# omerkurt-okt/buck-gnn

Hardware: AMD Instinct MI355X
Metric: graphs/sec (fwd+bwd) 6-layer SAGE h=512, ~5k-node meshes, batch 16, 1/2/4/8 GPU (higher is better)
Workload: dtype f32

## Files before the change

### buck-gnn_amd/bgnn/_lib.py

```python
from __future__ import annotations

import ctypes
import os
import threading

_HERE = os.path.dirname(os.path.abspath(__file__))
LIB_PATH = os.environ.get("BGNN_LIBRARY") or os.path.join(_HERE, "_lib", "libbgnn.so")
ABI_VERSION = 17

_lock = threading.Lock()
_lib = None

c_p = ctypes.c_void_p
c_i32 = ctypes.c_int32
c_i64 = ctypes.c_int64
c_f32 = ctypes.c_float
c_u64 = ctypes.c_uint64
c_sz = ctypes.c_size_t


class CsrStruct(ctypes.Structure):

    _fields_ = [
        ("rowptr", c_p),
        ("col", c_p),
        ("heavy_row", c_p),
        ("heavy_chunk0", c_p),
        ("chunk_heavy", c_p),
        ("n_rows", c_i64),
        ("nnz", c_i64),
        ("n_heavy", c_i32),
        ("n_chunks", c_i32),
        ("chunk", c_i32),
        ("ranges_all", c_i32),
        ("gsrc", c_p),
        ("gmask", c_p),
        ("gcnt", c_p),
        ("grow", c_p),
        ("n_groups", c_i64),
        ("group_rows", c_i32),
        ("_pad2", c_i32),
        ("ranges", c_p),
    ]


SIGNATURES = {
    "bgnn_abi_version": (c_i32, []),
    "bgnn_last_error_string": (ctypes.c_char_p, []),
    "bgnn_store_gather_graph": (c_i32, [c_p, c_i32, c_i64, c_i64, c_i64, c_i64, c_p, c_i64, c_p, c_p, c_p, c_p,
                                        c_p, c_p, c_p, c_p, c_p, c_p, c_p, c_p, c_p]),
    "bgnn_store_gather_rows": (c_i32, [c_p, c_i32, c_i32, c_i64, c_p, c_i64, c_p, c_p]),
    "bgnn_get_tuning": (c_i32, [c_i32]),
    "bgnn_heavy_timing": (c_i32, [c_i32]),
    "bgnn_gemm_w_tile": (c_i32, [c_i64, c_i64, c_i64]),
    "bgnn_gemm_wsplit_bytes": (c_sz, [c_i64, c_i64]),
    "bgnn_gemm_wsplit": (c_i32, [c_p, c_i32, c_i64, c_i64, c_i64, c_i64, c_p, c_i64, c_p, c_i64, c_i32, c_p]),
    "bgnn_gemm_f32_w": (c_i32, [c_i64, c_i64, c_i64, c_p, c_i64, c_p, c_i32, c_p, c_i64, c_p, c_i32, c_p, c_p, c_p,
                                c_p, c_i64, c_f32, c_u64, c_p]),
    "bgnn_heavy_timing_read": (c_i32, [c_i32, c_p, c_p]),
    "bgnn_set_tuning": (c_i32, [c_i32, c_i32]),
    "bgnn_graph_build_ws_bytes": (c_sz, [c_i64, c_i64]),
    "bgnn_graph_build": (c_i32, [c_p, c_i64, c_i64, c_p, c_p, c_p, c_p, c_p, c_p, c_sz, c_p, c_p]),
    "bgnn_index_csr_build": (c_i32, [c_p, c_i64, c_i64, c_p, c_p, c_p, c_sz, c_p, c_p]),
    "bgnn_heavy_plan_ws_bytes": (c_sz, [c_i64]),
    "bgnn_heavy_plan": (c_i32, [c_p, c_i64, c_i64, c_i32, c_p, c_p, c_p, c_p, c_p, c_sz, c_p]),
    "bgnn_spmm_fwd": (c_i32, [ctypes.POINTER(CsrStruct), c_p, c_i64, c_i32, c_i32, c_p, c_i64, c_p, c_p, c_p]),
    "bgnn_spmm_bwd": (c_i32, [ctypes.POINTER(CsrStruct), c_p, c_p, c_p, c_i64, c_i32, c_i32, c_p, c_i64, c_p, c_p,
                              c_i32, c_p]),
    "bgnn_heavy_ranges_bytes": (c_sz, [c_i32]),
    "bgnn_heavy_ranges": (c_i32, [ctypes.POINTER(CsrStruct), c_p, c_p]),
    "bgnn_range_partial_bytes": (c_sz, [c_i64, c_i32]),
    "bgnn_range_sums_finish": (c_i32, [c_p, c_i64, c_i32, ctypes.POINTER(CsrStruct), c_i32, c_p, c_i64, c_p, c_p,
                                       c_p]),
    "bgnn_bn_slots": (c_i32, [c_i64, c_i32]),
    "bgnn_bn_stats": (c_i32, [c_p, c_i64, c_i32, c_p, c_p]),
    "bgnn_bn_apply": (c_i32, [c_p, c_i64, c_i32, c_p, c_p, c_p, c_p]),
    "bgnn_bn_bwd_stats": (c_i32, [c_p, c_p, c_p, c_p, c_i64, c_i32, c_p, c_p]),
    "bgnn_bn_bwd_dx": (c_i32, [c_p, c_p, c_p, c_p, c_p, c_p, c_i64, c_i32, c_p, c_p]),
    "bgnn_spmm_bwd_add": (c_i32, [ctypes.POINTER(CsrStruct), c_p, c_p, c_p, c_i64, c_i32, c_i32, c_p, c_i64, c_p,
                                  c_i64, c_p, c_p, c_p]),
    "bgnn_spmm_bwd_max": (c_i32, [ctypes.POINTER(CsrStruct), c_p, c_p, c_i64, c_p, c_i64, c_i32, c_p, c_p, c_i64, c_p,
                                  c_i64, c_p, c_p, c_p]),
    "bgnn_spmm_max_arg_bytes": (c_sz, [c_i64, c_i32, c_i32]),
    "bgnn_sage_fwd_slots": (c_i32, [ctypes.POINTER(CsrStruct)]),
    "bgnn_group_plan": (c_i32, [c_p, c_p, c_i64, c_i32, c_i32, c_p, c_i64, c_p, c_p, c_p, c_p]),
    "bgnn_store_gather_groups": (c_i32, [c_p, c_i32, c_i32, c_i64, c_i64, c_i64, c_i64] + [c_p] * 14),
    "bgnn_sage_fwd": (c_i32, [ctypes.POINTER(CsrStruct), c_p, c_i64, c_p, c_i64, c_p, c_i32, c_i32, c_p, c_p, c_p,
                              c_p, c_p, c_i64, c_p]),
    "bgnn_bn_finalize": (c_i32, [c_p, c_i32, c_i32, c_i64, c_p, c_p, c_f32, c_f32, c_p, c_p, c_p, c_p, c_p, c_p,
                                 c_p]),
    "bgnn_bn_finalize_shifted": (c_i32, [c_p, c_i32, c_i32, c_i64, c_p, c_p, c_p, c_f32, c_f32, c_p, c_p, c_p, c_p, c_p, c_p,
                                 c_p]),
    "bgnn_bn_eval_coeffs": (c_i32, [c_i32, c_p, c_p, c_f32, c_p, c_p, c_p, c_p, c_p]),
    "bgnn_sage_apply": (c_i32, [c_p, c_p, c_p, c_p, c_i32, c_f32, c_u64, c_i64, c_i32, c_p, c_p, c_p, c_p, c_p]),
    "bgnn_sage_infer_bf16": (c_i32, [ctypes.POINTER(CsrStruct), c_p, c_i64, c_p, c_p, c_p, c_p, c_i64, c_i32, c_i32,
                                     c_p, c_i64, c_i32, c_p, c_p]),
    "bgnn_spmm_fwd_bf16": (c_i32, [ctypes.POINTER(CsrStruct), c_p, c_i64, c_i32, c_i32, c_p, c_i64, c_i32, c_p, c_p]),
    "bgnn_spmm_bwd_bf16": (c_i32, [ctypes.POINTER(CsrStruct), c_p, c_p, c_i64, c_i32, c_i32, c_p, c_i64, c_i32, c_p,
                                   c_p]),
    "bgnn_spmm_max_bf16": (c_i32, [ctypes.POINTER(CsrStruct), c_p, c_i64, c_i32, c_p, c_i64, c_p, c_p, c_p]),
    "bgnn_sage_tail_bf16": (c_i32, [c_p, c_i64, c_p, c_p, c_p, c_p, c_i64, c_i64, c_i32, c_p, c_i64, c_i32, c_p]),
    "bgnn_rows_slots": (c_i32, [c_i64]),
    "bgnn_sage_bwd_stats": (c_i32, [c_p, c_p, c_p, c_p, c_p, c_p, c_p, c_f32, c_u64, c_i64, c_i32, c_p, c_p]),
    "bgnn_reduce_partials": (c_i32, [c_p, c_i32, c_i32, c_p, c_p, c_i32, c_p]),
    "bgnn_linear_bwd_prep_slots": (c_i32, []),
    "bgnn_linear_bwd_prep": (c_i32, [c_p, c_p, c_i64, c_i32, c_p, c_p, c_p, c_p]),
    "bgnn_linear_bwd_prep_bf16": (c_i32, [c_p, c_p, c_i64, c_i32, c_p, c_p, c_p]),
    "bgnn_absmax_items_f32": (c_i32, [c_p, c_i32, c_i64, c_i64, c_i64, c_i64, c_p, c_i64, c_p]),
    "bgnn_add_dropped_bf16": (c_i32, [c_p, c_p, c_i64, c_f32, c_u64, c_p, c_p]),
    "bgnn_gemm_bf16_dropadd": (c_i32, [c_i64, c_i64, c_i64, c_p, c_i64, c_p, c_i64, c_p, c_i64, c_p, c_i64, c_f32,
                                       c_u64, c_p]),
    "bgnn_rel_error_loss": (c_i32, [c_p, c_p, c_i64, c_f32, c_f32, c_f32, c_p, c_p, c_p]),
    "bgnn_small_linear_fwd": (c_i32, [c_p, c_i64, c_i32, c_p, c_p, c_i32, c_i32, c_p, c_p]),
    "bgnn_small_linear_bwd": (c_i32, [c_p, c_p, c_p, c_i64, c_i32, c_p, c_i32, c_p, c_p, c_p, c_p]),
    "bgnn_sage_bwd_rows": (c_i32, [c_p, c_p, c_p, c_p, c_p, c_p, c_p, c_p, c_p, c_p, c_p, c_f32, c_u64, c_i32, c_i64,
                                   c_i32, c_p, c_i64, c_p, c_p, c_p, c_p, c_i32, c_p, c_p, c_p, c_p]),
    "bgnn_l2norm_bwd": (c_i32, [c_p, c_p, c_p, c_i64, c_i32, c_p, c_i64, c_p, c_p, c_p]),
    "bgnn_gemm_bf16": (c_i32, [c_i32, c_i32, c_i64, c_i64, c_i64, c_f32, c_p, c_i64, c_p, c_i64, c_f32, c_p, c_i64,
                               c_p, c_i32, c_i32, c_p, c_sz, c_p]),
    "bgnn_gemm_gather_add_bf16": (c_i32, [c_i64, c_i64, c_i64, c_p, c_i64, c_p, c_i64, c_p, c_i64, c_p, c_i32, c_p,
                                          c_p, c_i64, c_p, c_p, c_i64, c_i32, c_p, c_sz, c_p]),
    "bgnn_gemm_b16_variant": (c_i32, [c_i32]),
    "bgnn_add_dropout_bf16": (c_i32, [c_p, c_p, c_i64, c_f32, c_u64, c_p, c_p]),
    "bgnn_segment_sum_bf16": (c_i32, [c_p, c_p, c_i64, c_p, c_i64, c_i32, c_i32, c_p, c_i64, c_p]),
    "bgnn_segment_bcast_bf16": (c_i32, [c_p, c_p, c_i64, c_p, c_i64, c_i32, c_i32, c_p, c_i64, c_p]),
    "bgnn_gemm_ws_bytes": (c_sz, [c_i64, c_i64, c_i64, c_i32, c_i32]),
    "bgnn_gemm_set_cfg": (c_i32, [c_i32]),
    "bgnn_gemm_f32_planes": (c_i32, [c_i32, c_i32, c_i64, c_i64, c_i64, c_f32, c_p, c_i64, c_i64, c_i64, c_p, c_i64,
                                     c_f32, c_p, c_i64, c_i64, c_i64, c_p, c_i32, c_p, c_sz, c_p]),
    "bgnn_gemm_f32_scaled": (c_i32, [c_i32, c_i32, c_i64, c_i64, c_i64, c_f32, c_p, c_i64, c_i64, c_i64, c_p, c_i64,
                                     c_f32, c_p, c_i64, c_i64, c_i64, c_p, c_i32, c_p, c_p, c_p, c_i32, c_p, c_sz,
                                     c_p]),
    "bgnn_gemm_ws_bytes_ex": (c_sz, [c_i64, c_i64, c_i64, c_i32, c_i32, c_i32]),
    "bgnn_gemm_gather_add": (c_i32, [c_i32, c_i32, c_i64, c_i64, c_i64, c_p, c_i64, c_p, c_i64, c_p, c_i64, c_p, c_i32,
                                     c_p, c_p, c_i64, c_p, c_p, c_i64, c_i32, c_p, c_sz, c_p]),
    "bgnn_absmax_f32": (c_i32, [c_p, c_i64, c_i64, c_i64, c_p, c_i32, c_p]),
    "bgnn_gemm_f32_ex": (c_i32, [c_i32, c_i32, c_i64, c_i64, c_i64, c_f32, c_p, c_i64, c_p, c_i64, c_f32, c_p,
                                 c_i64, c_p, c_i32, c_p, c_sz, c_p]),
    "bgnn_topk_rank": (c_i32, [c_p, c_p, c_p, c_i64, c_p, c_p]),
    "bgnn_topk_select": (c_i32, [c_p, c_p, c_p, c_p, c_i64, c_p, c_p, c_p, c_p]),
    "bgnn_gather_scale": (c_i32, [c_p, c_i64, c_i32, c_p, c_p, c_i64, c_p, c_i64, c_p]),
    "bgnn_gather_scale_bwd": (c_i32, [c_p, c_i64, c_p, c_i64, c_i32, c_p, c_p, c_i64, c_p, c_i64, c_p, c_p]),
    "bgnn_filter_edges_ws_bytes": (c_sz, [c_i64]),
    "bgnn_filter_edges": (c_i32, [c_p, c_i64, c_p, c_i64, c_p, c_p, c_p, c_p, c_sz, c_p]),
    "bgnn_mlp2_supported": (c_i32, [c_i32, c_i32, c_i32]),
    "bgnn_mlp2_fwd": (c_i32, [c_p, c_i64, c_i32, c_i32, c_i32, c_p, c_p, c_p, c_p, c_p, c_p, c_p]),
    "bgnn_mlp2_bwd_ws_bytes": (c_sz, [c_i64]),
    "bgnn_mlp2_bwd": (c_i32, [c_p, c_i64, c_i32, c_i32, c_i32, c_p, c_p, c_p, c_p, c_p, c_p, c_p, c_p, c_p, c_p,
                              c_sz, c_p]),
    "bgnn_gemm_f32_dropadd": (c_i32, [c_i32, c_i32, c_i64, c_i64, c_i64, c_p, c_i64, c_p, c_i64, c_p, c_i64, c_p,
                                      c_p, c_p, c_i64, c_f32, c_u64, c_p, c_sz, c_p]),
    "bgnn_gemm_f32_dropadd_cols": (c_i32, [c_i64, c_i64, c_i64, c_p, c_i64, c_p, c_i64, c_p, c_i64, c_p, c_p, c_p,
                                           c_i64, c_i64, c_f32, c_u64, c_p, c_sz, c_p]),
    "bgnn_add_dropout": (c_i32, [c_p, c_p, c_i64, c_f32, c_u64, c_p, c_p]),
    "bgnn_fold_weights_supported": (c_i32, [c_i64, c_i64]),
    "bgnn_fold_weights_ws_bytes": (c_sz, [c_i64, c_i64]),
    "bgnn_fold_weights_fwd": (c_i32, [c_i64, c_i64, c_p, c_i64, c_p, c_i64, c_p, c_p, c_p, c_i64, c_p, c_p, c_i64,
                                      c_p, c_p]),
    "bgnn_fold_weights_bwd": (c_i32, [c_i64, c_i64, c_p, c_i64, c_p, c_p, c_i64, c_p, c_i64, c_p, c_p, c_p, c_i64,
                                      c_p, c_i64, c_p, c_p, c_sz, c_p]),
    "bgnn_gemm_f32": (c_i32, [c_i32, c_i32, c_i64, c_i64, c_i64, c_f32, c_p, c_i64, c_p, c_i64, c_f32, c_p, c_i64,
                              c_p, c_sz, c_p]),
}


class BgnnError(RuntimeError):
    def __init__(self, fn: str, code: int, msg: str):
        super().__init__(f"{fn} failed with code {code}: {msg}")
        self.code = code


def load():
    global _lib
    if _lib is not None:
        return _lib
    with _lock:
        if _lib is not None:
            return _lib
        if not os.path.exists(LIB_PATH):
            raise ImportError(
                f"bgnn: native library not found at {LIB_PATH}; build it with "
                "`python -c 'import __graft_entry__ as g; g.build()'` or `make -C buck-gnn_amd`")
        lib = ctypes.CDLL(LIB_PATH)
        for name, (res, args) in SIGNATURES.items():
            fn = getattr(lib, name)
            fn.restype = res
            fn.argtypes = args
        v = lib.bgnn_abi_version()
        if v != ABI_VERSION:
            raise ImportError(f"bgnn: ABI version mismatch (library {v}, python {ABI_VERSION})")
        _lib = lib
        return lib


def _checked(lib, name: str, args):
    fn = getattr(lib, name)
    sig = SIGNATURES.get(name)
    if sig is not None and len(args) != len(sig[1]):
        raise TypeError(f"bgnn: {name} takes {len(sig[1])} arguments, {len(args)} given")
    return fn


def call(name: str, *args):
    lib = load()
    rc = _checked(lib, name, args)(*args)
    if rc != 0:
        msg = lib.bgnn_last_error_string().decode(errors="replace")
        raise BgnnError(name, rc, msg)
    return rc


def query(name: str, *args):
    lib = load()
    return _checked(lib, name, args)(*args)
```

### buck-gnn_amd/bgnn/buckgnn.py

```python
from __future__ import annotations

from typing import Optional

import torch
from torch import Tensor, nn

from . import ea as ea_mod
from .ea import GradSlot as EAGradSlot, graphnet_block, skip_dropout
from . import _lib
from . import fused as _fused
from .fused import RangeRows, mlp, mlp_bf16, prepare_weights, sage_layer, small_mlp
from .graph import SegmentIndex, graph_for, _index_cache
from .nn import SAGEConv, SAGPooling, global_mean_pool, scatter_mean
from .ops import segment_reduce

FUSED_ENCODER = True
FOLD_ENCODER = True
FUSED_POOL = True

_SAGE_VARIANTS = {
    "GraphSage_sumAggr": ("sage_blocks_sum", "sum", True),
    "GraphSage_addAggr": ("sage_blocks_add", "add", True),
    "GraphSage_meanAggr": ("sage_blocks_mean", "mean", True),
    "GraphSage_maxAggr": ("sage_blocks_max", "max", True),
# ... 110 lines not shown
            self.batch_norms = nn.ModuleList()
            self.sage_mlps = nn.ModuleList()
            for _ in range(num_layers):
                getattr(self, attr).append(SAGEConv(in_channels=h, out_channels=h, normalize=True, aggr=aggr))
                self.batch_norms.append(nn.BatchNorm1d(h))
                self.sage_mlps.append(nn.Linear(h, h))
        self.batch_norm = nn.BatchNorm1d(h)
        self.relu = nn.ReLU()
        self.dropout = nn.Dropout(p=dropout_rate)
        self.pooling_mpl = MLPPooling(h, h, h)
        if model_name in ("GraphSAGE_SAG", "EAGNN_SAG"):
            n_before = num_layers // 2
            n_after = num_layers - n_before
            sag = model_name == "GraphSAGE_SAG"
            pre, bns = ("sage_layers_", True) if sag else ("gnn_layers_", False)

            def block():
                return SAGEConv(h, h, normalize=True, aggr="add") if sag else GraphNetBlock(h)
            setattr(self, pre + "1", nn.ModuleList([block() for _ in range(n_before)]))
            self.batch_norms_1 = nn.ModuleList([nn.BatchNorm1d(h) for _ in range(n_before)] if bns else [])
            self.pool = SAGPooling(h, ratio=0.5, GNN=SAGEConv, aggr="add")
            setattr(self, pre + "2", nn.ModuleList([block() for _ in range(n_after)]))
            self.batch_norms_2 = nn.ModuleList([nn.BatchNorm1d(h) for _ in range(n_after)] if bns else [])
        self.use_fused = True
        self.ea_bf16 = False
        self.infer_bf16 = False
        self._step = 0

    def get_pooling_layer(self, x: Tensor, edge_index: Tensor, batch: Optional[Tensor]) -> Tensor:
        mode = self.pooling_layer
        if mode == "mean":
            if batch is None:
                return global_mean_pool(x, None)
            return segment_reduce(x, batch_segments(batch), "mean")
        if mode == "hybrid":
            raise AttributeError("'BuckGNN' object has no attribute 'hybrid_pooling'")
        if mode == "mlp":
            return self.pooling_mpl(x, batch)
        if "super" not in mode and mode != "mlp_no_super" and mode != "mean_no_super":
            raise ValueError(f"Unknown pooling layer: {mode}")
        sup = super_node_index(batch, x.size(0), x.device)
        keep = torch.ones(x.size(0), dtype=torch.bool, device=x.device)
        keep[sup] = False
        real = torch.nonzero(keep).flatten()
        if batch is None:
            rb = torch.zeros(real.numel(), dtype=torch.long, device=x.device)
        else:
            rb = batch[real]
        if mode == "mean_no_super":
            return global_mean_pool(x[real], rb)
        if mode == "supernode_only":
            return x[sup]
        if mode == "supernode_with_pooling":
            return torch.cat([global_mean_pool(x[real], rb), x[sup]], 1)
        if mode == "mlp_no_super":
            return self.pooling_mpl(x[real], rb)
        raise ValueError(f"Unknown pooling layer: {mode}")

    def _seed(self) -> int:
        return int(torch.randint(0, 2 ** 62, (1,)).item())

    def _decode(self, h: Tensor) -> Tensor:
        dec = self.decoder
        hooked = bool(dec._forward_pre_hooks or dec._forward_hooks)
        out = small_mlp(dec, h) if (self.use_fused and not hooked) else None
        return dec(h) if out is None else out

    def _fused_ok(self, x: Tensor) -> bool:
        return (self.use_fused and x.is_cuda and x.dtype == torch.float32 and self.hidden_channels % 4 == 0
                and self.hidden_channels <= 512)

    def _sage_fused(self, x: Tensor, aggr: str) -> bool:
        return self._fused_ok(x) and aggr in ("add", "sum", "mean", "max")

    def _infer_bf16_on(self, x: Tensor, aggr: str, bns) -> bool:
        h = self.hidden_channels
        aggrs = ("add", "sum", "mean", "max") if self.infer_bf16 == "all" else ("add", "sum", "mean")
        return bool(self.infer_bf16 and not self.training and not torch.is_grad_enabled()
                    and self._fused_ok(x) and aggr in aggrs and h % 8 == 0 and h <= 512
                    and (bns is None or all(bn.track_running_stats and bn.running_mean is not None
                                            for bn in bns)))

    def _sage_loop_bf16(self, x: Tensor, edge_index: Tensor, convs, bns, aggr: str, pool=None):
        L = len(convs) if convs is not None else self.num_layers
        graph = graph_for(edge_index, x.size(0))
        if aggr == "max":
            x = self._sage_loop_bf16_max(x, graph, convs, bns, L)
            return (x, segment_reduce(x, pool, "mean")) if pool is not None else x
        red = 1 if aggr == "mean" else 0
        for i in range(L):
            conv = convs[i] if convs is not None else self.shared_graphsage_block
            coeffs = _fused.bn_eval_coeffs(bns[i]) if bns is not None else None
            x = _fused.sage_infer_layer(x, _fused.infer_weights(conv), conv.lin_l.bias, coeffs, graph, red,
                                        x_prev=x if 0 < i < L - 1 else None, out_f32=i == L - 1)
        return (x, segment_reduce(x, pool, "mean")) if pool is not None else x

    def _sage_loop_bf16_max(self, x: Tensor, graph, convs, bns, L: int) -> Tensor:
        if L == 0:
            return x
        N, H = x.size(0), self.hidden_channels
        bufs = [torch.empty(N, 2 * H, dtype=torch.bfloat16, device=x.device) for _ in range(min(L, 2))]
        y = torch.empty(N, H, dtype=torch.bfloat16, device=x.device)
        bufs[0][:, H:].copy_(x)
        out = None
        for i in range(L):
            conv = convs[i] if convs is not None else self.shared_graphsage_block
            coeffs = _fused.bn_eval_coeffs(bns[i]) if bns is not None else None
            cur = bufs[i % 2]
            last = i == L - 1
            out = (torch.empty(N, H, dtype=torch.float32, device=x.device) if last
                   else bufs[(i + 1) % 2][:, H:])
            _fused.sage_infer_max_layer(cur, _fused.infer_weights_max(conv), conv.lin_l.bias, coeffs, graph,
                                        cur[:, H:] if 0 < i < L - 1 else None, out, out_f32=last, y=y)
        return out

    def _foldable_encoder(self, x: Tensor) -> bool:
        enc = self.node_encoder
        return (FOLD_ENCODER and FUSED_ENCODER and isinstance(enc, nn.Sequential) and len(enc) >= 2
                and isinstance(enc[-1], nn.Linear) and enc[-1].out_features == self.hidden_channels
                and x.size(0) >= 1024 and self.num_layers >= 1)

    def _sage_loop(self, x: Tensor, edge_index: Tensor, convs, bns, aggr: str, skip_last_excluded: bool,
                   x_amax: Optional[Tensor] = None, x_in: Optional[nn.Linear] = None, pool=None):
        L = len(convs) if convs is not None else self.num_layers
        p = self.dropout.p
        if x_in is None and self._infer_bf16_on(x, aggr, bns):
            return self._sage_loop_bf16(x, edge_index, convs, bns, aggr, pool)
        if self._sage_fused(x, aggr):
            graph = graph_for(edge_index, x.size(0))
            red = {"mean": 1, "max": 2}.get(aggr, 0)
            amax = x_amax
            scratch = torch.zeros(4 * L + 5, dtype=torch.float32, device=x.device)
            bufs, fold_amax = scratch[:4 * L].view(L, 4), scratch[4 * L:]
            layers = [convs[i] if convs is not None else self.shared_graphsage_block for i in range(L)]
            rng_on = _range_rows_on(graph, red, x.size(0), layers[0].lin_l.weight.size(0))
            R = graph.fwd.plan.n_heavy if rng_on else 0
            wprep = prepare_weights([(c.lin_l.weight, c.lin_r.weight) for c in layers], bufs,
                                    [not (i == 0 and x_in is not None) for i in range(L)],
                                    n_rows=x.size(0) + R if red != 2 else 0)
            self._count_bn_batches(bns)
            x_full = None
            for i in range(L):
                conv = layers[i]
                bn = bns[i] if bns is not None else None
                skip = 0 < i < L - 1
                fold = x_in if i == 0 else None
                rng = (RangeRows(x_full=x_full, x_amax=bufs[i - 1, 3:4] if x_full is not None else None,
                                 out=i < L - 1, out_amax=bufs[i, 3:4]) if rng_on else None)
                pl = pool if (i == L - 1 and red != 2) else None
                out = sage_layer(x, conv.lin_l.weight, conv.lin_l.bias, conv.lin_r.weight, bn, graph, red,
                                 skip, p, self.training, self._seed(), x_amax=amax, return_amax=True,
                                 amax_buf=bufs[i], w_in=None if fold is None else fold.weight,
                                 b_in=None if fold is None else fold.bias, wprep=wprep[i], count_batch=False,
                                 fold_amax=fold_amax, rng=rng, pool=pl)
                x, amax = out[0], out[1]
                x_full = rng.holder[0] if (rng is not None and rng.holder) else None
            if pool is not None:
                return x, (out[2] if (red != 2 and L > 0) else segment_reduce(x, pool, "mean"))
            return x
        if x_in is not None:
            x = x_in(x)
        for i in range(L):
            x_prev = x
            conv = convs[i] if convs is not None else self.shared_graphsage_block
            x = conv(x, edge_index)
            if bns is not None:
                x = bns[i](x)
            x = self.relu(x)
            if 0 < i < L - 1:
                x = x + x_prev
            x = self.dropout(x)
        return (x, segment_reduce(x, pool, "mean")) if pool is not None else x

    def _count_bn_batches(self, bns) -> None:
        if bns is None or not self.training:
            return
        ts = [bn.num_batches_tracked for bn in bns if bn.track_running_stats]
        if ts:
            torch._foreach_add_(ts, 1)

    def _sag_sage_loop(self, x: Tensor, edge_index: Tensor, convs, bns, first_skip: bool,
                       x_amax: Optional[Tensor] = None, x_in: Optional[nn.Linear] = None) -> Tensor:
        p = self.dropout.p
        if self._sage_fused(x, "add"):
            graph = graph_for(edge_index, x.size(0))
            bufs = torch.zeros(len(convs), 3, dtype=torch.float32, device=x.device)
            for i, (conv, bn) in enumerate(zip(convs, bns)):
                skip = first_skip or i > 0
                fold = x_in if i == 0 else None
                y, y_amax = sage_layer(x, conv.lin_l.weight, conv.lin_l.bias, conv.lin_r.weight, bn, graph, 0,
                                       False, p, self.training, self._seed(), x_amax=x_amax, return_amax=True,
                                       amax_buf=bufs[i], w_in=None if fold is None else fold.weight,
                                       b_in=None if fold is None else fold.bias)
                x, x_amax = (y + x, None) if skip else (y, y_amax)
            return x
        if x_in is not None:
            x = x_in(x)
        for i, (conv, bn) in enumerate(zip(convs, bns)):
            identity = x
            x = self.dropout(self.relu(bn(conv(x, edge_index))))
            if first_skip or i > 0:
                x = x + identity
        return x

    def _skip_dropout(self, x, e, x_prev, e_prev, skip: bool, fused: bool, e_slot=None):
        if not fused:
            if skip:
                x, e = x + x_prev, e + e_prev
            return self.dropout(x), self.dropout(e)
        p = self.dropout.p
        return (skip_dropout(x, x_prev if skip else None, p, self.training, self._seed()),
                skip_dropout(e, e_prev if skip else None, p, self.training, self._seed(), slot=e_slot))

    def _ea_block(self, blk, x, e, edge_index, fused: bool):
        return graphnet_block(blk, x, e, edge_index, self.ea_bf16) if fused else blk(x, edge_index, e)

    def forward(self, x, edge_index, edge_attr, batch=None, mask=None):
        name = self.model_name
        if "super" in self.pooling_layer:
            is_real_node = x[:, -1] == 0 if x.size(1) > 0 else torch.ones(x.size(0), dtype=torch.bool,
                                                                           device=x.device)
            real_node_batch = batch[is_real_node] if batch is not None else None
        x_amax = None
        x_in = None
        sage = _SAGE_VARIANTS.get(name, (None, "add", None))[1] if name != "GraphSage_addAggr_Shared" else "add"
        infer = ((name in _SAGE_VARIANTS or name == "GraphSage_addAggr_Shared")
                 and self._infer_bf16_on(x, sage, self.batch_norms if name in _SAGE_VARIANTS else None))
        if (name in _SAGE_VARIANTS or name == "GraphSage_addAggr_Shared"
                or (name == "GraphSAGE_SAG" and len(self.sage_layers_1) >= 1)) and not infer \
                and self._sage_fused(x, sage) and sage != "max" and self._foldable_encoder(x):
            x_in = self.node_encoder[-1]
            x, x_amax = mlp(self.node_encoder[:-1], x, return_amax=True)
        elif self._fused_ok(x) and x.size(0) >= 1024 and FUSED_ENCODER:
            x, x_amax = mlp(self.node_encoder, x, return_amax=True)
        else:
            x = self.node_encoder(x)
        ea_fused = name in ("EA_GNN", "EA_GNN_Shared", "EAGNN_SAG") and self._fused_ok(x)
        if ea_fused:
            if self.ea_bf16 and ea_mod.BF16_STORAGE and edge_attr.size(0) >= 1024 and FUSED_ENCODER:
                e = mlp_bf16(self.edge_encoder, edge_attr)
            else:
                e = (mlp(self.edge_encoder, edge_attr) if edge_attr.size(0) >= 1024 and FUSED_ENCODER
                     else self.edge_encoder(edge_attr))
        if name == "EA_GNN_Shared":
            if not ea_fused:
                e = self.edge_encoder(edge_attr)
            for i in range(self.num_layers):
                x_prev, e_prev = x, e
                if ea_fused:
                    x, e = graphnet_block(self.shared_gn_block, x, e, edge_index, self.ea_bf16)
                else:
                    x, e = self.shared_gn_block(x, edge_index, e)
                x, e = self._skip_dropout(x, e, x_prev, e_prev, 0 < i < self.num_layers - 1, ea_fused)
        pool = (batch_segments(batch) if (FUSED_POOL and self.prediction_type == "buckling"
                                          and self.pooling_layer == "mean" and batch is not None
                                          and (name == "GraphSage_addAggr_Shared" or name in _SAGE_VARIANTS)
                                          and self._sage_fused(x, sage) and sage != "max") else None)
        pooled = None
        if name == "GraphSage_addAggr_Shared":
            x = self._sage_loop(x, edge_index, None, None, "add", True, x_amax, x_in, pool=pool)
            if pool is not None:
                x, pooled = x
        elif name == "EA_GNN":
            if not ea_fused:
                e = self.edge_encoder(edge_attr)
            L = len(self.gn_blocks)
            for i, blk in enumerate(self.gn_blocks):
                x_prev, e_prev = x, e
                slot = EAGradSlot() if (ea_fused and self.ea_bf16 and self.training and i < L - 1) else None
                if ea_fused:
                    x, e = graphnet_block(blk, x, e, edge_index, self.ea_bf16, slot=slot, slot_in=0 < i < L - 1)
                else:
                    x, e = blk(x, edge_index, e)
                x, e = self._skip_dropout(x, e, x_prev, e_prev, 0 < i < L - 1, ea_fused, e_slot=slot)
        elif name in _SAGE_VARIANTS:
            attr, aggr, _ = _SAGE_VARIANTS[name]
            x = self._sage_loop(x, edge_index, getattr(self, attr), self.batch_norms, aggr, True, x_amax, x_in,
                                pool=pool)
            if pool is not None:
                x, pooled = x
        elif name in ("GraphSage_addAggr_woBatchNorm", "GraphSage_MLP"):
            getattr(self, "sage_blocks_add")
        elif name == "GraphSage_sumAggr_woBatchNorm":
            getattr(self, "sage_blocks_sum")
        elif name == "GraphSAGE_SAG":
            x = self._sag_sage_loop(x, edge_index, self.sage_layers_1, self.batch_norms_1, False, x_amax, x_in)
            x, edge_index, edge_attr, batch, _perm, _score = self.pool(x, edge_index, edge_attr, batch)
            x = self._sag_sage_loop(x, edge_index, self.sage_layers_2, self.batch_norms_2, True)
        elif name == "EAGNN_SAG":
            if not ea_fused:
                e = self.edge_encoder(edge_attr)
            for i, blk in enumerate(self.gnn_layers_1):
                x_prev, e_prev = x, e
                x, e = self._ea_block(blk, x, e, edge_index, ea_fused)
                x, e = self.dropout(x), self.dropout(e)
                if i > 0:
                    x, e = x + x_prev, e + e_prev
            x, edge_index, e, batch, _perm, _score = self.pool(x, edge_index, e, batch)
            for blk in self.gnn_layers_2:
                x_prev, e_prev = x, e
                x, e = self._ea_block(blk, x, e, edge_index, ea_fused)
                x, e = self.dropout(x), self.dropout(e)
                x, e = x + x_prev, e + e_prev

        if self.prediction_type == "buckling":
            if pooled is None:
                pooled = self.get_pooling_layer(x, edge_index, batch)
# ... 7 lines not shown
```

### buck-gnn_amd/bgnn/fused.py

```python
from __future__ import annotations

import torch

from . import _lib
from .graph import Graph, _stream, require_cuda

GEMM_BACKEND = "hip"

PLANE_TILE = 128
Z_PLANES = False
DZ_PLANES = False
DGRAD_WT = True
FOLD_WEIGHTS_TORCH = False
FOLD_NATIVE = True
DGRAD_DROPADD = True

BF16_PREP = True
ABSMAX_ITEMS = True
PERSISTENT_WPACK = True
MAX_MERGED = True
WSPLIT = True

TIMERS = None
TIMER_EVENT = None
# ... 332 lines not shown
        ws_bytes = _lib.query("bgnn_mlp2_bwd_ws_bytes", N)
        ws = torch.empty(max(ws_bytes, 1), dtype=torch.uint8, device=x.device)
        _lib.call("bgnn_mlp2_bwd", x.data_ptr(), N, F, D1, D2, W1.data_ptr(), b1.data_ptr(), W2.data_ptr(),
                  h.data_ptr(), dh.data_ptr(), dW1.data_ptr(), db1.data_ptr(), dW2.data_ptr(), db2.data_ptr(),
                  ws.data_ptr(), ws_bytes, _stream())
        return None, dW1, db1, dW2, db2


class SmallMLPFn(torch.autograd.Function):

    @staticmethod
    def forward(ctx, x, relus, *params):
        x = x.contiguous()
        B = x.size(0)
        s = _stream()
        acts = [x]
        for i, relu in enumerate(relus):
            W, b = params[2 * i], params[2 * i + 1]
            N, K = W.shape
            y = torch.empty(B, N, dtype=torch.float32, device=x.device)
            _lib.call("bgnn_small_linear_fwd", acts[-1].data_ptr(), B, K, W.data_ptr(), _ptr(b), N, int(relu),
                      y.data_ptr(), s)
            acts.append(y)
        ctx.relus = relus
        ctx.has_bias = [params[2 * i + 1] is not None for i in range(len(relus))]
        ctx.save_for_backward(*acts, *[params[2 * i] for i in range(len(relus))])
        return acts[-1]

    @staticmethod
    def backward(ctx, g):
        L = len(ctx.relus)
        saved = ctx.saved_tensors
        acts, Ws = saved[:L + 1], saved[L + 1:]
        s = _stream()
        g = g.contiguous()
        B = g.size(0)
        grads = [None] * (2 * L)
        gx = None
        for i in reversed(range(L)):
            W = Ws[i]
            N, K = W.shape
            dW = torch.empty_like(W)
            db = torch.empty(N, dtype=torch.float32, device=W.device) if ctx.has_bias[i] else None
            need_dx = i > 0 or ctx.needs_input_grad[0]
            dx = torch.empty(B, K, dtype=torch.float32, device=W.device) if need_dx else None
            _lib.call("bgnn_small_linear_bwd", g.data_ptr(), acts[i + 1].data_ptr() if ctx.relus[i] else None,
                      acts[i].data_ptr(), B, K, W.data_ptr(), N, _ptr(dx), dW.data_ptr(), _ptr(db), s)
            grads[2 * i], grads[2 * i + 1] = dW, db
            g = dx
            gx = dx
        return (gx, None, *grads)


SMALL_MLP = True
SMALL_MLP_MAX_ROWS = 256


def small_mlp(seq: torch.nn.Sequential, x: torch.Tensor):
    if not (SMALL_MLP and x.is_cuda and x.dtype == torch.float32 and x.dim() == 2
            and 0 < x.size(0) <= SMALL_MLP_MAX_ROWS):
        return None
    mods = list(seq)
    relus, params = [], []
    i = 0
    while i < len(mods):
        m = mods[i]
        if not (isinstance(m, torch.nn.Linear) and m.weight.dtype == torch.float32 and m.in_features % 4 == 0
                and m.weight.is_contiguous()):
            return None
        relu = i + 1 < len(mods) and isinstance(mods[i + 1], torch.nn.ReLU)
        relus.append(relu)
        params += [m.weight, m.bias]
        i += 2 if relu else 1
    return SmallMLPFn.apply(x, tuple(relus), *params)


def _mlp2_prefix(mods, x: torch.Tensor) -> bool:
    if not FUSED_MLP2 or len(mods) < 4 or x.requires_grad or x.dtype != torch.float32 or x.dim() != 2:
        return False
    l1, r1, l2, r2 = mods[:4]
    if not (isinstance(l1, torch.nn.Linear) and isinstance(l2, torch.nn.Linear) and isinstance(r1, torch.nn.ReLU)
            and isinstance(r2, torch.nn.ReLU) and l1.bias is not None and l2.bias is not None):
        return False
    if l2.in_features != l1.out_features or x.size(1) != l1.in_features:
        return False
    return bool(_lib.query("bgnn_mlp2_supported", l1.in_features, l1.out_features, l2.out_features))


def _require_f32(x: torch.Tensor, what: str) -> None:
    if x.dtype != torch.float32:
        raise TypeError(f"{what}: the fused path takes float32 activations (got {x.dtype}); bf16 features run on "
                        "the per-module path (bgnn.nn.SAGEConv)")


def mlp(seq: torch.nn.Sequential, x: torch.Tensor, return_amax: bool = False, bf16: bool = False):
    _require_f32(x, "mlp")
    mods = list(seq)
    i = 0
    amax = None
    if not bf16 and _mlp2_prefix(mods, x):
        x, amax = _Mlp2Fn.apply(x.contiguous(), mods[0].weight, mods[0].bias, mods[2].weight, mods[2].bias)
        if len(mods) == 4:
            return (x, amax) if return_amax else x
        mods = mods[4:]
    n_lin = sum(isinstance(m, torch.nn.Linear) for m in mods)
    bufs = torch.zeros(n_lin, 2, dtype=torch.float32, device=x.device)
    k = 0
    while i < len(mods):
        m = mods[i]
        if isinstance(m, torch.nn.Linear):
            fuse = i + 1 < len(mods) and isinstance(mods[i + 1], torch.nn.ReLU)
            x, amax = linear(x, m.weight, m.bias, fuse, x_amax=amax, return_amax=True, bf16=bf16, amax_buf=bufs[k])
            k += 1
            i += 2 if fuse else 1
        else:
            x = m(x)
            amax = None
            i += 1
    return (x, amax) if return_amax else x


def _ptr(t):
    return None if t is None else t.data_ptr()


class RangeRows:
    __slots__ = ("x_full", "x_amax", "out", "out_amax", "bwd", "holder")

    def __init__(self, x_full=None, x_amax=None, out=False, out_amax=None, bwd=True):
        self.x_full, self.x_amax, self.out, self.out_amax, self.bwd = x_full, x_amax, out, out_amax, bwd
        self.holder = []


RANGE_ROWS = True


class LayerConfig:
    __slots__ = ("reduce", "bn", "training", "momentum", "eps", "skip", "p", "seed", "famax", "rng")

    def __init__(self, reduce: int, bn: bool, training: bool, momentum: float, eps: float, skip: bool,
                 p: float, seed: int):
        self.reduce = reduce
        self.bn = bn
        self.training = training
        self.momentum = momentum
        self.eps = eps
        self.skip = skip
        self.p = p if training else 0.0
        self.seed = seed
        self.famax = None
        self.rng = None


def _glue_fwd(o, bn_part, slots, x_prev, gamma, beta, running_mean, running_var, cfg: LayerConfig, next_amax,
              graph: Graph = None):
    N, H = o.shape
    dev = o.device
    s = _stream()
    scale = shift = mean = invstd = None
    if cfg.bn:
        scale = torch.empty(H, dtype=torch.float32, device=dev)
        shift = torch.empty(H, dtype=torch.float32, device=dev)
        mean = torch.empty(H, dtype=torch.float32, device=dev)
        invstd = torch.empty(H, dtype=torch.float32, device=dev)
        if cfg.training:
            _lib.call("bgnn_bn_finalize", bn_part.data_ptr(), slots, H, N, _ptr(gamma), _ptr(beta), cfg.eps,
                      cfg.momentum, _ptr(running_mean), _ptr(running_var), mean.data_ptr(), invstd.data_ptr(),
                      scale.data_ptr(), shift.data_ptr(), s)
        else:
            _lib.call("bgnn_bn_eval_coeffs", H, _ptr(gamma), _ptr(beta), cfg.eps, running_mean.data_ptr(),
                      running_var.data_ptr(), scale.data_ptr(), shift.data_ptr(), s)
            mean.copy_(running_mean)
            invstd.copy_(torch.rsqrt(running_var + cfg.eps))
    rng = cfg.rng
    if rng is not None and rng.out:
        R = graph.fwd.plan.n_heavy
        full = torch.empty(N + R, H, dtype=torch.float32, device=dev)
        x_next = full[:N]
        rp = torch.empty(_lib.query("bgnn_range_partial_bytes", N, H) // 4, dtype=torch.float32, device=dev)
        _lib.call("bgnn_sage_apply", o.data_ptr(), _ptr(scale), _ptr(shift), x_prev.data_ptr(), int(cfg.skip),
                  float(cfg.p), cfg.seed, N, H, x_next.data_ptr(), next_amax.data_ptr(), graph.fwd.ranges.data_ptr(),
                  rp.data_ptr(), s)
        _lib.call("bgnn_range_sums_finish", rp.data_ptr(), N, H, graph.fwd.ref(), 0, full[N:].data_ptr(), H,
                  next_amax.data_ptr(), rng.out_amax.data_ptr(), s)
        rng.holder.append(full)
        return x_next, (scale, shift, mean, invstd)
    x_next = torch.empty(N, H, dtype=torch.float32, device=dev)
    _lib.call("bgnn_sage_apply", o.data_ptr(), _ptr(scale), _ptr(shift), x_prev.data_ptr(), int(cfg.skip),
              float(cfg.p), cfg.seed, N, H, x_next.data_ptr(), next_amax.data_ptr(), None, None, s)
    return x_next, (scale, shift, mean, invstd)


def _glue_bwd_stats(g, o, scale, shift, mean, invstd, cfg: LayerConfig, g_rows=None):
    if not cfg.bn:
        return None, None, None, None
    N, H = o.shape
    dev = o.device
    s = _stream()
    rs = _lib.query("bgnn_rows_slots", N)
    part2 = torch.empty(rs, 2, H, dtype=torch.float32, device=dev)
    _lib.call("bgnn_sage_bwd_stats", g.data_ptr(), _ptr(g_rows), o.data_ptr(), scale.data_ptr(), shift.data_ptr(),
              mean.data_ptr(), invstd.data_ptr(), float(cfg.p), cfg.seed, N, H, part2.data_ptr(), s)
    sums = torch.empty(2, H, dtype=torch.float32, device=dev)
    _lib.call("bgnn_reduce_partials", part2.data_ptr(), rs, H, sums[0].data_ptr(), sums[1].data_ptr(), 0, s)
    dbeta, dgamma = sums[0], sums[1]
    if cfg.training:
        return dgamma, dbeta, sums[0], sums[1]
    z = torch.zeros(H, dtype=torch.float32, device=dev)
    return dgamma, dbeta, z, z


def _fold_native_ok(famax, wcat, w_in, b_in) -> bool:
    return bool(FOLD_NATIVE and GEMM_BACKEND == "hip" and famax is not None and famax.is_contiguous()
                and famax.numel() >= 5 and wcat.stride(1) == 1 and w_in.stride(1) == 1 and b_in.is_contiguous()
                and _lib.query("bgnn_fold_weights_supported", wcat.size(1), w_in.size(1)))


class SageLayerFn(torch.autograd.Function):

    @staticmethod
    def forward(ctx, x_prev, x_amax, w_l, b_l, w_r, gamma, beta, running_mean, running_var, graph: Graph,
                cfg: LayerConfig, amax=None, w_in=None, b_in=None, wprep=None, pool=None):
        dev = x_prev.device
        x_prev = x_prev.contiguous()
        H = w_l.size(0)
        N = x_prev.size(0)
        if isinstance(wprep, WPrep):
            wcat, wcat_t_pre, img_f, img_d = wprep.wcat, wprep.wcat_t, wprep, wprep
        elif wprep is not None:
            (wcat, wcat_t_pre), img_f, img_d = wprep, None, None
        else:
            wcat, wcat_t_pre, img_f, img_d = torch.cat([w_l, w_r], 0).contiguous(), None, None, None
        img_f = img_f if (img_f is not None and img_f.img_f is not None) else None
        img_d = img_d if (img_d is not None and img_d.img_d is not None) else None
        if amax is None:
            amax = torch.zeros(3, dtype=torch.float32, device=dev)
        w_amax, next_amax, dz_amax = amax[0:1], amax[1:2], amax[2:3]
        folded = w_in is not None
        if folded:
            if cfg.skip:
                raise ValueError("sage_layer: a folded input transform needs a layer without skip")
            wf_t = None
            fold_native = not FOLD_WEIGHTS_TORCH and _fold_native_ok(cfg.famax, wcat, w_in, b_in)
            if FOLD_WEIGHTS_TORCH:
                wf = torch.mm(wcat, w_in)
                bf = torch.mv(wcat, b_in)
            elif fold_native:
                K_in = w_in.size(1)
                wf = torch.empty(2 * H, K_in, dtype=torch.float32, device=dev)
                bf = torch.empty(2 * H, dtype=torch.float32, device=dev)
                wf_t = torch.empty(K_in, 2 * H, dtype=torch.float32, device=dev) if DGRAD_WT else None
                _lib.call("bgnn_fold_weights_fwd", H, K_in, wcat.data_ptr(), wcat.stride(0), w_in.data_ptr(),
                          w_in.stride(0), b_in.data_ptr(), cfg.famax.data_ptr(), wf.data_ptr(), K_in, bf.data_ptr(),
                          _ptr(wf_t), 2 * H, w_amax.data_ptr(), _stream())
            else:
                fs = cfg.famax
                fa = (fs[0:1], fs[1:2], fs[2:3]) if fs is not None else (None, None, None)
                if fs is not None:
                    absmax(wcat, fa[0], accumulate=True)
                    absmax(w_in, fa[1], accumulate=True)
                    absmax(b_in.view(1, -1), fa[2], accumulate=True)
                wf = gemm(wcat, w_in.contiguous(), trans_a=False, trans_b=False, a_amax=fa[0], b_amax=fa[1])
                bf = gemm(wcat, b_in.contiguous().view(H, 1), trans_a=False, trans_b=False, a_amax=fa[0],
                          b_amax=fa[2]).view(-1)
            if not fold_native:
                absmax(wf, w_amax, accumulate=True)
            wmat = wf
        else:
            if wprep is None:
                absmax(wcat, w_amax, accumulate=True)
            wmat, bf = wcat, None
        if x_amax is None:
            x_amax = absmax(x_prev)
        planes = Z_PLANES and H % PLANE_TILE == 0 and not folded
        rng = cfg.rng
        x_full = rng.x_full if (rng is not None and rng.x_full is not None and not folded and not planes) else None
        if x_full is not None and x_full.data_ptr() != x_prev.data_ptr():
            raise RuntimeError("sage_layer: RangeRows.x_full must start at x_prev")
        xa, a_amax_g = (x_full, rng.x_amax) if x_full is not None else (x_prev, x_amax)
        M = xa.size(0)
        with _timed("gemm_fwd_fold" if folded else "gemm_fwd"):
            if planes:
                z = torch.empty(2, N, H, dtype=torch.float32, device=dev)
                gemm(x_prev, wmat, trans_a=False, trans_b=True, out=Planes(z), a_amax=x_amax, b_amax=w_amax)
                zl, zr, ldz = z[0], z[1], H
            elif (img_f is not None and not folded
                  and _lib.query("bgnn_gemm_w_tile", M, 2 * H, H) == img_f.bn_f):
                z = torch.empty(M, 2 * H, dtype=torch.float32, device=dev)
                _lib.call("bgnn_gemm_f32_w", M, 2 * H, H, xa.data_ptr(), xa.stride(0), img_f.img_f.data_ptr(),
                          img_f.bn_f, z.data_ptr(), 2 * H, None, 0, a_amax_g.data_ptr(), w_amax.data_ptr(), None, None,
                          0, 0.0, 0, _stream())
                zl, zr, ldz = z, z[:, H:], 2 * H
            else:
                z = gemm(xa, wmat, trans_a=False, trans_b=True, bias=bf, a_amax=a_amax_g, b_amax=w_amax)
                zl, zr, ldz = z, z[:, H:], 2 * H
        hagg = z[N:] if x_full is not None else None
        o = torch.empty(N, H, dtype=torch.float32, device=dev)
        nrm = torch.empty(N, dtype=torch.float32, device=dev)
        slots = _lib.query("bgnn_sage_fwd_slots", graph.fwd.ref())
        bn_part = torch.empty(slots, 2, H, dtype=torch.float32, device=dev)
        part = (torch.empty(graph.fwd.plan.n_chunks * H, dtype=torch.float32, device=dev)
                if graph.fwd.plan.n_chunks else None)
        s = _stream()
        with _timed("sage_fwd"):
            _lib.call("bgnn_sage_fwd", graph.fwd.ref(), zl.data_ptr(), ldz, zr.data_ptr(), ldz, b_l.data_ptr(), H,
                      cfg.reduce, o.data_ptr(), nrm.data_ptr(), bn_part.data_ptr(), _ptr(part), _ptr(hagg),
                      2 * H if hagg is not None else 0, s)
        del z, zl, zr, hagg
        x_next, (scale, shift, mean, invstd) = _glue_fwd(o, bn_part, slots, x_prev, gamma, beta, running_mean,
                                                         running_var, cfg, next_amax, graph)
        ctx.graph = graph
        ctx.cfg = cfg
        ctx.folded = folded
        ctx.wcat_t = wcat_t_pre
        ctx.img_d = img_d if not folded else None
        ctx.set_materialize_grads(False)
        ctx.fold = (w_in, b_in, wf, wf_t) if folded else None
        ctx.save_for_backward(x_prev, o, nrm, wcat, gamma if gamma is not None else torch.empty(0, device=dev),
                              scale if scale is not None else torch.empty(0, device=dev),
                              shift if shift is not None else torch.empty(0, device=dev),
                              mean if mean is not None else torch.empty(0, device=dev),
                              invstd if invstd is not None else torch.empty(0, device=dev),
                              x_amax, w_amax, dz_amax)
        ctx.mark_non_differentiable(next_amax)
        ctx.pool = pool
        if pool is not None:
            from .ops import spmm_fwd
            pooled, _ = spmm_fwd(pool.fwd, x_next, 1, pool.num_rows)
            return x_next, next_amax, pooled
        return x_next, next_amax

    @staticmethod
    def backward(ctx, g, _g_amax, g_pool=None):
        cfg: LayerConfig = ctx.cfg
        g_rows = None
        if g_pool is not None:
            seg = ctx.pool
            gp = g_pool.contiguous() / seg.fwd.degree().clamp_min(1).to(g_pool.dtype).unsqueeze(1)
            if g is None and not cfg.skip:
                g, g_rows = gp, seg.index
            else:
                gb = gp.index_select(0, seg.index)
                g = gb if g is None else g + gb
        if g is None:
            return (None,) * 16
        x_prev, o, nrm, wcat, gamma, scale, shift, mean, invstd, x_amax, w_amax, dz_amax = ctx.saved_tensors
        graph: Graph = ctx.graph
        g = g.contiguous()
        N, H = o.shape
        planes = DZ_PLANES and H % PLANE_TILE == 0
        dev = o.device
        s = _stream()
        bn = cfg.bn
        dgamma, dbeta, sum_g2, sum_g2xhat = _glue_bwd_stats(g, o, scale, shift, mean, invstd, cfg, g_rows)
        if planes:
            dzt = torch.empty(2, N, H, dtype=torch.float32, device=dev)
            dz, dzl, dh, lddz = Planes(dzt), dzt[0], dzt[1], H
        else:
            dz = torch.empty(N, 2 * H, dtype=torch.float32, device=dev)
            dzl, dh, lddz = dz, dz[:, H:], 2 * H
        dropadd = (cfg.skip and DGRAD_DROPADD and GEMM_BACKEND == "hip" and DGRAD_WT and not planes
                   and H % 4 == 0 and _lib.query("bgnn_get_tuning", 5) == 2)
        gskip = torch.empty(N, H, dtype=torch.float32, device=dev) if (cfg.skip and not dropadd) else None
        rs = _lib.query("bgnn_rows_slots", N)
        part_db = torch.empty(rs, 2, H, dtype=torch.float32, device=dev)
        bw = graph.bwd
        rb = (cfg.rng is not None and cfg.rng.bwd and not planes and bw.ranges is not None)
        rp = (torch.empty(_lib.query("bgnn_range_partial_bytes", N, H) // 4, dtype=torch.float32, device=dev)
              if rb else None)
        _lib.call("bgnn_sage_bwd_rows", g.data_ptr(), _ptr(g_rows), o.data_ptr(), nrm.data_ptr(),
                  _ptr(scale) if bn else None, _ptr(shift) if bn else None,
                  _ptr(gamma) if (bn and gamma.numel()) else None,
                  _ptr(mean) if bn else None, _ptr(invstd) if bn else None, _ptr(sum_g2), _ptr(sum_g2xhat),
                  float(cfg.p), cfg.seed, int(cfg.skip and not dropadd), N, H, dh.data_ptr(), lddz, _ptr(gskip),
                  part_db.data_ptr(), dz_amax.data_ptr(), graph.fwd.rowptr.data_ptr() if ctx.folded else None,
                  (2 if cfg.reduce == 1 else 1) if ctx.folded else 0, _ptr(bw.ranges) if rb else None,
                  graph.fwd.rowptr.data_ptr() if (rb and cfg.reduce == 1) else None, _ptr(rp), s)
        if rb:
            _lib.call("bgnn_range_sums_finish", rp.data_ptr(), N, H, bw.ref(), 1, dzl.data_ptr(), lddz, None,
                      dz_amax.data_ptr(), s)
        db2 = torch.empty(2 if ctx.folded else 1, H, dtype=torch.float32, device=dev)
        _lib.call("bgnn_reduce_partials", part_db.data_ptr(), rs, H, db2[-1].data_ptr(),
                  db2[0].data_ptr() if ctx.folded else None, 0, s)
        db, db_zl = db2[-1], (db2[0] if ctx.folded else None)
        part = torch.empty(bw.plan.n_chunks * H, dtype=torch.float32, device=dev) if bw.plan.n_chunks else None
        with _timed("spmm_bwd"):
            _lib.call("bgnn_spmm_bwd", bw.ref(), graph.perm_t.data_ptr(), graph.fwd.rowptr.data_ptr(),
                      dh.data_ptr(), lddz, H, cfg.reduce, dzl.data_ptr(), lddz, _ptr(part),
                      dz_amax.data_ptr(), int(rb), s)
        has_affine = bn and gamma.numel() > 0
        if ctx.folded:
            w_in, b_in, wf, wf_t = ctx.fold
            wf_t = (wf_t if wf_t is not None else wf.t().contiguous()) if DGRAD_WT else wf
            with _timed("gemm_dgrad_fold"):
                dx = gemm(dz, wf_t, trans_a=False, trans_b=DGRAD_WT, a_amax=dz_amax, b_amax=w_amax)
            fs = cfg.famax
            fa = (fs[0:1], fs[1:2], fs[2:3], fs[3:4], fs[4:5]) if fs is not None else (None,) * 5
            with _timed("gemm_wgrad_fold"):
                dwf = gemm(dz, x_prev, trans_a=True, trans_b=False, a_amax=dz_amax, b_amax=x_amax,
                           c_amax=fa[3])
            dbf = db2.view(-1)
            fold_native = not FOLD_WEIGHTS_TORCH and _fold_native_ok(fs, wcat, w_in, b_in) and dwf.stride(1) == 1
            if fs is not None and not fold_native:
                absmax(db2, fa[4], accumulate=True)
            if fold_native:
                K_in = w_in.size(1)
                dw = torch.empty(2 * H, H, dtype=torch.float32, device=dev)
                dw_in = torch.empty(H, K_in, dtype=torch.float32, device=dev)
                db_in = torch.empty(H, dtype=torch.float32, device=dev)
                ws_bytes = _lib.query("bgnn_fold_weights_ws_bytes", H, K_in)
                ws = torch.empty(ws_bytes, dtype=torch.uint8, device=dev) if ws_bytes else None
                _lib.call("bgnn_fold_weights_bwd", H, K_in, dwf.data_ptr(), dwf.stride(0), dbf.data_ptr(),
                          wcat.data_ptr(), wcat.stride(0), w_in.data_ptr(), w_in.stride(0), b_in.data_ptr(),
                          fs.data_ptr(), dw.data_ptr(), H, dw_in.data_ptr(), K_in, db_in.data_ptr(), _ptr(ws),
                          ws_bytes, s)
            elif FOLD_WEIGHTS_TORCH:
                dw = torch.addmm(torch.outer(dbf, b_in), dwf, w_in.t())
                dw_in = torch.mm(wcat.t(), dwf)
                db_in = torch.mv(wcat.t(), dbf)
            else:
                dw = gemm(dwf, w_in.contiguous(), trans_a=False, trans_b=True, a_amax=fa[3],
                          b_amax=fa[1])
                dw.add_(torch.outer(dbf, b_in))
                dw_in = gemm(wcat, dwf, trans_a=True, trans_b=False, a_amax=fa[0], b_amax=fa[3])
                db_in = gemm(wcat, dbf.view(-1, 1), trans_a=True, trans_b=False, a_amax=fa[0],
                             b_amax=fa[4]).view(-1)
            return (dx, None, dw[:H], db, dw[H:], dgamma if has_affine else None, dbeta if has_affine else None,
                    None, None, None, None, None, dw_in, db_in, None, None)
        wcat_t = (ctx.wcat_t if ctx.wcat_t is not None else wcat.t().contiguous()) if DGRAD_WT else wcat
        img_d = ctx.img_d if (not planes and DGRAD_WT) else None
        if (img_d is not None and (dropadd or gskip is None)
                and _lib.query("bgnn_gemm_w_tile", N, H, 2 * H) == img_d.bn_d):
            dx = torch.empty(N, H, dtype=torch.float32, device=dev)
            with _timed("gemm_dgrad"):
                _lib.call("bgnn_gemm_f32_w", N, H, 2 * H, dz.data_ptr(), lddz, img_d.img_d.data_ptr(), img_d.bn_d,
                          dx.data_ptr(), H, None, 0, dz_amax.data_ptr(), w_amax.data_ptr(), None,
                          g.data_ptr() if dropadd else None, H, float(cfg.p) if dropadd else 0.0,
                          cfg.seed if dropadd else 0, s)
        elif dropadd:
            dx = torch.empty(N, H, dtype=torch.float32, device=dev)
            M_, K_ = N, 2 * H
            ws_bytes = _lib.query("bgnn_gemm_ws_bytes_ex", M_, H, K_, 0, 1, 0)
            ws = torch.empty(ws_bytes, dtype=torch.uint8, device=dev) if ws_bytes else None
            with _timed("gemm_dgrad"):
                _lib.call("bgnn_gemm_f32_dropadd", 0, 1, M_, H, K_, dz.data_ptr(), lddz, wcat_t.data_ptr(),
                          wcat_t.stride(0), dx.data_ptr(), H, dz_amax.data_ptr(), w_amax.data_ptr(), g.data_ptr(),
                          H, float(cfg.p), cfg.seed, _ptr(ws), ws_bytes, s)
        elif gskip is not None:
            with _timed("gemm_dgrad"):
                dx = gemm(dz, wcat_t, trans_a=False, trans_b=DGRAD_WT, out=gskip, beta=1.0, a_amax=dz_amax,
                          b_amax=w_amax)
        else:
            with _timed("gemm_dgrad"):
                dx = gemm(dz, wcat_t, trans_a=False, trans_b=DGRAD_WT, a_amax=dz_amax, b_amax=w_amax)
        with _timed("gemm_wgrad"):
            dw = gemm(dz, x_prev, trans_a=True, trans_b=False, a_amax=dz_amax, b_amax=x_amax)
        dw_l, dw_r = dw[:H], dw[H:]
        return (dx, None, dw_l, db, dw_r, dgamma if has_affine else None, dbeta if has_affine else None,
                None, None, None, None, None, None, None, None, None)


def _max_transform(x, w_l, w_r, graph: Graph, x_amax, w_amax, name: str):
    from .ops import spmm_fwd
    N, C = x.shape
    with _timed("agg_max"):
        agg, arg = spmm_fwd(graph.fwd, x, 2, N, want_arg=True)
    wk = torch.cat([w_l, w_r], 1)
    in_place = C % 32 == 0 and (x.data_ptr() - agg.data_ptr()) % 16 == 0
    a = Pair(agg, x) if in_place else torch.cat([agg, x], 1)
    with _timed(name):
        y = gemm(a, wk, trans_a=False, trans_b=True, a_amax=x_amax, b_amax=w_amax)
    return y, agg, arg


def _max_rows_fwd(y, b_l, H: int):
    from .graph import empty_csr
    N = y.size(0)
    dev = y.device
    csr = empty_csr(N, dev)
    bias = b_l if b_l is not None else torch.zeros(H, dtype=torch.float32, device=dev)
    o = torch.empty(N, H, dtype=torch.float32, device=dev)
    nrm = torch.empty(N, dtype=torch.float32, device=dev)
    slots = _lib.query("bgnn_sage_fwd_slots", csr.ref())
    bn_part = torch.empty(slots, 2, H, dtype=torch.float32, device=dev)
    _lib.call("bgnn_sage_fwd", csr.ref(), y.data_ptr(), y.stride(0), y.data_ptr(), y.stride(0), bias.data_ptr(), H,
              0, o.data_ptr(), nrm.data_ptr(), bn_part.data_ptr(), None, None, 0, _stream())
    return o, nrm, bn_part, slots


def _max_backward(dh, dz_amax, wcat_t, x, agg, arg, graph: Graph, x_amax, w_amax, addend_beta_src,
                  need_dx: bool, p: float = 0.0, seed: int = 0):
    N, H = dh.shape
    C = x.size(1)
    dev = dh.device
    dx = None
    hip16 = GEMM_BACKEND == "hip" and _lib.query("bgnn_get_tuning", 5) == 2
    if need_dx and MAX_MERGED and hip16 and C % 256 == 0:
        wkt = torch.cat([wcat_t[:, :H], wcat_t[:, H:]], 0)
        with _timed("gemm_dgrad"):
            dt = torch.empty(N, 2 * C, dtype=torch.float32, device=dev)
            if addend_beta_src is not None:
                ws_bytes = _lib.query("bgnn_gemm_ws_bytes_ex", N, 2 * C, H, 0, 1, 0)
                ws = torch.empty(ws_bytes, dtype=torch.uint8, device=dev) if ws_bytes else None
                _lib.call("bgnn_gemm_f32_dropadd_cols", N, 2 * C, H, dh.data_ptr(), dh.stride(0), wkt.data_ptr(), H,
                          dt.data_ptr(), 2 * C, dz_amax.data_ptr(), w_amax.data_ptr(), addend_beta_src.data_ptr(),
                          addend_beta_src.stride(0), C, float(p), seed, _ptr(ws), ws_bytes, _stream())
            else:
                gemm(dh, wkt, trans_a=False, trans_b=True, out=dt, a_amax=dz_amax, b_amax=w_amax)
        dagg, t = dt[:, :C], dt[:, C:]
        dx = torch.empty(N, C, dtype=torch.float32, device=dev)
        bw = graph.bwd
        part = torch.empty(bw.plan.n_chunks * C, dtype=torch.float32, device=dev) if bw.plan.n_chunks else None
        with _timed("spmm_bwd"):
            _lib.call("bgnn_spmm_bwd_max", bw.ref(), graph.perm_t.data_ptr(), graph.fwd.rowptr.data_ptr(), N,
                      dagg.data_ptr(), 2 * C, C, arg.data_ptr(), t.data_ptr(), 2 * C,
                      dx.data_ptr(), dx.stride(0), _ptr(part), None, _stream())
        del dt, dagg, t
    elif need_dx:
        wl_t, wr_t = wcat_t[:, :H], wcat_t[:, H:]
        with _timed("gemm_dgrad"):
            dagg = gemm(dh, wl_t, trans_a=False, trans_b=True, a_amax=dz_amax, b_amax=w_amax)
            if addend_beta_src is not None and hip16:
                t = torch.empty(N, wcat_t.size(0), dtype=torch.float32, device=dev)
                ws_bytes = _lib.query("bgnn_gemm_ws_bytes_ex", N, t.size(1), H, 0, 1, 0)
                ws = torch.empty(ws_bytes, dtype=torch.uint8, device=dev) if ws_bytes else None
                _lib.call("bgnn_gemm_f32_dropadd", 0, 1, N, t.size(1), H, dh.data_ptr(), dh.stride(0),
                          wr_t.data_ptr(), wr_t.stride(0), t.data_ptr(), t.stride(0), dz_amax.data_ptr(),
                          w_amax.data_ptr(), addend_beta_src.data_ptr(), addend_beta_src.stride(0), float(p), seed,
                          _ptr(ws), ws_bytes, _stream())
            else:
                t = gemm(dh, wr_t, trans_a=False, trans_b=True, a_amax=dz_amax, b_amax=w_amax)
                if addend_beta_src is not None:
                    t.add_(_dropped(addend_beta_src, p, seed))
        dx = torch.empty(N, x.size(1), dtype=torch.float32, device=dev)
        bw = graph.bwd
        part = torch.empty(bw.plan.n_chunks * x.size(1), dtype=torch.float32, device=dev) if bw.plan.n_chunks else None
        with _timed("spmm_bwd"):
            _lib.call("bgnn_spmm_bwd_max", bw.ref(), graph.perm_t.data_ptr(), graph.fwd.rowptr.data_ptr(), N,
                      dagg.data_ptr(), dagg.stride(0), x.size(1), arg.data_ptr(), t.data_ptr(), t.stride(0),
                      dx.data_ptr(), dx.stride(0), _ptr(part), None, _stream())
    with _timed("gemm_wgrad"):
        if (MAX_MERGED and GEMM_BACKEND == "hip" and C % 256 == 0 and agg.shape == x.shape
                and agg.stride() == x.stride() and (x.data_ptr() - agg.data_ptr()) % 16 == 0):
            dwt = gemm(Pair(agg, x), dh, trans_a=True, trans_b=False, a_amax=x_amax, b_amax=dz_amax)
            dw_l, dw_r = dwt[:C].t(), dwt[C:].t()
        else:
            dw_l = gemm(dh, agg, trans_a=True, trans_b=False, a_amax=dz_amax, b_amax=x_amax)
            dw_r = gemm(dh, x, trans_a=True, trans_b=False, a_amax=dz_amax, b_amax=x_amax)
    return dx, dw_l, dw_r


def _dropped(g, p: float, seed: int):
    out = torch.empty_like(g)
    _lib.call("bgnn_add_dropout", g.data_ptr(), None, g.numel(), float(p), seed, out.data_ptr(), _stream())
    return out


class SageMaxLayerFn(torch.autograd.Function):

    @staticmethod
    def forward(ctx, x_prev, x_amax, w_l, b_l, w_r, gamma, beta, running_mean, running_var, graph: Graph,
                cfg: LayerConfig, amax=None, wprep=None):
        dev = x_prev.device
        x_prev = x_prev.contiguous()
        H = w_l.size(0)
        if amax is None:
            amax = torch.zeros(3, dtype=torch.float32, device=dev)
        w_amax, next_amax, dz_amax = amax[0:1], amax[1:2], amax[2:3]
        if wprep is not None:
            w0, w1 = (wprep.wcat, wprep.wcat_t) if isinstance(wprep, WPrep) else wprep
            wcat_t = w1 if w1 is not None else w0.t().contiguous()
        else:
            wcat_t = torch.cat([w_l, w_r], 0).t().contiguous()
            absmax(wcat_t, w_amax, accumulate=True)
        if x_amax is None:
            x_amax = absmax(x_prev)
        y, agg, arg = _max_transform(x_prev, w_l, w_r, graph, x_amax, w_amax, "gemm_fwd_max")
        with _timed("sage_fwd"):
            o, nrm, bn_part, slots = _max_rows_fwd(y, b_l, H)
        del y
        x_next, (scale, shift, mean, invstd) = _glue_fwd(o, bn_part, slots, x_prev, gamma, beta, running_mean,
                                                         running_var, cfg, next_amax)
        ctx.graph = graph
        ctx.cfg = cfg
        ctx.set_materialize_grads(False)
        e = torch.empty(0, device=dev)
        ctx.save_for_backward(x_prev, agg, arg, o, nrm, wcat_t, gamma if gamma is not None else e,
                              scale if scale is not None else e, shift if shift is not None else e,
                              mean if mean is not None else e, invstd if invstd is not None else e,
                              x_amax, w_amax, dz_amax)
        ctx.mark_non_differentiable(next_amax)
        return x_next, next_amax

    @staticmethod
    def backward(ctx, g, _g_amax):
        if g is None:
            return (None,) * 13
        (x_prev, agg, arg, o, nrm, wcat_t, gamma, scale, shift, mean, invstd, x_amax, w_amax,
         dz_amax) = ctx.saved_tensors
        cfg: LayerConfig = ctx.cfg
        g = g.contiguous()
        N, H = o.shape
        dev = o.device
        s = _stream()
        bn = cfg.bn
        dgamma, dbeta, sum_g2, sum_g2xhat = _glue_bwd_stats(g, o, scale, shift, mean, invstd, cfg)
        dh = torch.empty(N, H, dtype=torch.float32, device=dev)
        rs = _lib.query("bgnn_rows_slots", N)
        part_db = torch.empty(rs, 2, H, dtype=torch.float32, device=dev)
        _lib.call("bgnn_sage_bwd_rows", g.data_ptr(), None, o.data_ptr(), nrm.data_ptr(),
                  _ptr(scale) if bn else None, _ptr(shift) if bn else None,
                  _ptr(gamma) if (bn and gamma.numel()) else None,
                  _ptr(mean) if bn else None, _ptr(invstd) if bn else None, _ptr(sum_g2), _ptr(sum_g2xhat),
                  float(cfg.p), cfg.seed, 0, N, H, dh.data_ptr(), H, None, part_db.data_ptr(), dz_amax.data_ptr(),
                  None, 0, None, None, None, s)
        db = torch.empty(H, dtype=torch.float32, device=dev)
        _lib.call("bgnn_reduce_partials", part_db.data_ptr(), rs, H, db.data_ptr(), None, 0, s)
        dx, dw_l, dw_r = _max_backward(dh, dz_amax, wcat_t, x_prev, agg, arg, ctx.graph, x_amax, w_amax,
                                       g if cfg.skip else None, ctx.needs_input_grad[0], cfg.p, cfg.seed)
        has_affine = bn and gamma.numel() > 0
        return (dx, None, dw_l, db, dw_r, dgamma if has_affine else None, dbeta if has_affine else None,
                None, None, None, None, None, None)


def _weight_pack(pairs, L: int, H: int):
    dev = pairs[0][0].device
    W = torch.empty(L, 2 * H, H, dtype=torch.float32, device=dev)
    Wt = torch.empty(L, H, 2 * H, dtype=torch.float32, device=dev) if DGRAD_WT else None
    torch._foreach_copy_([W[i, k * H:(k + 1) * H] for i in range(L) for k in (0, 1)], [t for pr in pairs for t in pr])
    if Wt is not None:
        Wt.copy_(W.transpose(1, 2))
    return W, Wt


class WPrep:
    __slots__ = ("wcat", "wcat_t", "img_f", "bn_f", "img_d", "bn_d")

    def __init__(self, wcat, wcat_t, img_f=None, bn_f=0, img_d=None, bn_d=0):
        self.wcat, self.wcat_t = wcat, wcat_t
        self.img_f, self.bn_f, self.img_d, self.bn_d = img_f, bn_f, img_d, bn_d


def _wsplit_run(W, i, j, amax_bufs, M):
    _, N, K = W.shape
    bn = _lib.query("bgnn_gemm_w_tile", M, N, K)
    if bn == 0:
        return None, 0
    nb = _lib.query("bgnn_gemm_wsplit_bytes", N, K)
    img = torch.empty(j - i, nb, dtype=torch.uint8, device=W.device)
    _lib.call("bgnn_gemm_wsplit", W[i].data_ptr(), j - i, W.stride(0), N, K, W.stride(1), amax_bufs[i].data_ptr(),
              amax_bufs.stride(0), img.data_ptr(), nb, bn, _stream())
    return img, bn


def prepare_weights(pairs, amax_bufs: torch.Tensor, fill_amax, n_rows: int = 0):
    L = len(pairs)
    H = pairs[0][0].size(0)
    with torch.no_grad():
        if PERSISTENT_WPACK and all(a.dtype == torch.float32 and b.dtype == torch.float32 and a.is_contiguous()
                                    and b.is_contiguous() and a.shape == (H, H) and b.shape == (H, H)
                                    for a, b in pairs):
            W, Wt = _weight_pack(pairs, L, H)
        else:
            W = torch.cat([t for pr in pairs for t in pr], 0).view(L, 2 * H, H)
            Wt = W.transpose(1, 2).contiguous() if DGRAD_WT else None
        i = 0
        while i < L:
            if not fill_amax[i]:
                i += 1
                continue
            j = i
            while j < L and fill_amax[j]:
                j += 1
            if ABSMAX_ITEMS and amax_bufs.is_contiguous() and H % 4 == 0:
                _lib.call("bgnn_absmax_items_f32", W[i].data_ptr(), j - i, 2 * H * H, 2 * H, H, H,
                          amax_bufs[i].data_ptr(), amax_bufs.stride(0), _stream())
            else:
                for k in range(i, j):
                    absmax(W[k], amax_bufs[k, 0:1], accumulate=True)
            i = j
        out = [WPrep(W[i], Wt[i] if Wt is not None else None) for i in range(L)]
        if (WSPLIT and n_rows > 0 and GEMM_BACKEND == "hip" and Wt is not None and not Z_PLANES and not DZ_PLANES
                and amax_bufs.is_contiguous() and _lib.query("bgnn_get_tuning", 5) == 2):
            i = 0
            while i < L:
                if not fill_amax[i]:
                    i += 1
                    continue
                j = i
                while j < L and fill_amax[j]:
                    j += 1
                img_f, bn_f = _wsplit_run(W, i, j, amax_bufs, n_rows)
                img_d, bn_d = _wsplit_run(Wt, i, j, amax_bufs, n_rows)
                for k in range(i, j):
                    o = out[k]
                    if img_f is not None:
                        o.img_f, o.bn_f = img_f[k - i], bn_f
                    if img_d is not None:
                        o.img_d, o.bn_d = img_d[k - i], bn_d
                i = j
    return out


def sage_layer(x_prev: torch.Tensor, w_l: torch.Tensor, b_l: torch.Tensor, w_r: torch.Tensor,
               bn_module, graph: Graph, reduce: int, skip: bool, p: float, training: bool,
               seed: int, x_amax: torch.Tensor = None, return_amax: bool = False, amax_buf=None,
               w_in: torch.Tensor = None, b_in: torch.Tensor = None, wprep=None, count_batch: bool = True,
               fold_amax: torch.Tensor = None, rng: RangeRows = None, pool=None):
    require_cuda(x_prev, w_l, b_l, w_r, what="sage_layer")
    _require_f32(x_prev, "sage_layer")
    H = w_l.size(0)
    if w_in is None and x_prev.size(1) != H:
        raise ValueError(f"sage_layer: x has {x_prev.size(1)} features, the layer {H}")
    if H % 4 or H > 512:
        raise ValueError(f"sage_layer: fused path needs H % 4 == 0 and H <= 512 (got {H})")
    if reduce not in (0, 1, 2):
        raise ValueError("sage_layer: reduce must be 0 (sum), 1 (mean) or 2 (max)")
    if reduce == 2 and w_in is not None:
        raise ValueError("sage_layer: max aggregation needs its input rows (no folded input transform)")
    if reduce == 2 and pool is not None:
        raise ValueError("sage_layer: the fused mean pool is for sum / mean layers")
    if bn_module is not None:
        use_batch_stats = training or not bn_module.track_running_stats
        momentum = bn_module.momentum
        if training and bn_module.track_running_stats:
            if count_batch:
                bn_module.num_batches_tracked.add_(1)
            if momentum is None:
                momentum = 1.0 / float(bn_module.num_batches_tracked.item())
        cfg = LayerConfig(reduce, True, use_batch_stats, float(momentum or 0.0) if bn_module.track_running_stats
                          else 0.0, float(bn_module.eps), skip, p, seed)
        cfg.p = p if training else 0.0
        cfg.famax = fold_amax if w_in is not None else None
        cfg.rng = rng if reduce != 2 else None
        if reduce == 2:
            out = SageMaxLayerFn.apply(x_prev, x_amax, w_l, b_l, w_r, bn_module.weight, bn_module.bias,
                                       bn_module.running_mean, bn_module.running_var, graph, cfg, amax_buf, wprep)
        else:
            out = SageLayerFn.apply(x_prev, x_amax, w_l, b_l, w_r, bn_module.weight, bn_module.bias,
                                    bn_module.running_mean, bn_module.running_var, graph, cfg, amax_buf, w_in, b_in,
                                    wprep, pool)
    else:
        cfg = LayerConfig(reduce, False, training, 0.0, 0.0, skip, p, seed)
        cfg.famax = fold_amax if w_in is not None else None
        cfg.rng = rng if reduce != 2 else None
        if reduce == 2:
            out = SageMaxLayerFn.apply(x_prev, x_amax, w_l, b_l, w_r, None, None, None, None, graph, cfg, amax_buf,
                                       wprep)
        else:
            out = SageLayerFn.apply(x_prev, x_amax, w_l, b_l, w_r, None, None, None, None, graph, cfg, amax_buf,
                                    w_in, b_in, wprep, pool)
    if pool is not None:
        return out if return_amax else (out[0], out[2])
    return out if return_amax else out[0]


class SageConvFn(torch.autograd.Function):

    @staticmethod
    def forward(ctx, x, w_l, b_l, w_r, graph: Graph, reduce: int):
        dev = x.device
        x = x.contiguous()
        N = x.size(0)
        H = w_l.size(0)
        wcat = torch.cat([w_l, w_r], 0).contiguous()
        amax = torch.zeros(2, dtype=torch.float32, device=dev)
        w_amax, x_amax = amax[0:1], amax[1:2]
        absmax(wcat, w_amax, accumulate=True)
        absmax(x, x_amax, accumulate=True)
        ctx.graph = graph
        ctx.reduce = reduce
        ctx.has_bias = b_l is not None
        if reduce == 2:
            y, agg, arg = _max_transform(x, w_l, w_r, graph, x_amax, w_amax, "conv_gemm_fwd")
            with _timed("conv_sage_fwd"):
                o, nrm, _, _ = _max_rows_fwd(y, b_l, H)
            ctx.save_for_backward(x, o, nrm, wcat, x_amax, w_amax, agg, arg)
            return o
        with _timed("conv_gemm_fwd"):
            z = gemm(x, wcat, trans_a=False, trans_b=True, a_amax=x_amax, b_amax=w_amax)
        bias = b_l if b_l is not None else torch.zeros(H, dtype=torch.float32, device=dev)
        o = torch.empty(N, H, dtype=torch.float32, device=dev)
        nrm = torch.empty(N, dtype=torch.float32, device=dev)
        slots = _lib.query("bgnn_sage_fwd_slots", graph.fwd.ref())
        bn_part = torch.empty(slots, 2, H, dtype=torch.float32, device=dev)
        part = (torch.empty(graph.fwd.plan.n_chunks * H, dtype=torch.float32, device=dev)
                if graph.fwd.plan.n_chunks else None)
        with _timed("conv_sage_fwd"):
            _lib.call("bgnn_sage_fwd", graph.fwd.ref(), z.data_ptr(), 2 * H, z[:, H:].data_ptr(), 2 * H,
                      bias.data_ptr(), H, reduce, o.data_ptr(), nrm.data_ptr(), bn_part.data_ptr(), _ptr(part),
                      None, 0, _stream())
        ctx.save_for_backward(x, o, nrm, wcat, x_amax, w_amax)
        return o

    @staticmethod
    def backward(ctx, g):
        x, o, nrm, wcat, x_amax, w_amax = ctx.saved_tensors[:6]
        graph: Graph = ctx.graph
        g = g.contiguous()
        N, H = o.shape
        dev = o.device
        s = _stream()
        mx = ctx.reduce == 2
        dz = torch.empty(N, H if mx else 2 * H, dtype=torch.float32, device=dev)
        dh = dz if mx else dz[:, H:]
        rs = _lib.query("bgnn_rows_slots", N)
        part_db = torch.empty(rs, 2, H, dtype=torch.float32, device=dev)
        dz_amax = torch.zeros(1, dtype=torch.float32, device=dev)
        _lib.call("bgnn_l2norm_bwd", g.data_ptr(), o.data_ptr(), nrm.data_ptr(), N, H, dh.data_ptr(), dh.stride(0),
                  part_db.data_ptr(), dz_amax.data_ptr(), s)
        db = None
        if ctx.has_bias and ctx.needs_input_grad[2]:
            db = torch.empty(H, dtype=torch.float32, device=dev)
            _lib.call("bgnn_reduce_partials", part_db.data_ptr(), rs, H, db.data_ptr(), None, 0, s)
        if mx:
            agg, arg = ctx.saved_tensors[6:]
            dx, dw_l, dw_r = _max_backward(dh, dz_amax, wcat.t().contiguous(), x, agg, arg, graph, x_amax, w_amax,
                                           None, ctx.needs_input_grad[0])
            return dx, dw_l, db, dw_r, None, None
        bw = graph.bwd
        part = torch.empty(bw.plan.n_chunks * H, dtype=torch.float32, device=dev) if bw.plan.n_chunks else None
        with _timed("conv_spmm_bwd"):
            _lib.call("bgnn_spmm_bwd", bw.ref(), graph.perm_t.data_ptr(), graph.fwd.rowptr.data_ptr(),
                      dh.data_ptr(), 2 * H, H, ctx.reduce, dz.data_ptr(), 2 * H, _ptr(part),
                      dz_amax.data_ptr(), 0, s)
        dx = None
        if ctx.needs_input_grad[0]:
            with _timed("conv_gemm_dgrad"):
                dx = gemm(dz, wcat.t().contiguous(), trans_a=False, trans_b=True, a_amax=dz_amax, b_amax=w_amax)
        dw = None
        if ctx.needs_input_grad[1] or ctx.needs_input_grad[3]:
            with _timed("conv_gemm_wgrad"):
                dw = gemm(dz, x, trans_a=True, trans_b=False, a_amax=dz_amax, b_amax=x_amax)
        return (dx, None if dw is None else dw[:H], db, None if dw is None else dw[H:], None, None)


def sage_conv(x: torch.Tensor, w_l: torch.Tensor, b_l, w_r: torch.Tensor, graph: Graph, reduce: int):
    require_cuda(x, w_l, w_r, what="sage_conv")
    _require_f32(x, "sage_conv")
    return SageConvFn.apply(x, w_l, b_l, w_r, graph, reduce)



def infer_weights(conv) -> torch.Tensor:
    w_l, w_r = conv.lin_l.weight, conv.lin_r.weight
    key = (w_l._version, w_r._version, w_l.data_ptr(), w_r.data_ptr(), str(w_l.device))
    hit = getattr(conv, "_bgnn_infer_wcat", None)
    if hit is not None and hit[0] == key:
        return hit[1]
    with torch.no_grad():
        wcat = torch.cat([w_l.detach(), w_r.detach()], 0).to(torch.bfloat16).contiguous()
    conv._bgnn_infer_wcat = (key, wcat)
    return wcat


def bn_eval_coeffs(bn):
    H = bn.num_features
    dev = bn.running_mean.device
    scale = torch.empty(H, dtype=torch.float32, device=dev)
    shift = torch.empty(H, dtype=torch.float32, device=dev)
    _lib.call("bgnn_bn_eval_coeffs", H, _ptr(bn.weight), _ptr(bn.bias), float(bn.eps), bn.running_mean.data_ptr(),
              bn.running_var.data_ptr(), scale.data_ptr(), shift.data_ptr(), _stream())
    return scale, shift


@torch.no_grad()
def sage_infer_layer(x: torch.Tensor, w_cat: torch.Tensor, bias, bn_coeffs, graph: Graph, reduce: int,
                     x_prev=None, out_f32: bool = False) -> torch.Tensor:
    require_cuda(x, w_cat, bias, x_prev, what="sage_infer_layer")
    N, H = x.size(0), w_cat.size(1)
    if w_cat.dtype != torch.bfloat16 or w_cat.size(0) != 2 * H or x.size(1) != H:
        raise ValueError("sage_infer_layer: w_cat must be bfloat16 [2H, H] and x [N, H]")
    if H % 8 or H > 512:
        raise ValueError(f"sage_infer_layer: needs H % 8 == 0 and H <= 512 (got {H})")
    if reduce not in (0, 1):
        raise ValueError("sage_infer_layer: reduce must be 0 (sum) or 1 (mean)")
    dev = x.device
    xb = x if x.dtype == torch.bfloat16 else x.to(torch.bfloat16)
    if xb.stride(1) != 1 or xb.stride(0) % 8:
        xb = xb.contiguous()
    with _timed("infer_gemm"):
        z = gemm_bf16(xb, w_cat, trans_a=False, trans_b=True, out_bf16=True)
    xp = None
    if x_prev is not None:
        xp = x_prev if x_prev.dtype == torch.bfloat16 else x_prev.to(torch.bfloat16)
        if xp.stride(1) != 1 or xp.stride(0) % 8:
            xp = xp.contiguous()
    scale, shift = bn_coeffs if bn_coeffs is not None else (None, None)
    out = torch.empty(N, H, dtype=torch.float32 if out_f32 else torch.bfloat16, device=dev)
    n_chunks = graph.fwd.plan.n_chunks
    part = torch.empty(n_chunks * H, dtype=torch.float32, device=dev) if n_chunks else None
    with _timed("sage_infer"):
        _lib.call("bgnn_sage_infer_bf16", graph.fwd.ref(), z.data_ptr(), z.stride(0), _ptr(bias), _ptr(scale),
                  _ptr(shift), _ptr(xp), xp.stride(0) if xp is not None else 0, H, reduce, out.data_ptr(),
                  out.stride(0), int(out_f32), _ptr(part), _stream())
    return out



def infer_weights_max(conv) -> torch.Tensor:
    w_l, w_r = conv.lin_l.weight, conv.lin_r.weight
    key = (w_l._version, w_r._version, w_l.data_ptr(), w_r.data_ptr(), str(w_l.device))
    hit = getattr(conv, "_bgnn_infer_wcat_max", None)
    if hit is not None and hit[0] == key:
# ... 38 lines not shown
```

### buck-gnn_amd/csrc/common.h

```cpp
#pragma once

#include <hip/hip_runtime.h>
#include <stdint.h>
#include <stdio.h>
#include <stdarg.h>
#include <string.h>

#include "../../include/bgnn.h"

namespace bgnn {

constexpr int kWave = 64;
constexpr int kNumXcd = 8;

void set_error(const char* fmt, ...);
int fail(int code, const char* fmt, ...);

#define BGNN_HIP(expr)                                                              \
    do {                                                                            \
        hipError_t _e = (expr);                                                     \
        if (_e != hipSuccess)                                                       \
            return ::bgnn::fail((int)_e, "%s failed: %s (%s:%d)", #expr,            \
                                hipGetErrorString(_e), __FILE__, __LINE__);         \
    } while (0)

#define BGNN_CHECK_LAUNCH() BGNN_HIP(hipGetLastError())

#define BGNN_REQUIRE(cond, ...)                                                     \
    do {                                                                            \
        if (!(cond)) return ::bgnn::fail(BGNN_E_ARG, __VA_ARGS__);                  \
    } while (0)

static inline hipStream_t as_stream(void* s) { return reinterpret_cast<hipStream_t>(s); }
static inline bool aligned16(const void* p) { return ((uintptr_t)p & 15) == 0; }

static inline size_t align_up(size_t x, size_t a) { return (x + a - 1) / a * a; }

__device__ __forceinline__ int xcd_remap(int b, int nblk) {
    const int q = nblk / kNumXcd, r = nblk % kNumXcd;
    const int x = b % kNumXcd, i = b / kNumXcd;
    return (x < r ? x * (q + 1) : r * (q + 1) + (x - r) * q) + i;
}

__device__ __forceinline__ int xcd_remap_rev(int b, int nblk) {
    const int q = nblk / kNumXcd, r = nblk % kNumXcd;
    const int x = b % kNumXcd, i = b / kNumXcd;
    const int len = x < r ? q + 1 : q;
    return (x < r ? x * (q + 1) : r * (q + 1) + (x - r) * q) + len - 1 - i;
}

__device__ __forceinline__ float group_sum(float v, int width) {
    for (int m = width >> 1; m > 0; m >>= 1) v += __shfl_xor(v, m, kWave);
    return v;
}

__device__ __forceinline__ uint64_t mix64(uint64_t z) {
    z += 0x9E3779B97F4A7C15ull;
    z = (z ^ (z >> 30)) * 0xBF58476D1CE4E5B9ull;
    z = (z ^ (z >> 27)) * 0x94D049BB133111EBull;
    return z ^ (z >> 31);
}

__device__ __forceinline__ uint32_t keep_bits4(uint64_t seed, uint64_t g, uint32_t thr) {
    const uint64_t h = mix64(seed ^ (g * 0xD1B54A32D192ED03ull));
    uint32_t m = 0;
#pragma unroll
    for (int k = 0; k < 4; ++k) m |= (((uint32_t)(h >> (16 * k)) & 0xFFFFu) >= thr ? 1u : 0u) << k;
    return m;
}

static inline uint32_t dropout_threshold(float p) {
    if (!(p > 0.f)) return 0u;
    double t = (double)p * 65536.0 + 0.5;
    if (t > 65536.0) t = 65536.0;
    return (uint32_t)t;
}

void set_gemm_mode(int mode);
int gemm_mode();
void set_rows_nt(int on);
int rows_nt();
void set_rows_rev(int on);
int rows_rev();

__device__ __forceinline__ void store4(float* p, float a, float b, float c, float d, bool nt) {
    typedef float f32x4_t __attribute__((ext_vector_type(4)));
    const f32x4_t t = {a, b, c, d};
    if (nt) __builtin_nontemporal_store(t, reinterpret_cast<f32x4_t*>(p));
    else *reinterpret_cast<f32x4_t*>(p) = t;
}

}
```

### buck-gnn_amd/csrc/sage.hip

```cpp
#include "common.h"
#include "ranges.h"

namespace bgnn {

constexpr int kGroups = 16;

__global__ __launch_bounds__(256) void k_slots_stage1(float* __restrict__ part, int n_slots, int W, int per) {
    const int c = blockIdx.x * 256 + threadIdx.x;
    const int g = blockIdx.y;
    if (c >= W) return;
    const int s0 = g * per, s1 = min(n_slots, s0 + per);
    if (s0 >= s1) return;
    float acc[8] = {0, 0, 0, 0, 0, 0, 0, 0};
    int s = s0;
    for (; s + 8 <= s1; s += 8) {
#pragma unroll
        for (int u = 0; u < 8; ++u) acc[u] += part[(int64_t)(s + u) * W + c];
    }
    for (; s < s1; ++s) acc[0] += part[(int64_t)s * W + c];
    part[(int64_t)s0 * W + c] = ((acc[0] + acc[1]) + (acc[2] + acc[3])) + ((acc[4] + acc[5]) + (acc[6] + acc[7]));
}

inline int slots_stage1(float* part, int n_slots, int H, hipStream_t s) {
    if (n_slots <= kGroups) return 1;
    const int per = (n_slots + kGroups - 1) / kGroups;
    hipLaunchKernelGGL(k_slots_stage1, dim3((2 * H + 255) / 256, kGroups), dim3(256), 0, s, part, n_slots, 2 * H,
                       per);
    return per;
}

__global__ __launch_bounds__(256) void k_reduce_partials(const float* __restrict__ part, int n_slots, int stride,
                                                         int H, float* __restrict__ out0, float* __restrict__ out1,
                                                         int accumulate) {
    __shared__ double red[4][2][64];
    const int cl = threadIdx.x & 63, ph = threadIdx.x >> 6;
    const int c = blockIdx.x * 64 + cl;
    double s0 = 0.0, s1 = 0.0;
    if (c < H)
        for (int sl = ph * stride; sl < n_slots; sl += 4 * stride) {
            s0 += (double)part[(int64_t)sl * 2 * H + c];
            s1 += (double)part[(int64_t)sl * 2 * H + H + c];
        }
    red[ph][0][cl] = s0;
    red[ph][1][cl] = s1;
    __syncthreads();
    if (ph == 0 && c < H) {
        s0 = (red[0][0][cl] + red[1][0][cl]) + (red[2][0][cl] + red[3][0][cl]);
        s1 = (red[0][1][cl] + red[1][1][cl]) + (red[2][1][cl] + red[3][1][cl]);
        if (out0) out0[c] = accumulate ? out0[c] + (float)s0 : (float)s0;
        if (out1) out1[c] = accumulate ? out1[c] + (float)s1 : (float)s1;
    }
}

__global__ __launch_bounds__(256) void k_bn_finalize(const float* __restrict__ part, int n_slots, int stride, int H,
                                                     int64_t count, const float* __restrict__ gamma,
                                                     const float* __restrict__ beta, float eps, float momentum,
                                                     float* __restrict__ rmean, float* __restrict__ rvar,
                                                     float* __restrict__ mean, float* __restrict__ invstd,
                                                     float* __restrict__ scale, float* __restrict__ shift) {
    __shared__ double red[4][2][64];
    const int cl = threadIdx.x & 63, ph = threadIdx.x >> 6;
    const int c = blockIdx.x * 64 + cl;
    double s0 = 0.0, s1 = 0.0;
    if (c < H)
        for (int sl = ph * stride; sl < n_slots; sl += 4 * stride) {
            s0 += (double)part[(int64_t)sl * 2 * H + c];
            s1 += (double)part[(int64_t)sl * 2 * H + H + c];
        }
    red[ph][0][cl] = s0;
    red[ph][1][cl] = s1;
    __syncthreads();
    if (ph == 0 && c < H) {
        s0 = (red[0][0][cl] + red[1][0][cl]) + (red[2][0][cl] + red[3][0][cl]);
        s1 = (red[0][1][cl] + red[1][1][cl]) + (red[2][1][cl] + red[3][1][cl]);
        const double n = (double)count;
        const double mu = s0 / n;
        double var = s1 / n - mu * mu;
        if (var < 0.0) var = 0.0;
        const double is = 1.0 / sqrt(var + (double)eps);
        const float g = gamma ? gamma[c] : 1.f;
        const float b = beta ? beta[c] : 0.f;
        mean[c] = (float)mu;
        invstd[c] = (float)is;
        scale[c] = (float)((double)g * is);
        shift[c] = (float)((double)b - mu * (double)g * is);
        if (rmean && rvar && momentum > 0.f) {
            const double unb = count > 1 ? var * n / (n - 1.0) : var;
            rmean[c] = (float)((1.0 - momentum) * (double)rmean[c] + momentum * mu);
            rvar[c] = (float)((1.0 - momentum) * (double)rvar[c] + momentum * unb);
        }
    }
}

template <int MODE>
__global__ __launch_bounds__(256) void k_reduce_slots(const float* __restrict__ part, int n_slots, int H,
                                                      float* __restrict__ out0, float* __restrict__ out1,
                                                      int accumulate, int64_t count, const float* __restrict__ gamma,
                                                      const float* __restrict__ beta, float eps, float momentum,
                                                      float* __restrict__ rmean, float* __restrict__ rvar,
                                                      float* __restrict__ mean, float* __restrict__ invstd,
                                                      float* __restrict__ scale, float* __restrict__ shift,
                                                      const float* __restrict__ kshift) {
    constexpr int CPB = 8, NPH = 256 / CPB;
    __shared__ double red[2][NPH][CPB];
    const int cl = threadIdx.x % CPB, ph = threadIdx.x / CPB;
    const int c = blockIdx.x * CPB + cl;
    const int64_t W = 2 * (int64_t)H;
    double s0 = 0.0, s1 = 0.0;
    if (c < H) {
        int sl = ph;
        for (; sl + 7 * NPH < n_slots; sl += 8 * NPH) {
            float a[8], b[8];
#pragma unroll
            for (int u = 0; u < 8; ++u) {
                a[u] = part[(int64_t)(sl + u * NPH) * W + c];
                b[u] = part[(int64_t)(sl + u * NPH) * W + H + c];
            }
#pragma unroll
            for (int u = 0; u < 8; ++u) {
                s0 += (double)a[u];
                s1 += (double)b[u];
            }
        }
        for (; sl < n_slots; sl += NPH) {
            s0 += (double)part[(int64_t)sl * W + c];
            s1 += (double)part[(int64_t)sl * W + H + c];
        }
    }
    red[0][ph][cl] = s0;
    red[1][ph][cl] = s1;
    __syncthreads();
    for (int o = NPH / 2; o > 0; o >>= 1) {
        if (ph < o) {
            red[0][ph][cl] += red[0][ph + o][cl];
            red[1][ph][cl] += red[1][ph + o][cl];
        }
        __syncthreads();
    }
    if (ph != 0 || c >= H) return;
    s0 = red[0][0][cl];
    s1 = red[1][0][cl];
    if constexpr (MODE == 0) {
        if (out0) out0[c] = accumulate ? out0[c] + (float)s0 : (float)s0;
        if (out1) out1[c] = accumulate ? out1[c] + (float)s1 : (float)s1;
    } else {
        const double n = (double)count;
        const double mu0 = s0 / n;
        double var = s1 / n - mu0 * mu0;
        if (var < 0.0) var = 0.0;
        const double mu = kshift ? (double)kshift[c] + mu0 : mu0;
        const double is = 1.0 / sqrt(var + (double)eps);
        const float g = gamma ? gamma[c] : 1.f;
        const float b = beta ? beta[c] : 0.f;
        mean[c] = (float)mu;
        invstd[c] = (float)is;
        scale[c] = (float)((double)g * is);
        shift[c] = (float)((double)b - mu * (double)g * is);
        if (rmean && rvar && momentum > 0.f) {
            const double unb = count > 1 ? var * n / (n - 1.0) : var;
            rmean[c] = (float)((1.0 - momentum) * (double)rmean[c] + momentum * mu);
            rvar[c] = (float)((1.0 - momentum) * (double)rvar[c] + momentum * unb);
        }
    }
}

static int g_one_pass_reduce = 1;

__global__ void k_bn_eval(int H, const float* __restrict__ gamma, const float* __restrict__ beta, float eps,
                          const float* __restrict__ rmean, const float* __restrict__ rvar,
                          float* __restrict__ scale, float* __restrict__ shift) {
    const int c = blockIdx.x * blockDim.x + threadIdx.x;
    if (c >= H) return;
    const double is = 1.0 / sqrt((double)rvar[c] + (double)eps);
    const double g = gamma ? gamma[c] : 1.0;
    const double b = beta ? beta[c] : 0.0;
    scale[c] = (float)(g * is);
    shift[c] = (float)(b - (double)rmean[c] * g * is);
}

__device__ __forceinline__ void block_amax(uint32_t* amax, uint32_t m) {
    for (int o = 32; o > 0; o >>= 1) m = max(m, (uint32_t)__shfl_xor((int)m, o, kWave));
    __shared__ uint32_t red[4];
    if ((threadIdx.x & 63) == 0) red[threadIdx.x >> 6] = m;
    __syncthreads();
    if (threadIdx.x == 0) {
        m = max(max(red[0], red[1]), max(red[2], red[3]));
        if (m) atomicMax(amax, m);
    }
}

__global__ __launch_bounds__(256) void k_sage_apply(const float4* __restrict__ o, const float* __restrict__ scale,
                                                    const float* __restrict__ shift,
                                                    const float4* __restrict__ xprev, int skip, uint32_t thr,
                                                    float inv_keep, uint64_t seed, int64_t n4, int H4,
                                                    float4* __restrict__ xn, uint32_t* __restrict__ amax, int nt,
                                                    int rev) {
    uint32_t m = 0;
    int64_t lo = 0, hi = n4, i0 = (int64_t)blockIdx.x * blockDim.x + threadIdx.x, st = (int64_t)gridDim.x * blockDim.x;
    if (rev) {
        const int64_t nr = n4 / H4, x = blockIdx.x & 7;
        lo = (nr * x / 8) * H4;
        hi = (nr * (x + 1) / 8) * H4;
        i0 = (int64_t)(blockIdx.x >> 3) * blockDim.x + threadIdx.x;
        st = (int64_t)(gridDim.x >> 3) * blockDim.x;
    }
    for (int64_t q = i0; q < hi - lo; q += st) {
        const int64_t i = rev ? hi - 1 - q : q;
        const int c = (int)(i % H4) * 4;
        float4 v = o[i];
        float y[4] = {v.x, v.y, v.z, v.w};
        if (scale) {
            const float4 sc = *reinterpret_cast<const float4*>(scale + c);
            const float4 sh = *reinterpret_cast<const float4*>(shift + c);
            y[0] = y[0] * sc.x + sh.x; y[1] = y[1] * sc.y + sh.y;
            y[2] = y[2] * sc.z + sh.z; y[3] = y[3] * sc.w + sh.w;
        }
#pragma unroll
        for (int k = 0; k < 4; ++k) y[k] = fmaxf(y[k], 0.f);
        if (skip) {
            const float4 p = xprev[i];
            y[0] += p.x; y[1] += p.y; y[2] += p.z; y[3] += p.w;
        }
        if (thr) {
            const uint32_t keep = keep_bits4(seed, (uint64_t)i, thr);
#pragma unroll
            for (int k = 0; k < 4; ++k) y[k] = ((keep >> k) & 1u) ? y[k] * inv_keep : 0.f;
        }
        store4(reinterpret_cast<float*>(xn + i), y[0], y[1], y[2], y[3], nt);
#pragma unroll
        for (int k = 0; k < 4; ++k) m = max(m, __float_as_uint(y[k]) & 0x7fffffffu);
    }
    if (amax) block_amax(amax, m);
}

template <int NV>
__global__ __launch_bounds__(256) void k_sage_apply_rows(const float* __restrict__ o, const float* __restrict__ scale,
                                                         const float* __restrict__ shift,
                                                         const float* __restrict__ xprev, int skip, uint32_t thr,
                                                         float inv_keep, uint64_t seed, int64_t n_rows, int H,
                                                         int64_t rpb, float* __restrict__ xn,
                                                         uint32_t* __restrict__ amax, int nt,
                                                         const int32_t* __restrict__ ranges,
                                                         float* __restrict__ rpart) {
    const int lane = threadIdx.x & 63;
    const int wave = __builtin_amdgcn_readfirstlane(threadIdx.x >> 6);
    const int lb = xcd_remap_rev(blockIdx.x, gridDim.x);
    const int64_t r0 = (int64_t)lb * rpb;
    const int64_t r1 = min(n_rows, r0 + rpb);
    const int H4 = H / 4;
    BlockRanges br;
    br.load(ranges, r0, r1);
    __shared__ float4 racc[4][kRangeSlots][128];
    int c4[NV];
    bool cok[NV];
    float4 sc[NV], sh[NV];
#pragma unroll
    for (int v = 0; v < NV; ++v) {
        c4[v] = lane + 64 * v;
        cok[v] = c4[v] < H4;
        const int c = cok[v] ? 4 * c4[v] : 0;
        sc[v] = scale ? *reinterpret_cast<const float4*>(scale + c) : make_float4(1.f, 1.f, 1.f, 1.f);
        sh[v] = shift ? *reinterpret_cast<const float4*>(shift + c) : make_float4(0.f, 0.f, 0.f, 0.f);
#pragma unroll
        for (int q = 0; q < kRangeSlots; ++q)
            if (cok[v]) racc[wave][q][c4[v]] = make_float4(0.f, 0.f, 0.f, 0.f);
    }
    uint32_t m = 0;
    auto row = [&](int64_t r) {
        const int sl = br.slot(r);
#pragma unroll
        for (int v = 0; v < NV; ++v) {
            if (!cok[v]) continue;
            const int64_t i = r * H4 + c4[v];
            const float4 ov = reinterpret_cast<const float4*>(o)[i];
            float y[4] = {ov.x, ov.y, ov.z, ov.w};
            if (scale) {
                y[0] = y[0] * sc[v].x + sh[v].x; y[1] = y[1] * sc[v].y + sh[v].y;
                y[2] = y[2] * sc[v].z + sh[v].z; y[3] = y[3] * sc[v].w + sh[v].w;
            }
#pragma unroll
            for (int k = 0; k < 4; ++k) y[k] = fmaxf(y[k], 0.f);
            if (skip) {
                const float4 p = reinterpret_cast<const float4*>(xprev)[i];
                y[0] += p.x; y[1] += p.y; y[2] += p.z; y[3] += p.w;
            }
            if (thr) {
                const uint32_t keep = keep_bits4(seed, (uint64_t)i, thr);
#pragma unroll
                for (int k = 0; k < 4; ++k) y[k] = ((keep >> k) & 1u) ? y[k] * inv_keep : 0.f;
            }
            store4(xn + 4 * i, y[0], y[1], y[2], y[3], nt);
#pragma unroll
            for (int k = 0; k < 4; ++k) m = max(m, __float_as_uint(y[k]) & 0x7fffffffu);
            if (sl >= 0) {
                float4 t = racc[wave][sl][c4[v]];
                t.x += y[0]; t.y += y[1]; t.z += y[2]; t.w += y[3];
                racc[wave][sl][c4[v]] = t;
            }
        }
    };
    int64_t r = r1 - 1 - wave;
    for (; r - 4 >= r0; r -= 8) {
        row(r);
        row(r - 4);
    }
    if (r >= r0) row(r);
    if (amax) block_amax(amax, m);
    __syncthreads();
    float4* dst = reinterpret_cast<float4*>(rpart + (int64_t)lb * kRangeSlots * H);
    for (int c = threadIdx.x; c < kRangeSlots * H4; c += 256) {
        const int q = c / H4, cc = c % H4;
        const float4 a0 = racc[0][q][cc], a1 = racc[1][q][cc], a2 = racc[2][q][cc], a3 = racc[3][q][cc];
        dst[c] = make_float4((a0.x + a1.x) + (a2.x + a3.x), (a0.y + a1.y) + (a2.y + a3.y),
                             (a0.z + a1.z) + (a2.z + a3.z), (a0.w + a1.w) + (a2.w + a3.w));
    }
}

__global__ __launch_bounds__(256) void k_sage_bwd_stats(const float* __restrict__ g,
                                                        const int64_t* __restrict__ g_rows,
                                                        const float* __restrict__ o,
                                                        const float* __restrict__ scale,
                                                        const float* __restrict__ shift,
                                                        const float* __restrict__ mean,
                                                        const float* __restrict__ invstd, uint32_t thr,
                                                        float inv_keep, uint64_t seed, int64_t n_rows, int H,
                                                        int64_t rows_per_block, float* __restrict__ part) {
    __shared__ __attribute__((aligned(16))) float red[2][2][512];
    const int H4 = H / 4;
    const int rpi = 256 / H4;
    const int t = threadIdx.x;
    const int c4 = t % H4, ph = t / H4;
    const int lb = xcd_remap(blockIdx.x, gridDim.x);
    const int64_t r0 = (int64_t)lb * rows_per_block;
    const int64_t r1 = min(n_rows, r0 + rows_per_block);
    float s0[4] = {0, 0, 0, 0}, s1[4] = {0, 0, 0, 0};
    const int c = c4 * 4;
    if (ph < rpi) {
        const float4 sc = *reinterpret_cast<const float4*>(scale + c);
        const float4 sh = *reinterpret_cast<const float4*>(shift + c);
        const float4 mu = *reinterpret_cast<const float4*>(mean + c);
        const float4 is = *reinterpret_cast<const float4*>(invstd + c);
        const float scv[4] = {sc.x, sc.y, sc.z, sc.w}, shv[4] = {sh.x, sh.y, sh.z, sh.w};
        const float muv[4] = {mu.x, mu.y, mu.z, mu.w}, isv[4] = {is.x, is.y, is.z, is.w};
        for (int64_t r = r0 + ph; r < r1; r += rpi) {
            const int64_t i4 = r * H4 + c4;
            const float4 gv = reinterpret_cast<const float4*>(g)[(g_rows ? g_rows[r] : r) * H4 + c4];
            const float4 ov = reinterpret_cast<const float4*>(o)[i4];
            float gg[4] = {gv.x, gv.y, gv.z, gv.w}, oo[4] = {ov.x, ov.y, ov.z, ov.w};
            uint32_t m = 0xF;
            if (thr) m = keep_bits4(seed, (uint64_t)i4, thr);
#pragma unroll
            for (int k = 0; k < 4; ++k) {
                float g1 = ((m >> k) & 1u) ? gg[k] * (thr ? inv_keep : 1.f) : 0.f;
                const float yp = oo[k] * scv[k] + shv[k];
                const float g2 = yp > 0.f ? g1 : 0.f;
                const float xh = (oo[k] - muv[k]) * isv[k];
                s0[k] += g2;
                s1[k] += g2 * xh;
            }
        }
    }
    __shared__ __attribute__((aligned(16))) float red_all[256][8];
#pragma unroll
    for (int k = 0; k < 4; ++k) { red_all[t][k] = s0[k]; red_all[t][4 + k] = s1[k]; }
    __syncthreads();
    (void)red;
    if (t < H4) {
        float a0[4] = {0, 0, 0, 0}, a1[4] = {0, 0, 0, 0};
        for (int q = 0; q < rpi; ++q)
#pragma unroll
            for (int k = 0; k < 4; ++k) {
                a0[k] += red_all[q * H4 + t][k];
                a1[k] += red_all[q * H4 + t][4 + k];
            }
        float* dst = part + (int64_t)lb * 2 * H;
        *reinterpret_cast<float4*>(dst + c) = make_float4(a0[0], a0[1], a0[2], a0[3]);
        *reinterpret_cast<float4*>(dst + H + c) = make_float4(a1[0], a1[1], a1[2], a1[3]);
    }
}

template <int NV, bool RELU = true, bool RANGES = false>
__global__ __launch_bounds__(256) __attribute__((amdgpu_waves_per_eu(4))) void k_sage_bwd_rows(
    const float* __restrict__ g, const int64_t* __restrict__ g_rows, const float* __restrict__ o,
    const float* __restrict__ nrm, const float* __restrict__ scale, const float* __restrict__ shift, const float* __restrict__ gamma,
    const float* __restrict__ mean, const float* __restrict__ invstd, const float* __restrict__ sum_g2,
    const float* __restrict__ sum_g2xhat, uint32_t thr, float inv_keep, uint64_t seed, int skip,
    int64_t n_rows, int H, int64_t rows_per_block, float* __restrict__ dh, int64_t lddh,
    float* __restrict__ gskip, float* __restrict__ part, uint32_t* __restrict__ amax, int nt,
    const int32_t* __restrict__ w_rowptr, int w_mode, int rev, const int32_t* __restrict__ ranges,
    const int32_t* __restrict__ rw_rowptr, float* __restrict__ rpart) {
    const int lane = threadIdx.x & 63;
    uint32_t tmax = 0;
    const int wave = __builtin_amdgcn_readfirstlane(threadIdx.x >> 6);
    const int lb = xcd_remap(blockIdx.x, gridDim.x);
    const int64_t r0 = (int64_t)lb * rows_per_block;
    const int64_t r1 = min(n_rows, r0 + rows_per_block);
    const int H4 = H / 4;
    const bool bn = (mean != nullptr);
    const float invn = 1.f / (float)(n_rows > 0 ? n_rows : 1);
    int cpos[NV];
    bool cok[NV];
#pragma unroll
    for (int v = 0; v < NV; ++v) {
        cpos[v] = (lane + 64 * v) * 4;
        cok[v] = cpos[v] < H;
    }
    __shared__ __attribute__((aligned(16))) float cst[7][512];
    for (int c = threadIdx.x; c < H; c += 256) {
        cst[0][c] = scale ? scale[c] : 1.f;
        cst[1][c] = shift ? shift[c] : 0.f;
        if (bn) {
            const float gi = (gamma ? gamma[c] : 1.f) * invstd[c];
            cst[2][c] = gi;
            cst[3][c] = gi * sum_g2[c] * invn;
            cst[4][c] = gi * sum_g2xhat[c] * invn;
            cst[5][c] = mean[c];
            cst[6][c] = invstd[c];
        } else {
            cst[2][c] = 1.f; cst[3][c] = 0.f; cst[4][c] = 0.f; cst[5][c] = 0.f; cst[6][c] = 0.f;
        }
    }
    __syncthreads();
    float db[NV][4], dw[NV][4];
#pragma unroll
    for (int v = 0; v < NV; ++v)
#pragma unroll
        for (int k = 0; k < 4; ++k) db[v][k] = dw[v][k] = 0.f;
    __shared__ __attribute__((aligned(16))) float red[4][RANGES ? kRangeSlots : 2][512];
    BlockRanges br;
    if constexpr (RANGES) {
        br.load(ranges, r0, r1);
#pragma unroll
        for (int q = 0; q < kRangeSlots; ++q)
#pragma unroll
            for (int v = 0; v < NV; ++v)
                if (cok[v]) *reinterpret_cast<float4*>(&red[wave][q][cpos[v]]) = make_float4(0.f, 0.f, 0.f, 0.f);
    }

    float4 gn[NV], on[NV];
    auto fetch = [&](int64_t rr) {
        const int64_t gr = g_rows ? g_rows[rr] : rr;
#pragma unroll
        for (int v = 0; v < NV; ++v) {
            const int64_t i4 = rr * H4 + (cok[v] ? (cpos[v] >> 2) : 0);
            gn[v] = reinterpret_cast<const float4*>(g)[gr * H4 + (cok[v] ? (cpos[v] >> 2) : 0)];
            on[v] = reinterpret_cast<const float4*>(o)[i4];
        }
    };
    const int64_t nr = r1 - r0 - wave;
    const int64_t cnt = nr > 0 ? (nr + 3) / 4 : 0;
    const int64_t rfirst = rev ? r1 - 1 - wave : r0 + wave;
    const int64_t rstep = rev ? -4 : 4;
    if (cnt > 0) fetch(rfirst);
    for (int64_t j = 0; j < cnt; ++j) {
        const int64_t r = rfirst + j * rstep;
        float ov[NV][4], dov[NV][4], g1v[NV][4];
        float4 gc[NV], oc[NV];
#pragma unroll
        for (int v = 0; v < NV; ++v) { gc[v] = gn[v]; oc[v] = on[v]; }
        if (j + 1 < cnt) fetch(r + rstep);
        float dot = 0.f;
#pragma unroll
        for (int v = 0; v < NV; ++v) {
            if (!cok[v]) {
#pragma unroll
                for (int k = 0; k < 4; ++k) ov[v][k] = dov[v][k] = g1v[v][k] = 0.f;
                continue;
            }
// ... 220 lines not shown
    for (int k = 0; k < 8; ++k) red[t][k] = acc[k];
    __syncthreads();
    if (t < C8) {
        float s8[8];
#pragma unroll
        for (int k = 0; k < 8; ++k) s8[k] = red[t][k];
        for (int q = 1; q < rpi; ++q)
#pragma unroll
            for (int k = 0; k < 8; ++k) s8[k] += red[t + q * C8][k];
        float4* dst = reinterpret_cast<float4*>(part + (int64_t)blockIdx.x * 2 * (8 * C8)) + 2 * t;
        dst[0] = make_float4(s8[0], s8[1], s8[2], s8[3]);
        dst[1] = make_float4(s8[4], s8[5], s8[6], s8[7]);
    }
}

extern "C" int bgnn_linear_bwd_prep_bf16(const void* g, const void* y, int64_t N, int32_t C, void* g_out,
                                         float* partial, void* stream) {
    BGNN_REQUIRE(g && partial && N >= 0, "linear_bwd_prep_bf16: null pointer or negative size");
    BGNN_REQUIRE(y == nullptr || g_out != nullptr, "linear_bwd_prep_bf16: a ReLU mask needs g_out");
    BGNN_REQUIRE(C >= 8 && C <= 2048 && C % 8 == 0 && (256 % (C / 8)) == 0,
                 "linear_bwd_prep_bf16: C = %d must be 8 * a power of two <= 2048", C);
    BGNN_REQUIRE((((uintptr_t)g | (uintptr_t)(g_out ? g_out : g) | (uintptr_t)partial | (uintptr_t)(y ? y : g)) & 15) == 0,
                 "linear_bwd_prep_bf16: pointers must be 16-B aligned");
    hipStream_t s = as_stream(stream);
    hipLaunchKernelGGL(k_linear_bwd_prep_bf16, dim3(kPrepBlocks), dim3(256), 0, s, reinterpret_cast<const uint4*>(g),
                       reinterpret_cast<const uint4*>(y), N, C / 8, reinterpret_cast<uint4*>(g_out), partial);
    BGNN_CHECK_LAUNCH();
    return BGNN_OK;
}

extern "C" int32_t bgnn_linear_bwd_prep_slots(void) { return kPrepBlocks; }

extern "C" int bgnn_linear_bwd_prep(const float* g, const float* y, int64_t N, int32_t C, float* g_out,
                                    float* partial, float* amax, void* stream) {
    BGNN_REQUIRE(g && partial && amax && N >= 0, "linear_bwd_prep: null pointer or negative size");
    BGNN_REQUIRE(y == nullptr || g_out != nullptr, "linear_bwd_prep: a ReLU mask needs g_out");
    BGNN_REQUIRE(C >= 4 && C <= 1024 && C % 4 == 0 && (256 % (C / 4)) == 0,
                 "linear_bwd_prep: C = %d must be 4 * a power of two <= 1024", C);
    BGNN_REQUIRE((((uintptr_t)g | (uintptr_t)(g_out ? g_out : g) | (uintptr_t)partial | (uintptr_t)(y ? y : g)) & 15) == 0,
                 "linear_bwd_prep: pointers must be 16-B aligned");
    hipStream_t s = as_stream(stream);
    hipLaunchKernelGGL(k_linear_bwd_prep, dim3(kPrepBlocks), dim3(256), 0, s, reinterpret_cast<const float4*>(g),
                       reinterpret_cast<const float4*>(y), N, C / 4, reinterpret_cast<float4*>(g_out), partial,
                       reinterpret_cast<uint32_t*>(amax));
    BGNN_CHECK_LAUNCH();
    return BGNN_OK;
}

extern "C" int bgnn_reduce_partials(const float* partial, int32_t n_slots, int32_t H, float* out0, float* out1,
                                    int32_t accumulate, void* stream) {
    BGNN_REQUIRE(partial && H > 0 && n_slots >= 0, "reduce_partials: bad args");
    hipStream_t s = as_stream(stream);
    if (g_one_pass_reduce) {
        hipLaunchKernelGGL(k_reduce_slots<0>, dim3((H + 7) / 8), dim3(256), 0, s, partial, n_slots, H, out0, out1,
                           accumulate, (int64_t)0, nullptr, nullptr, 0.f, 0.f, nullptr, nullptr, nullptr, nullptr,
                           nullptr, nullptr, nullptr);
        BGNN_CHECK_LAUNCH();
        return BGNN_OK;
    }
    const int stride = slots_stage1(const_cast<float*>(partial), n_slots, H, s);
    BGNN_CHECK_LAUNCH();
    hipLaunchKernelGGL(k_reduce_partials, dim3((H + 63) / 64), dim3(256), 0, s, partial, n_slots, stride, H, out0,
                       out1, accumulate);
    BGNN_CHECK_LAUNCH();
    return BGNN_OK;
}

extern "C" int bgnn_bn_finalize(const float* bn_partial, int32_t n_slots, int32_t H, int64_t count,
                                const float* gamma, const float* beta, float eps, float momentum,
                                float* running_mean, float* running_var, float* mean, float* invstd, float* scale,
                                float* shift, void* stream) {
    BGNN_REQUIRE(bn_partial && H > 0 && count > 0 && mean && invstd && scale && shift, "bn_finalize: bad args");
    hipStream_t s = as_stream(stream);
    if (g_one_pass_reduce) {
        hipLaunchKernelGGL(k_reduce_slots<1>, dim3((H + 7) / 8), dim3(256), 0, s, bn_partial, n_slots, H, nullptr,
                           nullptr, 0, count, gamma, beta, eps, momentum, running_mean, running_var, mean, invstd,
                           scale, shift, nullptr);
        BGNN_CHECK_LAUNCH();
        return BGNN_OK;
    }
    const int stride = slots_stage1(const_cast<float*>(bn_partial), n_slots, H, s);
    BGNN_CHECK_LAUNCH();
    hipLaunchKernelGGL(k_bn_finalize, dim3((H + 63) / 64), dim3(256), 0, s, bn_partial, n_slots, stride, H, count,
                       gamma, beta, eps, momentum, running_mean, running_var, mean, invstd, scale, shift);
    BGNN_CHECK_LAUNCH();
    return BGNN_OK;
}

extern "C" int bgnn_bn_finalize_shifted(const float* bn_partial, int32_t n_slots, int32_t H, int64_t count,
                                        const float* kshift, const float* gamma, const float* beta, float eps,
                                        float momentum, float* running_mean, float* running_var, float* mean,
                                        float* invstd, float* scale, float* shift, void* stream) {
    BGNN_REQUIRE(bn_partial && kshift && H > 0 && count > 0 && mean && invstd && scale && shift,
                 "bn_finalize_shifted: bad args");
    hipLaunchKernelGGL(k_reduce_slots<1>, dim3((H + 7) / 8), dim3(256), 0, as_stream(stream), bn_partial, n_slots, H,
                       nullptr, nullptr, 0, count, gamma, beta, eps, momentum, running_mean, running_var, mean, invstd,
                       scale, shift, kshift);
    BGNN_CHECK_LAUNCH();
    return BGNN_OK;
}

extern "C" int bgnn_bn_eval_coeffs(int32_t H, const float* gamma, const float* beta, float eps,
                                   const float* running_mean, const float* running_var, float* scale, float* shift,
                                   void* stream) {
    BGNN_REQUIRE(H > 0 && running_mean && running_var && scale && shift, "bn_eval_coeffs: bad args");
    hipStream_t s = as_stream(stream);
    hipLaunchKernelGGL(k_bn_eval, dim3((H + 255) / 256), dim3(256), 0, s, H, gamma, beta, eps, running_mean,
                       running_var, scale, shift);
    BGNN_CHECK_LAUNCH();
    return BGNN_OK;
}

extern "C" int bgnn_sage_apply(const float* o, const float* scale, const float* shift, const float* x_prev,
                               int32_t skip, float p, uint64_t seed, int64_t n_rows, int32_t H, float* x_next,
                               float* amax, const int32_t* ranges, float* range_partial, void* stream) {
    BGNN_REQUIRE(H > 0 && H % 4 == 0, "sage_apply: H must be a multiple of 4");
    BGNN_REQUIRE(n_rows >= 0, "sage_apply: negative n_rows");
    BGNN_REQUIRE(n_rows == 0 || (o && x_next), "sage_apply: null o / x_next");
    BGNN_REQUIRE(p >= 0.f && p < 1.f, "sage_apply: dropout p must be in [0, 1)");
    BGNN_REQUIRE((scale == nullptr) == (shift == nullptr), "sage_apply: scale/shift must both be set or NULL");
    BGNN_REQUIRE(!skip || x_prev, "sage_apply: skip requires x_prev");
    BGNN_REQUIRE(al16(o) && al16(x_next) && (!x_prev || al16(x_prev)) && (!scale || (al16(scale) && al16(shift))),
                 "sage_apply: pointers must be 16-byte aligned");
    BGNN_REQUIRE(!ranges || (range_partial && ((uintptr_t)range_partial & 15) == 0 && H <= 512),
                 "sage_apply: ranges need a 16-B aligned range_partial and H <= 512");
    if (n_rows == 0) return BGNN_OK;
    hipStream_t s = as_stream(stream);
    if (ranges) {
        const uint32_t thr = dropout_threshold(p);
        const float inv_keep = thr ? 1.f / (1.f - p) : 1.f;
        int64_t rpb = 0;
        const int64_t blocks = rows_slots_of(n_rows, &rpb);
        if (H > 256)
            hipLaunchKernelGGL(k_sage_apply_rows<2>, dim3((unsigned)blocks), dim3(256), 0, s, o, scale, shift, x_prev,
                               skip, thr, inv_keep, seed, n_rows, H, rpb, x_next, reinterpret_cast<uint32_t*>(amax),
                               rows_nt(), ranges, range_partial);
        else
            hipLaunchKernelGGL(k_sage_apply_rows<1>, dim3((unsigned)blocks), dim3(256), 0, s, o, scale, shift, x_prev,
                               skip, thr, inv_keep, seed, n_rows, H, rpb, x_next, reinterpret_cast<uint32_t*>(amax),
                               rows_nt(), ranges, range_partial);
        BGNN_CHECK_LAUNCH();
        return BGNN_OK;
    }
    const int64_t n4 = n_rows * (H / 4);
    int64_t blocks = (n4 + 255) / 256;
    if (blocks > 4096) blocks = 4096;
    const int rev = (rows_rev() & 2) ? 1 : 0;
    if (rev) blocks = (blocks + 7) / 8 * 8;
    const uint32_t thr = dropout_threshold(p);
    const float inv_keep = thr ? 1.f / (1.f - p) : 1.f;
    hipLaunchKernelGGL(k_sage_apply, dim3((unsigned)blocks), dim3(256), 0, s, (const float4*)o, scale, shift,
                       (const float4*)x_prev, skip, thr, inv_keep, seed, n4, H / 4, (float4*)x_next,
                       reinterpret_cast<uint32_t*>(amax), rows_nt(), rev);
    BGNN_CHECK_LAUNCH();
    return BGNN_OK;
}

extern "C" int32_t bgnn_rows_slots(int64_t n_rows) {
    int64_t rpb = 0;
    return (int32_t)rows_grid(n_rows, 4, &rpb);
}

extern "C" int bgnn_sage_bwd_stats(const float* g, const int64_t* g_rows, const float* o, const float* scale,
                                   const float* shift,
                                   const float* mean, const float* invstd, float p, uint64_t seed, int64_t n_rows,
                                   int32_t H, float* partial2, void* stream) {
    BGNN_REQUIRE(H > 0 && H % 4 == 0 && H <= 1024, "sage_bwd_stats: H=%d unsupported", H);
    BGNN_REQUIRE(n_rows >= 0, "sage_bwd_stats: negative n_rows");
    BGNN_REQUIRE(g && o && scale && shift && mean && invstd && partial2, "sage_bwd_stats: null pointer");
    BGNN_REQUIRE(al16(g) && al16(o) && al16(scale) && al16(shift) && al16(mean) && al16(invstd) && al16(partial2),
                 "sage_bwd_stats: pointers must be 16-byte aligned");
    hipStream_t s = as_stream(stream);
    int64_t rpb = 0;
    const int64_t blocks = rows_grid(n_rows, 4, &rpb);
    const uint32_t thr = dropout_threshold(p);
    const float inv_keep = thr ? 1.f / (1.f - p) : 1.f;
    hipLaunchKernelGGL(k_sage_bwd_stats, dim3((unsigned)blocks), dim3(256), 0, s, g, g_rows, o, scale, shift, mean, invstd,
                       thr, inv_keep, seed, n_rows, H, rpb, partial2);
    BGNN_CHECK_LAUNCH();
    return BGNN_OK;
}

extern "C" int bgnn_sage_bwd_rows(const float* g, const int64_t* g_rows, const float* o, const float* nrm,
                                  const float* scale,
                                  const float* shift, const float* gamma, const float* mean, const float* invstd,
                                  const float* sum_g2, const float* sum_g2xhat, float p, uint64_t seed,
                                  int32_t skip, int64_t n_rows, int32_t H, float* dh, int64_t lddh, float* gskip,
                                  float* partial_db, float* amax, const int32_t* w_rowptr, int32_t w_mode,
                                  const int32_t* ranges, const int32_t* range_w_rowptr, float* range_partial,
                                  void* stream) {
    BGNN_REQUIRE(H > 0 && H % 4 == 0 && H <= 512, "sage_bwd_rows: H=%d unsupported", H);
    BGNN_REQUIRE(n_rows >= 0, "sage_bwd_rows: negative n_rows");
    BGNN_REQUIRE(g && o && nrm && dh && partial_db, "sage_bwd_rows: null pointer");
    BGNN_REQUIRE(w_mode >= 0 && w_mode <= 2 && (w_mode == 0 || w_rowptr), "sage_bwd_rows: bad row weights");
    BGNN_REQUIRE(lddh >= H && lddh % 4 == 0, "sage_bwd_rows: bad lddh");
    BGNN_REQUIRE(!skip || gskip, "sage_bwd_rows: skip requires gskip");
    BGNN_REQUIRE(!mean || (invstd && sum_g2 && sum_g2xhat), "sage_bwd_rows: BN stats incomplete");
    BGNN_REQUIRE(al16(g) && al16(o) && al16(dh) && (!gskip || al16(gskip)) && al16(partial_db),
                 "sage_bwd_rows: pointers must be 16-byte aligned");
    BGNN_REQUIRE(!ranges || (range_partial && al16(range_partial)), "sage_bwd_rows: ranges need range_partial");
    hipStream_t s = as_stream(stream);
    int64_t rpb = 0;
    const int64_t blocks = rows_grid(n_rows, 4, &rpb);
    const uint32_t thr = dropout_threshold(p);
    const float inv_keep = thr ? 1.f / (1.f - p) : 1.f;
#define BGNN_ROWS(NV, R)                                                                                              \
    hipLaunchKernelGGL((k_sage_bwd_rows<NV, true, R>), dim3((unsigned)blocks), dim3(256), 0, s, g, g_rows, o, nrm,   \
                       scale,                                                                                       \
                       shift, gamma, mean, invstd, sum_g2, sum_g2xhat, thr, inv_keep, seed, skip, n_rows, H, rpb,    \
                       dh, lddh, gskip, partial_db, reinterpret_cast<uint32_t*>(amax), rows_nt(), w_rowptr, w_mode,  \
                       rows_rev() & 1, ranges, range_w_rowptr, range_partial)
    if (ranges) {
        if (H > 256) BGNN_ROWS(2, true);
        else BGNN_ROWS(1, true);
    } else {
        if (H > 256) BGNN_ROWS(2, false);
        else BGNN_ROWS(1, false);
    }
#undef BGNN_ROWS
    BGNN_CHECK_LAUNCH();
    return BGNN_OK;
}

extern "C" int bgnn_l2norm_bwd(const float* g, const float* o, const float* nrm, int64_t n_rows, int32_t H,
                               float* dh, int64_t lddh, float* partial_db, float* amax, void* stream) {
    BGNN_REQUIRE(H > 0 && H % 4 == 0 && H <= 512, "l2norm_bwd: H=%d unsupported", H);
    BGNN_REQUIRE(n_rows >= 0, "l2norm_bwd: negative n_rows");
    BGNN_REQUIRE(g && o && nrm && dh && partial_db && amax, "l2norm_bwd: null pointer");
    BGNN_REQUIRE(lddh >= H && lddh % 4 == 0, "l2norm_bwd: bad lddh");
    BGNN_REQUIRE(al16(g) && al16(o) && al16(dh) && al16(partial_db), "l2norm_bwd: pointers must be 16-byte aligned");
    hipStream_t s = as_stream(stream);
    int64_t rpb = 0;
    const int64_t blocks = rows_grid(n_rows, 4, &rpb);
    if (H > 256)
        hipLaunchKernelGGL((k_sage_bwd_rows<2, false>), dim3((unsigned)blocks), dim3(256), 0, s, g, nullptr, o, nrm, nullptr,
                           nullptr, nullptr, nullptr, nullptr, nullptr, nullptr, 0u, 1.f, (uint64_t)0, 0, n_rows, H,
                           rpb, dh, lddh, nullptr, partial_db, reinterpret_cast<uint32_t*>(amax), rows_nt(), nullptr,
                           0, rows_rev() & 1, nullptr, nullptr, nullptr);
    else
        hipLaunchKernelGGL((k_sage_bwd_rows<1, false>), dim3((unsigned)blocks), dim3(256), 0, s, g, nullptr, o, nrm, nullptr,
                           nullptr, nullptr, nullptr, nullptr, nullptr, nullptr, 0u, 1.f, (uint64_t)0, 0, n_rows, H,
                           rpb, dh, lddh, nullptr, partial_db, reinterpret_cast<uint32_t*>(amax), rows_nt(), nullptr,
                           0, rows_rev() & 1, nullptr, nullptr, nullptr);
    BGNN_CHECK_LAUNCH();
    return BGNN_OK;
}
```

### buck-gnn_amd/csrc/spmm.hip

```cpp
#include <vector>

#include "common.h"
#include "gemm_common.h"
#include "seg_common.h"

namespace bgnn {

enum : int { OP_SUM = 0, OP_MEAN = 1, OP_MAX = 2, OP_MEANT = 3, OP_MAXT = 4 };
enum : int { EPI_PLAIN = 0, EPI_SAGE = 1 };

struct SegArgs {
    const int32_t* rowptr;
    const int32_t* col;
    const int32_t* heavy_row;
    const int32_t* heavy_chunk0;
    const int32_t* chunk_heavy;
    int64_t n_rows;
    int32_t n_heavy, n_chunks, chunk;
    int32_t H;
    int64_t rows_per_block;
    const float* x;     int64_t ldx;
    float* out;         int64_t ldo;
    uint8_t* arg8;
    int32_t* heavy_of;
// ... 908 lines not shown
static bool g_heavy_on = false;
static int g_heavy_dir = 0;

inline HeavyEv* heavy_ev_next(int fwd) {
    if (!g_heavy_on) return nullptr;
    if (g_heavy_used == g_heavy_ev.size()) {
        HeavyEv e{};
        if (hipEventCreateWithFlags(&e.a, hipEventDisableSystemFence) != hipSuccess ||
            hipEventCreateWithFlags(&e.b, hipEventDisableSystemFence) != hipSuccess)
            return nullptr;
        g_heavy_ev.push_back(e);
    }
    HeavyEv* e = &g_heavy_ev[g_heavy_used++];
    e->fwd = fwd;
    return e;
}

inline bool use_group(const SegArgs& A, int op, int vec, int lpr) {
    return g_seg_kernel == 0 && A.gcnt != nullptr && vec == 4 && lpr == 64 && A.chunk <= 64 &&
           (op == OP_SUM || op == OP_MEAN || op == OP_MEANT);
}

inline int64_t light_blocks_sage(const SegArgs& A) {
    return use_group(A, OP_SUM, 4, 64) ? group_grid(A.n_groups) : sweep_grid(A.n_rows);
}

template <int VEC, int NV, int LPR, int OP, int EPI>
int launch_all(SegArgs A, int ctiles, int max_blocks, hipStream_t s, int64_t* blocks_out) {
    int64_t rpb = 0;
    const bool group = use_group(A, OP, VEC, LPR) && ctiles == 1;
    const bool sweep = (VEC == 4 && LPR == 64 && g_seg_kernel != 1 && A.chunk <= 64);
    int64_t blocks;
    if (group) {
        blocks = group_grid(A.n_groups);
    } else if (sweep || EPI == EPI_SAGE) {
        blocks = sweep_grid(A.n_rows);
        rpb = (A.n_rows + blocks - 1) / blocks;
    } else {
        blocks = light_grid(A.n_rows, kWave / LPR, max_blocks, &rpb);
    }
    A.rows_per_block = rpb;
    A.nt = g_seg_nt;
    A.rev = (rows_rev() >> (EPI == EPI_SAGE ? 2 : 3)) & 1;
    if (blocks_out) *blocks_out = blocks;
    A.light_slots = (int32_t)blocks;
    if (A.n_rows > 0) {
        if constexpr (VEC == 4 && LPR == 64 && (OP == OP_SUM || OP == OP_MEAN || OP == OP_MEANT)) {
            if (group) {
                const dim3 gr((unsigned)blocks);
                if (A.group_rows == 8)
                    hipLaunchKernelGGL((k_seg_group<NV, OP, EPI, 8, 4>), gr, dim3(256), 0, s, A);
                else
                    hipLaunchKernelGGL((k_seg_group<NV, OP, EPI, 4, 8>), gr, dim3(256), 0, s, A);
                BGNN_CHECK_LAUNCH();
            }
        }
        if (group) {
        } else if constexpr (VEC == 4 && LPR == 64) {
            if (sweep) {
                const int u = g_seg_u ? g_seg_u : 12;
                if (u == 8)
                    hipLaunchKernelGGL((k_seg_sweep<NV, OP, EPI, 8>), dim3((unsigned)blocks, ctiles), dim3(256), 0,
                                       s, A);
                else if (u == 16)
                    hipLaunchKernelGGL((k_seg_sweep<NV, OP, EPI, 16>), dim3((unsigned)blocks, ctiles), dim3(256), 0,
                                       s, A);
                else
                    hipLaunchKernelGGL((k_seg_sweep<NV, OP, EPI, 12>), dim3((unsigned)blocks, ctiles), dim3(256), 0,
                                       s, A);
            } else {
                hipLaunchKernelGGL((k_seg_light<VEC, NV, LPR, OP, EPI>), dim3((unsigned)blocks, ctiles), dim3(256),
                                   0, s, A);
            }
        } else {
            hipLaunchKernelGGL((k_seg_light<VEC, NV, LPR, OP, EPI>), dim3((unsigned)blocks, ctiles), dim3(256), 0,
                               s, A);
        }
        BGNN_CHECK_LAUNCH();
    }
    if (A.n_chunks > 0) {
        HeavyEv* ev = heavy_ev_next(g_heavy_dir == 0);
        if (ev) (void)hipEventRecord(ev->a, s);
        const bool all_range = A.ranges_all && A.hfirst && (A.hagg || A.hdone);
        constexpr int COP = (OP == OP_MAX) ? OP_MAX : (OP == OP_MAXT ? OP_MAXT : (OP == OP_MEANT ? OP_MEANT : OP_SUM));
        if (!all_range) {
            hipLaunchKernelGGL((k_seg_chunk<VEC, NV, LPR, COP>), dim3((A.n_chunks + 3) / 4, ctiles), dim3(256), 0, s,
                               A);
            BGNN_CHECK_LAUNCH();
        }
        constexpr int MOP = (OP == OP_MAX) ? OP_MAX : (OP == OP_MEAN ? OP_MEAN : OP_SUM);
        if (!(all_range && A.hdone)) {
            hipLaunchKernelGGL((k_seg_combine<VEC, NV, LPR, MOP, EPI>), dim3(A.n_heavy, ctiles),
                               dim3(MOP == OP_MAX ? 256 : 64 * kCombineWaves), 0, s, A);
            BGNN_CHECK_LAUNCH();
        }
        if (ev) (void)hipEventRecord(ev->b, s);
    }
    return BGNN_OK;
}

template <int OP>
int dispatch_plain(SegArgs A, const Geometry& g, hipStream_t s) {
#define BGNN_PLAIN(V, N, L)                                                              \
    if (g.vec == V && g.nv == N && g.lpr == L)                                           \
        return launch_all<V, N, L, OP, EPI_PLAIN>(A, g.ctiles, 2048, s, nullptr);
    BGNN_PLAIN(4, 2, 64)
    BGNN_PLAIN(4, 1, 64)
    BGNN_PLAIN(4, 1, 32)
    BGNN_PLAIN(4, 1, 16)
    BGNN_PLAIN(1, 1, 64)
    BGNN_PLAIN(1, 1, 32)
    BGNN_PLAIN(1, 1, 16)
#undef BGNN_PLAIN
    return fail(BGNN_E_UNSUPPORTED, "spmm: no kernel for vec=%d nv=%d lpr=%d", g.vec, g.nv, g.lpr);
}


inline SegArgs args_from_csr(const bgnn_csr_t* c) {
    SegArgs A{};
    A.rowptr = c->rowptr;
    A.col = c->col;
    A.heavy_row = c->heavy_row;
    A.heavy_chunk0 = c->heavy_chunk0;
    A.chunk_heavy = c->chunk_heavy;
    A.n_rows = c->n_rows;
    A.n_heavy = c->n_heavy;
    A.n_chunks = c->n_chunks;
    A.chunk = c->chunk > 0 ? c->chunk : 0x7fffffff;
    if (c->gsrc && c->gmask && c->gcnt && (c->group_rows == 4 || c->group_rows == 8)) {
        A.gsrc = c->gsrc;
        A.gmask = c->gmask;
        A.gcnt = c->gcnt;
        A.group_rows = c->group_rows;
        A.grow = c->grow;
        A.n_groups = c->grow ? c->n_groups : (c->n_rows + c->group_rows - 1) / c->group_rows;
    }
    if (c->ranges && c->n_heavy > 0) {
        A.hfirst = c->ranges + 2 + 3 * c->n_heavy;
        A.ranges_all = c->ranges_all;
    }
    return A;
}

inline int check_plain(const char* name, const char* xn, const char* on, const bgnn_csr_t* c, const void* x,
                       const void* out) {
    BGNN_REQUIRE(c->n_rows >= 0, "%s: negative n_rows", name);
    BGNN_REQUIRE(c->n_rows == 0 || (x && out), "%s: null %s / %s", name, xn, on);
    BGNN_REQUIRE(c->nnz <= 0 || c->col, "%s: null col", name);
    BGNN_REQUIRE(c->n_chunks <= 0 || (c->heavy_row && c->heavy_chunk0 && c->chunk_heavy),
                 "%s: heavy rows need the CSR's chunk plan", name);
    return BGNN_OK;
}

extern int g_x6_bdma;
extern int g_h3p_nsb;
#ifdef BGNN_H3P_ABLATION
extern int g_h3p_abl;
#endif

}

using namespace bgnn;

extern "C" int bgnn_spmm_fwd(const bgnn_csr_t* csr, const float* x, int64_t ldx, int32_t H, int32_t reduce,
                             float* out, int64_t ldo, void* arg, float* partial, void* stream) {
    BGNN_REQUIRE(csr && csr->rowptr, "spmm_fwd: null csr");
    BGNN_REQUIRE(H > 0 && ldx >= H && ldo >= H, "spmm_fwd: bad H/ld");
    BGNN_REQUIRE(reduce >= 0 && reduce <= 2, "spmm_fwd: bad reduce %d", reduce);
    BGNN_REQUIRE(csr->n_chunks == 0 || partial, "spmm_fwd: partial scratch required for heavy rows");
    if (const int rc = check_plain("spmm_fwd", "x", "out", csr, x, out)) return rc;
    SegArgs A = args_from_csr(csr);
    g_heavy_dir = 0;
    A.H = H;
    A.x = x; A.ldx = ldx;
    A.out = out; A.ldo = ldo;
    if (arg) {
        BGNN_REQUIRE(csr->chunk > 0 && csr->chunk < 255,
                     "spmm_fwd(max, arg): the CSR's chunk must be in [1, 254] for the compact argmax (got %d)",
                     csr->chunk);
        const MaxArgLayout L = max_arg_layout(csr->n_rows, H);
        A.arg8 = static_cast<uint8_t*>(arg);
        A.heavy_of = reinterpret_cast<int32_t*>(static_cast<char*>(arg) + L.heavy_of);
        A.arg_h = reinterpret_cast<int32_t*>(static_cast<char*>(arg) + L.arg_h);
    }
    if (csr->n_rows == 0) return BGNN_OK;
    A.partial = partial;
    A.partial_arg = partial ? reinterpret_cast<int32_t*>(partial + (int64_t)csr->n_chunks * H) : nullptr;
    const bool al = aligned16(x) && aligned16(out) && ldx % 4 == 0 && ldo % 4 == 0 &&
                    (!partial || aligned16(partial)) && (!arg || aligned16(arg));
    const Geometry g = pick_geometry(H, al);
    hipStream_t s = as_stream(stream);
    switch (reduce) {
        case BGNN_REDUCE_SUM: return dispatch_plain<OP_SUM>(A, g, s);
        case BGNN_REDUCE_MEAN: return dispatch_plain<OP_MEAN>(A, g, s);
        default: return dispatch_plain<OP_MAX>(A, g, s);
    }
}

static int spmm_bwd_impl(const bgnn_csr_t* csr_t, const int32_t* perm_t, const int32_t* fwd_rowptr,
                         int64_t fwd_rows, const float* g, int64_t ldg, int32_t H, int32_t reduce, const void* arg,
                         const float* addend, int64_t ld_add, float* gx, int64_t ldgx, float* partial, float* amax,
                         int heavy_done, void* stream);

extern "C" int bgnn_spmm_bwd(const bgnn_csr_t* csr_t, const int32_t* perm_t, const int32_t* fwd_rowptr,
                             const float* g, int64_t ldg, int32_t H, int32_t reduce, float* gx, int64_t ldgx,
                             float* partial, float* amax, int32_t heavy_done, void* stream) {
    BGNN_REQUIRE(reduce != BGNN_REDUCE_MAX, "spmm_bwd: max aggregation takes bgnn_spmm_bwd_max");
    BGNN_REQUIRE(!heavy_done || (csr_t && csr_t->ranges), "spmm_bwd: heavy_done needs the CSR's ranges");
    return spmm_bwd_impl(csr_t, perm_t, fwd_rowptr, 0, g, ldg, H, reduce, nullptr, nullptr, 0, gx, ldgx, partial,
                         amax, heavy_done ? 1 : 0, stream);
}

extern "C" int bgnn_spmm_bwd_add(const bgnn_csr_t* csr_t, const int32_t* perm_t, const int32_t* fwd_rowptr,
                                 const float* g, int64_t ldg, int32_t H, int32_t reduce, const float* addend,
                                 int64_t ld_add, float* gx, int64_t ldgx, float* partial, float* amax, void* stream) {
    BGNN_REQUIRE(reduce != BGNN_REDUCE_MAX, "spmm_bwd_add: max aggregation takes bgnn_spmm_bwd_max");
    return spmm_bwd_impl(csr_t, perm_t, fwd_rowptr, 0, g, ldg, H, reduce, nullptr, addend, ld_add, gx, ldgx, partial,
                         amax, 0, stream);
}

extern "C" int bgnn_spmm_bwd_max(const bgnn_csr_t* csr_t, const int32_t* perm_t, const int32_t* fwd_rowptr,
                                 int64_t fwd_rows, const float* g, int64_t ldg, int32_t H, const void* arg,
                                 const float* addend, int64_t ld_add, float* gx, int64_t ldgx, float* partial,
                                 float* amax, void* stream) {
    BGNN_REQUIRE(perm_t && fwd_rowptr && arg && fwd_rows >= 0, "spmm_bwd_max: perm_t, fwd_rowptr and arg required");
    return spmm_bwd_impl(csr_t, perm_t, fwd_rowptr, fwd_rows, g, ldg, H, BGNN_REDUCE_MAX, arg, addend, ld_add, gx, ldgx,
                         partial, amax, 0, stream);
}

static int spmm_bwd_impl(const bgnn_csr_t* csr_t, const int32_t* perm_t, const int32_t* fwd_rowptr,
                         int64_t fwd_rows, const float* g, int64_t ldg, int32_t H, int32_t reduce, const void* arg,
                         const float* addend, int64_t ld_add, float* gx, int64_t ldgx, float* partial, float* amax,
                         int heavy_done, void* stream) {
    BGNN_REQUIRE(csr_t && csr_t->rowptr, "spmm_bwd: null csr");
    BGNN_REQUIRE(!addend || ld_add >= H, "spmm_bwd: bad ld_add");
    BGNN_REQUIRE(H > 0 && ldg >= H && ldgx >= H, "spmm_bwd: bad H/ld");
    BGNN_REQUIRE(csr_t->n_chunks == 0 || partial, "spmm_bwd: partial scratch required");
    if (const int rc = check_plain("spmm_bwd", "g", "gx", csr_t, g, gx)) return rc;
    BGNN_REQUIRE(reduce != BGNN_REDUCE_MEAN || fwd_rowptr, "spmm_bwd(mean): fwd_rowptr required");
    BGNN_REQUIRE(reduce == BGNN_REDUCE_SUM || reduce == BGNN_REDUCE_MEAN || (perm_t && arg && fwd_rowptr),
                 "spmm_bwd(max): perm_t, fwd_rowptr and arg required");
    if (csr_t->n_rows == 0) return BGNN_OK;
    SegArgs A = args_from_csr(csr_t);
    g_heavy_dir = 1;
    A.H = H;
    A.x = g; A.ldx = ldg;
    A.out = gx; A.ldo = ldgx;
    A.partial = partial;
    A.fwd_rowptr = fwd_rowptr;
    A.perm_t = perm_t;
    if (arg) {
        const MaxArgLayout L = max_arg_layout(fwd_rows, H);
        A.arg8_in = static_cast<const uint8_t*>(arg);
        A.heavy_of_in = reinterpret_cast<const int32_t*>(static_cast<const char*>(arg) + L.heavy_of);
        A.arg_h_in = reinterpret_cast<const int32_t*>(static_cast<const char*>(arg) + L.arg_h);
    }
    A.amax = reinterpret_cast<uint32_t*>(amax);
    A.add = addend;
    A.ld_add = ld_add;
    A.hdone = heavy_done;
    const bool al = aligned16(g) && aligned16(gx) && ldg % 4 == 0 && ldgx % 4 == 0 &&
                    (!partial || aligned16(partial)) && (!arg || aligned16(arg)) &&
                    (!addend || (aligned16(addend) && ld_add % 4 == 0));
    const Geometry geo = pick_geometry(H, al);
    hipStream_t s = as_stream(stream);
    switch (reduce) {
        case BGNN_REDUCE_SUM: return dispatch_plain<OP_SUM>(A, geo, s);
        case BGNN_REDUCE_MEAN: return dispatch_plain<OP_MEANT>(A, geo, s);
        default: return dispatch_plain<OP_MAXT>(A, geo, s);
    }
}

extern "C" int32_t bgnn_sage_fwd_slots(const bgnn_csr_t* csr) {
    if (!csr) return -1;
    const SegArgs A = args_from_csr(csr);
    return (int32_t)(light_blocks_sage(A) + (csr->n_chunks > 0 ? csr->n_heavy : 0));
}

extern "C" int32_t bgnn_get_tuning(int32_t knob) {
    switch (knob) {
        case BGNN_TUNE_SEG_KERNEL: return g_seg_kernel;
        case BGNN_TUNE_SEG_BLOCKS: return g_seg_blocks;
        case BGNN_TUNE_SEG_U: return g_seg_u;
        case BGNN_TUNE_SEG_NT: return g_seg_nt;
        case BGNN_TUNE_GEMM_MODE: return gemm_mode();
        case BGNN_TUNE_ROWS_NT: return rows_nt();
        case BGNN_TUNE_GROUP_BLOCKS: return g_grp_blocks;
        case BGNN_TUNE_ROWS_REV: return rows_rev();
        case BGNN_TUNE_GEMM_BDMA: return g_x6_bdma == 2 && g_h3p_nsb == 4 ? 3 : g_x6_bdma;
        default: return -1;
    }
}

extern "C" int bgnn_set_tuning(int32_t knob, int32_t value) {
    switch (knob) {
        case BGNN_TUNE_SEG_KERNEL:
            BGNN_REQUIRE(value >= 0 && value <= 2, "set_tuning: kernel must be 0 (auto), 1 (blocked) or 2 (sweep)");
            g_seg_kernel = value;
            return BGNN_OK;
        case BGNN_TUNE_SEG_BLOCKS:
            BGNN_REQUIRE(value >= 8 && value <= 65536, "set_tuning: blocks out of range");
            g_seg_blocks = value;
            return BGNN_OK;
        case BGNN_TUNE_SEG_U:
            BGNN_REQUIRE(value == 0 || value == 8 || value == 12 || value == 16,
                         "set_tuning: U must be 0 (auto), 8, 12 or 16");
// ... 105 lines not shown
```

### include/bgnn.h

```cpp
#ifndef BGNN_H
#define BGNN_H

#include <stddef.h>
#include <stdint.h>

#ifdef __cplusplus
extern "C" {
#endif

#define BGNN_ABI_VERSION 17

#define BGNN_OK 0
#define BGNN_E_ARG 1001
#define BGNN_E_WS 1002
#define BGNN_E_UNSUPPORTED 1003

#define BGNN_REDUCE_SUM 0
#define BGNN_REDUCE_MEAN 1
#define BGNN_REDUCE_MAX 2

int bgnn_abi_version(void);
const char* bgnn_last_error_string(void);

#define BGNN_TUNE_SEG_KERNEL 1
#define BGNN_TUNE_SEG_BLOCKS 2
#define BGNN_TUNE_SEG_U 3
#define BGNN_TUNE_SEG_NT 4
#define BGNN_TUNE_GEMM_MODE 5
#define BGNN_TUNE_ROWS_NT 6
#define BGNN_TUNE_GROUP_BLOCKS 7
#define BGNN_TUNE_ROWS_REV 13
#define BGNN_TUNE_GEMM_BDMA 16
int bgnn_heavy_timing(int32_t enable);
int bgnn_heavy_timing_read(int32_t which, float* total_ms, int32_t* count);
int32_t bgnn_get_tuning(int32_t knob);
int bgnn_set_tuning(int32_t knob, int32_t value);

typedef struct bgnn_csr {
    const int32_t* rowptr;
    const int32_t* col;
    const int32_t* heavy_row;
    const int32_t* heavy_chunk0;
    const int32_t* chunk_heavy;
    int64_t n_rows;
    int64_t nnz;
    int32_t n_heavy;
    int32_t n_chunks;
    int32_t chunk;
    int32_t ranges_all;
    const int32_t* gsrc;
    const uint8_t* gmask;
    const int32_t* gcnt;
    const int32_t* grow;
    int64_t n_groups;
    int32_t group_rows;
    int32_t _pad2;
    const int32_t* ranges;
} bgnn_csr_t;

size_t bgnn_graph_build_ws_bytes(int64_t num_edges, int64_t num_nodes);

int bgnn_graph_build(const int64_t* edge_index, int64_t num_edges, int64_t num_nodes,
                     int32_t* rowptr, int32_t* col,
                     int32_t* rowptr_t, int32_t* col_t, int32_t* perm_t,
                     void* ws, size_t ws_bytes, int32_t* dev_status, void* stream);

int bgnn_index_csr_build(const int64_t* index, int64_t n, int64_t num_rows,
                         int32_t* rowptr, int32_t* col,
                         void* ws, size_t ws_bytes, int32_t* dev_status, void* stream);

size_t bgnn_heavy_plan_ws_bytes(int64_t n_rows);
int bgnn_heavy_plan(const int32_t* rowptr, int64_t n_rows, int64_t nnz, int32_t chunk,
                    int32_t* heavy_row, int32_t* heavy_chunk0, int32_t* chunk_heavy,
                    int32_t* dev_counts, void* ws, size_t ws_bytes, void* stream);

size_t bgnn_heavy_ranges_bytes(int32_t n_heavy);
int bgnn_heavy_ranges(const bgnn_csr_t* csr, int32_t* ranges, void* stream);

size_t bgnn_range_partial_bytes(int64_t n_rows, int32_t H);
int bgnn_range_sums_finish(const float* range_partial, int64_t n_rows, int32_t H, const bgnn_csr_t* csr,
                           int32_t mode, float* out, int64_t ldo, const float* amax_floor, float* amax,
                           void* stream);

int bgnn_group_plan(const int32_t* rowptr, const int32_t* col, int64_t n_rows, int32_t chunk,
                    int32_t group_rows, const int32_t* grow, int64_t n_groups,
                    int32_t* gsrc, uint8_t* gmask, int32_t* gcnt, void* stream);

int bgnn_spmm_fwd(const bgnn_csr_t* csr, const float* x, int64_t ldx, int32_t H,
                  int32_t reduce, float* out, int64_t ldo, void* arg,
                  float* partial, void* stream);
size_t bgnn_spmm_max_arg_bytes(int64_t n_rows, int32_t H, int32_t n_heavy);

int bgnn_spmm_bwd(const bgnn_csr_t* csr_t, const int32_t* perm_t, const int32_t* fwd_rowptr,
                  const float* g, int64_t ldg, int32_t H, int32_t reduce,
                  float* gx, int64_t ldgx, float* partial, float* amax, int32_t heavy_done, void* stream);
int bgnn_spmm_bwd_add(const bgnn_csr_t* csr_t, const int32_t* perm_t, const int32_t* fwd_rowptr,
                      const float* g, int64_t ldg, int32_t H, int32_t reduce,
                      const float* addend, int64_t ld_add, float* gx, int64_t ldgx, float* partial,
                      float* amax, void* stream);
int bgnn_spmm_bwd_max(const bgnn_csr_t* csr_t, const int32_t* perm_t, const int32_t* fwd_rowptr,
                      int64_t fwd_rows, const float* g, int64_t ldg, int32_t H, const void* arg,
                      const float* addend, int64_t ld_add, float* gx, int64_t ldgx, float* partial,
                      float* amax, void* stream);

int32_t bgnn_sage_fwd_slots(const bgnn_csr_t* csr);
int bgnn_sage_fwd(const bgnn_csr_t* csr, const float* zl, int64_t ldzl, const float* zr, int64_t ldzr,
                  const float* bias, int32_t H, int32_t reduce, float* o, float* nrm,
                  float* bn_partial, float* partial, const float* heavy_agg, int64_t ld_heavy_agg,
                  void* stream);

int bgnn_bn_finalize(const float* bn_partial, int32_t n_slots, int32_t H, int64_t count,
                     const float* gamma, const float* beta, float eps, float momentum,
                     float* running_mean, float* running_var,
                     float* mean, float* invstd, float* scale, float* shift, void* stream);
int bgnn_bn_eval_coeffs(int32_t H, const float* gamma, const float* beta, float eps,
                        const float* running_mean, const float* running_var,
                        float* scale, float* shift, void* stream);

int bgnn_sage_apply(const float* o, const float* scale, const float* shift,
                    const float* x_prev, int32_t skip, float p, uint64_t seed,
                    int64_t n_rows, int32_t H, float* x_next, float* amax,
                    const int32_t* ranges, float* range_partial, void* stream);

int bgnn_sage_infer_bf16(const bgnn_csr_t* csr, const void* z, int64_t ldz, const float* bias,
                         const float* scale, const float* shift, const void* x_prev, int64_t ldx,
                         int32_t H, int32_t reduce, void* out, int64_t ldo, int32_t out_f32,
                         float* partial, void* stream);

int bgnn_spmm_fwd_bf16(const bgnn_csr_t* csr, const void* x, int64_t ldx, int32_t H, int32_t reduce,
                       void* out, int64_t ldo, int32_t out_f32, float* partial, void* stream);
int bgnn_spmm_bwd_bf16(const bgnn_csr_t* csr_t, const int32_t* fwd_rowptr, const void* g, int64_t ldg,
                       int32_t H, int32_t reduce, void* gx, int64_t ldgx, int32_t out_f32,
                       float* partial, void* stream);

int bgnn_spmm_max_bf16(const bgnn_csr_t* csr, const void* x, int64_t ldx, int32_t H,
                       void* out, int64_t ldo, void* arg, float* partial, void* stream);

int bgnn_sage_tail_bf16(const void* y, int64_t ldy, const float* bias, const float* scale,
                        const float* shift, const void* x_prev, int64_t ldx, int64_t n_rows,
                        int32_t H, void* out, int64_t ldo, int32_t out_f32, void* stream);

int32_t bgnn_rows_slots(int64_t n_rows);
int bgnn_sage_bwd_stats(const float* g, const int64_t* g_rows, const float* o, const float* scale,
                        const float* shift,
                        const float* mean, const float* invstd, float p, uint64_t seed,
                        int64_t n_rows, int32_t H, float* partial2, void* stream);

int32_t bgnn_linear_bwd_prep_slots(void);
int bgnn_linear_bwd_prep(const float* g, const float* y, int64_t N, int32_t C, float* g_out,
                         float* partial, float* amax, void* stream);
int bgnn_linear_bwd_prep_bf16(const void* g, const void* y, int64_t N, int32_t C, void* g_out,
                              float* partial, void* stream);
int bgnn_reduce_partials(const float* partial, int32_t n_slots, int32_t H,
                         float* out0, float* out1, int32_t accumulate, void* stream);

int bgnn_sage_bwd_rows(const float* g, const int64_t* g_rows, const float* o, const float* nrm,
                       const float* scale, const float* shift, const float* gamma,
                       const float* mean, const float* invstd,
                       const float* sum_g2, const float* sum_g2xhat,
                       float p, uint64_t seed, int32_t skip,
                       int64_t n_rows, int32_t H, float* dh, int64_t lddh,
                       float* gskip, float* partial_db, float* amax,
                       const int32_t* w_rowptr, int32_t w_mode, const int32_t* ranges,
                       const int32_t* range_w_rowptr, float* range_partial, void* stream);

int bgnn_l2norm_bwd(const float* g, const float* o, const float* nrm, int64_t n_rows, int32_t H,
                    float* dh, int64_t lddh, float* partial_db, float* amax, void* stream);

int bgnn_gemm_bf16(int32_t trans_a, int32_t trans_b, int64_t M, int64_t N, int64_t K, float alpha,
                   const void* A, int64_t lda, const void* B, int64_t ldb, float beta, void* C, int64_t ldc,
                   const float* bias, int32_t relu, int32_t storage, void* ws, size_t ws_bytes, void* stream);
int bgnn_gemm_gather_add_bf16(int64_t M, int64_t N, int64_t K, const void* A, int64_t lda, const void* B,
                              int64_t ldb, void* C, int64_t ldc, const float* bias, int32_t relu,
                              const float* add0, const int64_t* idx0, int64_t ld0, const float* add1,
                              const int64_t* idx1, int64_t ld1, int32_t storage, void* ws, size_t ws_bytes,
                              void* stream);
int bgnn_gemm_b16_variant(int32_t variant);
int bgnn_add_dropout_bf16(const void* a, const void* b, int64_t n, float p, uint64_t seed, void* out,
                          void* stream);
int bgnn_add_dropped_bf16(const void* a, const void* b, int64_t n, float p, uint64_t seed, void* out,
                          void* stream);
int bgnn_gemm_bf16_dropadd(int64_t M, int64_t N, int64_t K, const void* A, int64_t lda, const void* B,
                           int64_t ldb, void* C, int64_t ldc, const void* src, int64_t ld_src, float p,
                           uint64_t seed, void* stream);
int bgnn_segment_sum_bf16(const int32_t* rowptr, const int32_t* col, int64_t n_rows, const void* x,
                          int64_t ldx, int32_t H, int32_t mean, float* out, int64_t ldo, void* stream);
int bgnn_segment_bcast_bf16(const int32_t* rowptr, const int32_t* col, int64_t n_rows, const float* g, int64_t ldg,
                            int32_t H, int32_t mean, void* out, int64_t ldo, void* stream);

size_t bgnn_gemm_ws_bytes(int64_t M, int64_t N, int64_t K, int32_t trans_a, int32_t trans_b);
int bgnn_gemm_set_cfg(int32_t cfg);
int bgnn_gemm_f32(int32_t trans_a, int32_t trans_b, int64_t M, int64_t N, int64_t K,
                  float alpha, const float* A, int64_t lda, const float* B, int64_t ldb,
                  float beta, float* C, int64_t ldc, void* ws, size_t ws_bytes, void* stream);
int bgnn_gemm_f32_ex(int32_t trans_a, int32_t trans_b, int64_t M, int64_t N, int64_t K,
                     float alpha, const float* A, int64_t lda, const float* B, int64_t ldb,
                     float beta, float* C, int64_t ldc, const float* bias, int32_t relu,
                     void* ws, size_t ws_bytes, void* stream);
int bgnn_gemm_f32_scaled(int32_t trans_a, int32_t trans_b, int64_t M, int64_t N, int64_t K,
                         float alpha, const float* A, int64_t lda, int64_t a_blk, int64_t a_pstride,
                         const float* B, int64_t ldb, float beta, float* C, int64_t ldc,
                         int64_t c_blk, int64_t c_pstride, const float* bias, int32_t relu,
                         const float* a_amax, const float* b_amax, float* c_amax,
                         int32_t precision, void* ws, size_t ws_bytes, void* stream);
int bgnn_gemm_f32_dropadd(int32_t trans_a, int32_t trans_b, int64_t M, int64_t N, int64_t K,
                          const float* A, int64_t lda, const float* B, int64_t ldb, float* C, int64_t ldc,
                          const float* a_amax, const float* b_amax, const float* src, int64_t ld_src,
                          float p, uint64_t seed, void* ws, size_t ws_bytes, void* stream);
int bgnn_gemm_f32_dropadd_cols(int64_t M, int64_t N, int64_t K, const float* A, int64_t lda, const float* B,
                               int64_t ldb, float* C, int64_t ldc, const float* a_amax, const float* b_amax,
                               const float* src, int64_t ld_src, int64_t src_col0, float p, uint64_t seed, void* ws,
                               size_t ws_bytes, void* stream);
int32_t bgnn_gemm_w_tile(int64_t M, int64_t N, int64_t K);
size_t bgnn_gemm_wsplit_bytes(int64_t N, int64_t K);
int bgnn_gemm_wsplit(const float* W, int32_t n_items, int64_t item_stride, int64_t N, int64_t K, int64_t ldw,
                     const float* amax, int64_t amax_stride, void* img, int64_t img_stride, int32_t bn,
                     void* stream);
int bgnn_gemm_f32_w(int64_t M, int64_t N, int64_t K, const float* A, int64_t lda, const void* wimg, int32_t bn,
                    float* C, int64_t ldc, const float* bias, int32_t relu, const float* a_amax,
                    const float* b_amax, float* c_amax, const float* src, int64_t ld_src, float p, uint64_t seed,
                    void* stream);
size_t bgnn_gemm_ws_bytes_ex(int64_t M, int64_t N, int64_t K, int32_t trans_a, int32_t trans_b,
                             int32_t precision);
int bgnn_gemm_gather_add(int32_t trans_a, int32_t trans_b, int64_t M, int64_t N, int64_t K,
                         const float* A, int64_t lda, const float* B, int64_t ldb, float* C, int64_t ldc,
                         const float* bias, int32_t relu, const float* add0, const int64_t* idx0, int64_t ld0,
                         const float* add1, const int64_t* idx1, int64_t ld1, int32_t precision,
                         void* ws, size_t ws_bytes, void* stream);
int bgnn_absmax_f32(const float* x, int64_t rows, int64_t cols, int64_t ld, float* out,
                    int32_t accumulate, void* stream);
int bgnn_absmax_items_f32(const float* x, int32_t n_items, int64_t item_stride, int64_t rows, int64_t cols,
                          int64_t ld, float* out, int64_t out_stride, void* stream);
int32_t bgnn_fold_weights_supported(int64_t H, int64_t K_in);
size_t bgnn_fold_weights_ws_bytes(int64_t H, int64_t K_in);
int bgnn_fold_weights_fwd(int64_t H, int64_t K_in, const float* wcat, int64_t ld_wcat, const float* w_in,
                          int64_t ld_win, const float* b_in, float* fold_amax, float* wf, int64_t ld_wf,
                          float* bf, float* wf_t, int64_t ld_wft, float* w_amax, void* stream);
int bgnn_fold_weights_bwd(int64_t H, int64_t K_in, const float* dwf, int64_t ld_dwf, const float* dbf,
                          const float* wcat, int64_t ld_wcat, const float* w_in, int64_t ld_win,
                          const float* b_in, float* fold_amax, float* dwcat, int64_t ld_dwcat, float* dw_in,
                          int64_t ld_dwin, float* db_in, void* ws, size_t ws_bytes, void* stream);
int bgnn_gemm_f32_planes(int32_t trans_a, int32_t trans_b, int64_t M, int64_t N, int64_t K,
                         float alpha, const float* A, int64_t lda, int64_t a_blk, int64_t a_pstride,
                         const float* B, int64_t ldb, float beta, float* C, int64_t ldc,
                         int64_t c_blk, int64_t c_pstride, const float* bias, int32_t relu,
                         void* ws, size_t ws_bytes, void* stream);

int bgnn_store_gather_graph(const int64_t* table, int32_t B, int64_t Nb, int64_t Eb,
                            int64_t max_nodes, int64_t max_edges,
                            const int32_t* edge_index, int64_t ld_ei,
                            const int32_t* rowptr, const int32_t* col,
                            const int32_t* rowptr_t, const int32_t* col_t, const int32_t* perm_t,
                            int64_t* edge_index_out, int32_t* rowptr_out, int32_t* col_out,
                            int32_t* rowptr_t_out, int32_t* col_t_out, int32_t* perm_t_out,
                            int64_t* batch_out, void* stream);
int bgnn_store_gather_groups(const int64_t* gtable, int32_t B, int32_t group_rows, int64_t Nb, int64_t Gb,
                             int64_t max_edges, int64_t max_groups,
                             const int32_t* gsrc, const uint8_t* gmask, const int32_t* gcnt,
                             const int32_t* gsrc_t, const uint8_t* gmask_t, const int32_t* gcnt_t,
                             int32_t* gsrc_out, uint8_t* gmask_out, int32_t* gcnt_out,
                             int32_t* gsrc_t_out, uint8_t* gmask_t_out, int32_t* gcnt_t_out,
                             int32_t* grow_out, void* stream);
int bgnn_store_gather_rows(const int64_t* table, int32_t B, int32_t per_edge, int64_t max_rows,
                           const void* src, int64_t row_bytes, void* dst, void* stream);

int bgnn_topk_rank(const float* score, const int64_t* batch, const int64_t* ptr, int64_t n,
                   int32_t* rank, void* stream);
int bgnn_topk_select(const int32_t* rank, const int64_t* batch, const int64_t* k, const int64_t* new_ptr,
                     int64_t n, int64_t* perm, int32_t* new_id, int64_t* batch_out, void* stream);
int bgnn_gather_scale(const float* x, int64_t ldx, int32_t H, const int64_t* perm, const float* score,
                      int64_t k, float* out, int64_t ldo, void* stream);
int bgnn_gather_scale_bwd(const float* g, int64_t ldg, const float* x, int64_t ldx, int32_t H,
                          const int32_t* new_id, const float* score, int64_t n, float* dx, int64_t lddx,
                          float* dscore, void* stream);
size_t bgnn_filter_edges_ws_bytes(int64_t num_edges);
// ... 41 lines not shown
```

Measured before the change: 2167.

## Fuse last-layer BN/ReLU/dropout apply with global mean pooling

In the final SAGE layer, the elementwise apply (BN scale/shift, ReLU, skip, dropout) and the global mean pool become a single segment-walking kernel, with a combine pass for heavy segments. When the caller does not need the per-node output, x_next is never written, which saves a full N×H write and its re-read by a separate pool SpMM. The backward pool-gradient degree division also moves into a small custom kernel, replacing a chain of torch ops. In exchange the last layer reads rows through the pool's column indices instead of linearly, and the path falls back to the old one on argument errors.

```diff
diff --git a/buck-gnn_amd/bgnn/_lib.py b/buck-gnn_amd/bgnn/_lib.py
--- a/buck-gnn_amd/bgnn/_lib.py
+++ b/buck-gnn_amd/bgnn/_lib.py
@@ -6,7 +6,7 @@
 
 _HERE = os.path.dirname(os.path.abspath(__file__))
 LIB_PATH = os.environ.get("BGNN_LIBRARY") or os.path.join(_HERE, "_lib", "libbgnn.so")
-ABI_VERSION = 17
+ABI_VERSION = 18
 
 _lock = threading.Lock()
 _lib = None
@@ -93,6 +93,9 @@
                                  c_p]),
     "bgnn_bn_eval_coeffs": (c_i32, [c_i32, c_p, c_p, c_f32, c_p, c_p, c_p, c_p, c_p]),
     "bgnn_sage_apply": (c_i32, [c_p, c_p, c_p, c_p, c_i32, c_f32, c_u64, c_i64, c_i32, c_p, c_p, c_p, c_p, c_p]),
+    "bgnn_sage_apply_pool": (c_i32, [c_p, c_p, c_p, c_p, c_i32, c_f32, c_u64, c_i64, c_i32, c_p, c_p,
+                                     ctypes.POINTER(CsrStruct), c_i32, c_p, c_p, c_p]),
+    "bgnn_pool_grad_scale": (c_i32, [c_p, c_p, c_i64, c_i32, c_p, c_p]),
     "bgnn_sage_infer_bf16": (c_i32, [ctypes.POINTER(CsrStruct), c_p, c_i64, c_p, c_p, c_p, c_p, c_i64, c_i32, c_i32,
                                      c_p, c_i64, c_i32, c_p, c_p]),
     "bgnn_spmm_fwd_bf16": (c_i32, [ctypes.POINTER(CsrStruct), c_p, c_i64, c_i32, c_i32, c_p, c_i64, c_i32, c_p, c_p]),
diff --git a/buck-gnn_amd/bgnn/buckgnn.py b/buck-gnn_amd/bgnn/buckgnn.py
--- a/buck-gnn_amd/bgnn/buckgnn.py
+++ b/buck-gnn_amd/bgnn/buckgnn.py
@@ -286,7 +286,7 @@
                                  skip, p, self.training, self._seed(), x_amax=amax, return_amax=True,
                                  amax_buf=bufs[i], w_in=None if fold is None else fold.weight,
                                  b_in=None if fold is None else fold.bias, wprep=wprep[i], count_batch=False,
-                                 fold_amax=fold_amax, rng=rng, pool=pl)
+                                 fold_amax=fold_amax, rng=rng, pool=pl, need_x=pl is None)
                 x, amax = out[0], out[1]
                 x_full = rng.holder[0] if (rng is not None and rng.holder) else None
             if pool is not None:
diff --git a/buck-gnn_amd/bgnn/fused.py b/buck-gnn_amd/bgnn/fused.py
--- a/buck-gnn_amd/bgnn/fused.py
+++ b/buck-gnn_amd/bgnn/fused.py
@@ -508,8 +508,11 @@
         self.rng = None
 
 
+_E_ARG = 1001
+
+
 def _glue_fwd(o, bn_part, slots, x_prev, gamma, beta, running_mean, running_var, cfg: LayerConfig, next_amax,
-              graph: Graph = None):
+              graph: Graph = None, pool=None, need_x: bool = True):
     N, H = o.shape
     dev = o.device
     s = _stream()
@@ -540,11 +543,25 @@
         _lib.call("bgnn_range_sums_finish", rp.data_ptr(), N, H, graph.fwd.ref(), 0, full[N:].data_ptr(), H,
                   next_amax.data_ptr(), rng.out_amax.data_ptr(), s)
         rng.holder.append(full)
-        return x_next, (scale, shift, mean, invstd)
+        return x_next, (scale, shift, mean, invstd), None
+    if pool is not None and N > 0 and pool.n == N:
+        x_next = torch.empty(N, H, dtype=torch.float32, device=dev) if need_x else None
+        pooled = torch.empty(pool.num_rows, H, dtype=torch.float32, device=dev)
+        nch = pool.fwd.plan.n_chunks
+        part = torch.empty(nch * H, dtype=torch.float32, device=dev) if nch else None
+        try:
+            _lib.call("bgnn_sage_apply_pool", o.data_ptr(), _ptr(scale), _ptr(shift), x_prev.data_ptr(),
+                      int(cfg.skip), float(cfg.p), cfg.seed, N, H, _ptr(x_next),
+                      next_amax.data_ptr() if need_x else None,
+                      pool.fwd.ref(), 1, _ptr(part), pooled.data_ptr(), s)
+            return x_next, (scale, shift, mean, invstd), pooled
+        except _lib.BgnnError as e:
+            if e.code != _E_ARG:
+                raise
     x_next = torch.empty(N, H, dtype=torch.float32, device=dev)
     _lib.call("bgnn_sage_apply", o.data_ptr(), _ptr(scale), _ptr(shift), x_prev.data_ptr(), int(cfg.skip),
               float(cfg.p), cfg.seed, N, H, x_next.data_ptr(), next_amax.data_ptr(), None, None, s)
-    return x_next, (scale, shift, mean, invstd)
+    return x_next, (scale, shift, mean, invstd), None
 
 
 def _glue_bwd_stats(g, o, scale, shift, mean, invstd, cfg: LayerConfig, g_rows=None):
@@ -576,7 +593,7 @@
 
     @staticmethod
     def forward(ctx, x_prev, x_amax, w_l, b_l, w_r, gamma, beta, running_mean, running_var, graph: Graph,
-                cfg: LayerConfig, amax=None, w_in=None, b_in=None, wprep=None, pool=None):
+                cfg: LayerConfig, amax=None, w_in=None, b_in=None, wprep=None, pool=None, need_x: bool = True):
         dev = x_prev.device
         x_prev = x_prev.contiguous()
         H = w_l.size(0)
@@ -663,8 +680,8 @@
                       cfg.reduce, o.data_ptr(), nrm.data_ptr(), bn_part.data_ptr(), _ptr(part), _ptr(hagg),
                       2 * H if hagg is not None else 0, s)
         del z, zl, zr, hagg
-        x_next, (scale, shift, mean, invstd) = _glue_fwd(o, bn_part, slots, x_prev, gamma, beta, running_mean,
-                                                         running_var, cfg, next_amax, graph)
+        x_next, (scale, shift, mean, invstd), pooled = _glue_fwd(o, bn_part, slots, x_prev, gamma, beta, running_mean,
+                                                                 running_var, cfg, next_amax, graph, pool, need_x)
         ctx.graph = graph
         ctx.cfg = cfg
         ctx.folded = folded
@@ -681,9 +698,10 @@
         ctx.mark_non_differentiable(next_amax)
         ctx.pool = pool
         if pool is not None:
-            from .ops import spmm_fwd
-            pooled, _ = spmm_fwd(pool.fwd, x_next, 1, pool.num_rows)
-            return x_next, next_amax, pooled
+            if pooled is None:
+                from .ops import spmm_fwd
+                pooled, _ = spmm_fwd(pool.fwd, x_next, 1, pool.num_rows)
+            return (x_next if need_x else None), next_amax, pooled
         return x_next, next_amax
 
     @staticmethod
@@ -692,14 +710,17 @@
         g_rows = None
         if g_pool is not None:
             seg = ctx.pool
-            gp = g_pool.contiguous() / seg.fwd.degree().clamp_min(1).to(g_pool.dtype).unsqueeze(1)
+            gpc = g_pool.contiguous()
+            gp = torch.empty_like(gpc)
+            _lib.call("bgnn_pool_grad_scale", gpc.data_ptr(), seg.fwd.rowptr.data_ptr(), gpc.size(0), gpc.size(1),
+                      gp.data_ptr(), _stream())
             if g is None and not cfg.skip:
                 g, g_rows = gp, seg.index
             else:
                 gb = gp.index_select(0, seg.index)
                 g = gb if g is None else g + gb
         if g is None:
-            return (None,) * 16
+            return (None,) * 17
         x_prev, o, nrm, wcat, gamma, scale, shift, mean, invstd, x_amax, w_amax, dz_amax = ctx.saved_tensors
         graph: Graph = ctx.graph
         g = g.contiguous()
@@ -782,7 +803,7 @@
                 db_in = gemm(wcat, dbf.view(-1, 1), trans_a=True, trans_b=False, a_amax=fa[0],
                              b_amax=fa[4]).view(-1)
             return (dx, None, dw[:H], db, dw[H:], dgamma if has_affine else None, dbeta if has_affine else None,
-                    None, None, None, None, None, dw_in, db_in, None, None)
+                    None, None, None, None, None, dw_in, db_in, None, None, None)
         wcat_t = (ctx.wcat_t if ctx.wcat_t is not None else wcat.t().contiguous()) if DGRAD_WT else wcat
         img_d = ctx.img_d if (not planes and DGRAD_WT) else None
         if (img_d is not None and (dropadd or gskip is None)
@@ -813,7 +834,7 @@
             dw = gemm(dz, x_prev, trans_a=True, trans_b=False, a_amax=dz_amax, b_amax=x_amax)
         dw_l, dw_r = dw[:H], dw[H:]
         return (dx, None, dw_l, db, dw_r, dgamma if has_affine else None, dbeta if has_affine else None,
-                None, None, None, None, None, None, None, None, None)
+                None, None, None, None, None, None, None, None, None, None)
 
 
 def _max_transform(x, w_l, w_r, graph: Graph, x_amax, w_amax, name: str):
@@ -935,8 +956,8 @@
         with _timed("sage_fwd"):
             o, nrm, bn_part, slots = _max_rows_fwd(y, b_l, H)
         del y
-        x_next, (scale, shift, mean, invstd) = _glue_fwd(o, bn_part, slots, x_prev, gamma, beta, running_mean,
-                                                         running_var, cfg, next_amax)
+        x_next, (scale, shift, mean, invstd), _ = _glue_fwd(o, bn_part, slots, x_prev, gamma, beta, running_mean,
+                                                            running_var, cfg, next_amax)
         ctx.graph = graph
         ctx.cfg = cfg
         ctx.set_materialize_grads(False)
@@ -1062,7 +1083,7 @@
                bn_module, graph: Graph, reduce: int, skip: bool, p: float, training: bool,
                seed: int, x_amax: torch.Tensor = None, return_amax: bool = False, amax_buf=None,
                w_in: torch.Tensor = None, b_in: torch.Tensor = None, wprep=None, count_batch: bool = True,
-               fold_amax: torch.Tensor = None, rng: RangeRows = None, pool=None):
+               fold_amax: torch.Tensor = None, rng: RangeRows = None, pool=None, need_x: bool = True):
     require_cuda(x_prev, w_l, b_l, w_r, what="sage_layer")
     _require_f32(x_prev, "sage_layer")
     H = w_l.size(0)
@@ -1095,7 +1116,7 @@
         else:
             out = SageLayerFn.apply(x_prev, x_amax, w_l, b_l, w_r, bn_module.weight, bn_module.bias,
                                     bn_module.running_mean, bn_module.running_var, graph, cfg, amax_buf, w_in, b_in,
-                                    wprep, pool)
+                                    wprep, pool, need_x)
     else:
         cfg = LayerConfig(reduce, False, training, 0.0, 0.0, skip, p, seed)
         cfg.famax = fold_amax if w_in is not None else None
@@ -1105,7 +1126,7 @@
                                        wprep)
         else:
             out = SageLayerFn.apply(x_prev, x_amax, w_l, b_l, w_r, None, None, None, None, graph, cfg, amax_buf,
-                                    w_in, b_in, wprep, pool)
+                                    w_in, b_in, wprep, pool, need_x)
     if pool is not None:
         return out if return_amax else (out[0], out[2])
     return out if return_amax else out[0]
diff --git a/buck-gnn_amd/csrc/common.h b/buck-gnn_amd/csrc/common.h
--- a/buck-gnn_amd/csrc/common.h
+++ b/buck-gnn_amd/csrc/common.h
@@ -82,6 +82,7 @@
 int rows_nt();
 void set_rows_rev(int on);
 int rows_rev();
+int seg_combine_plain(const bgnn_csr_t* csr, int32_t H, int32_t reduce, float* partial, float* out, hipStream_t s);
 
 __device__ __forceinline__ void store4(float* p, float a, float b, float c, float d, bool nt) {
     typedef float f32x4_t __attribute__((ext_vector_type(4)));
diff --git a/buck-gnn_amd/csrc/sage.hip b/buck-gnn_amd/csrc/sage.hip
--- a/buck-gnn_amd/csrc/sage.hip
+++ b/buck-gnn_amd/csrc/sage.hip
@@ -1,5 +1,6 @@
 #include "common.h"
 #include "ranges.h"
+#include "seg_common.h"
 
 namespace bgnn {
 
@@ -189,6 +190,24 @@
     }
 }
 
+__device__ __forceinline__ void x_next4(float (&y)[4], bool bn, const float4& sc, const float4& sh, bool skip,
+                                        const float4& p, uint32_t thr, float inv_keep, uint64_t seed, uint64_t i) {
+    if (bn) {
+        y[0] = y[0] * sc.x + sh.x; y[1] = y[1] * sc.y + sh.y;
+        y[2] = y[2] * sc.z + sh.z; y[3] = y[3] * sc.w + sh.w;
+    }
+#pragma unroll
+    for (int k = 0; k < 4; ++k) y[k] = fmaxf(y[k], 0.f);
+    if (skip) {
+        y[0] += p.x; y[1] += p.y; y[2] += p.z; y[3] += p.w;
+    }
+    if (thr) {
+        const uint32_t keep = keep_bits4(seed, i, thr);
+#pragma unroll
+        for (int k = 0; k < 4; ++k) y[k] = ((keep >> k) & 1u) ? y[k] * inv_keep : 0.f;
+    }
+}
+
 __global__ __launch_bounds__(256) void k_sage_apply(const float4* __restrict__ o, const float* __restrict__ scale,
                                                     const float* __restrict__ shift,
                                                     const float4* __restrict__ xprev, int skip, uint32_t thr,
@@ -209,23 +228,14 @@
         const int c = (int)(i % H4) * 4;
         float4 v = o[i];
         float y[4] = {v.x, v.y, v.z, v.w};
+        float4 sc = make_float4(1.f, 1.f, 1.f, 1.f), sh = make_float4(0.f, 0.f, 0.f, 0.f);
+        float4 p = make_float4(0.f, 0.f, 0.f, 0.f);
         if (scale) {
-            const float4 sc = *reinterpret_cast<const float4*>(scale + c);
-            const float4 sh = *reinterpret_cast<const float4*>(shift + c);
-            y[0] = y[0] * sc.x + sh.x; y[1] = y[1] * sc.y + sh.y;
-            y[2] = y[2] * sc.z + sh.z; y[3] = y[3] * sc.w + sh.w;
-        }
-#pragma unroll
-        for (int k = 0; k < 4; ++k) y[k] = fmaxf(y[k], 0.f);
-        if (skip) {
-            const float4 p = xprev[i];
-            y[0] += p.x; y[1] += p.y; y[2] += p.z; y[3] += p.w;
-        }
-        if (thr) {
-            const uint32_t keep = keep_bits4(seed, (uint64_t)i, thr);
-#pragma unroll
-            for (int k = 0; k < 4; ++k) y[k] = ((keep >> k) & 1u) ? y[k] * inv_keep : 0.f;
-        }
+            sc = *reinterpret_cast<const float4*>(scale + c);
+            sh = *reinterpret_cast<const float4*>(shift + c);
+        }
+        if (skip) p = xprev[i];
+        x_next4(y, scale != nullptr, sc, sh, skip != 0, p, thr, inv_keep, seed, (uint64_t)i);
         store4(reinterpret_cast<float*>(xn + i), y[0], y[1], y[2], y[3], nt);
 #pragma unroll
         for (int k = 0; k < 4; ++k) m = max(m, __float_as_uint(y[k]) & 0x7fffffffu);
@@ -274,21 +284,9 @@
             const int64_t i = r * H4 + c4[v];
             const float4 ov = reinterpret_cast<const float4*>(o)[i];
             float y[4] = {ov.x, ov.y, ov.z, ov.w};
-            if (scale) {
-                y[0] = y[0] * sc[v].x + sh[v].x; y[1] = y[1] * sc[v].y + sh[v].y;
-                y[2] = y[2] * sc[v].z + sh[v].z; y[3] = y[3] * sc[v].w + sh[v].w;
-            }
-#pragma unroll
-            for (int k = 0; k < 4; ++k) y[k] = fmaxf(y[k], 0.f);
-            if (skip) {
-                const float4 p = reinterpret_cast<const float4*>(xprev)[i];
-                y[0] += p.x; y[1] += p.y; y[2] += p.z; y[3] += p.w;
-            }
-            if (thr) {
-                const uint32_t keep = keep_bits4(seed, (uint64_t)i, thr);
-#pragma unroll
-                for (int k = 0; k < 4; ++k) y[k] = ((keep >> k) & 1u) ? y[k] * inv_keep : 0.f;
-            }
+            float4 p = make_float4(0.f, 0.f, 0.f, 0.f);
+            if (skip) p = reinterpret_cast<const float4*>(xprev)[i];
+            x_next4(y, scale != nullptr, sc[v], sh[v], skip != 0, p, thr, inv_keep, seed, (uint64_t)i);
             store4(xn + 4 * i, y[0], y[1], y[2], y[3], nt);
 #pragma unroll
             for (int k = 0; k < 4; ++k) m = max(m, __float_as_uint(y[k]) & 0x7fffffffu);
@@ -314,6 +312,113 @@
         dst[c] = make_float4((a0.x + a1.x) + (a2.x + a3.x), (a0.y + a1.y) + (a2.y + a3.y),
                              (a0.z + a1.z) + (a2.z + a3.z), (a0.w + a1.w) + (a2.w + a3.w));
     }
+}
+
+struct ApplyPoolArgs {
+    const float* o;
+    const float* scale;
+    const float* shift;
+    const float* xprev;
+    uint32_t thr;
+    float inv_keep;
+    uint64_t seed;
+    int32_t H, nt;
+    float* xn;
+    uint32_t* amax;
+    const int32_t* rowptr;
+    const int32_t* col;
+    const int32_t* heavy_row;
+    const int32_t* heavy_chunk0;
+    const int32_t* chunk_heavy;
+    int32_t n_chunks, chunk, mean;
+    int32_t ct;
+    int64_t n_light;
+    float* partial;
+    float* out;
+};
+
+template <bool SKIP>
+__device__ __forceinline__ void apply_pool_batch(const ApplyPoolArgs& A, float (&acc)[4], uint32_t& m, int32_t e,
+                                                 int32_t nvalid, int c4, bool cok, const float4& sc,
+                                                 const float4& sh) {
+    constexpr int U = 8;
+    const int H4 = A.H / 4;
+    int64_t i[U];
+#pragma unroll
+    for (int u = 0; u < U; ++u) i[u] = (int64_t)A.col[e + (u < nvalid ? u : 0)] * H4 + c4;
+    float4 ov[U], pv[SKIP ? U : 1];
+#pragma unroll
+    for (int u = 0; u < U; ++u) {
+        ov[u] = reinterpret_cast<const float4*>(A.o)[i[u]];
+        if constexpr (SKIP) pv[u] = reinterpret_cast<const float4*>(A.xprev)[i[u]];
+    }
+#pragma unroll
+    for (int u = 0; u < U; ++u) {
+        const bool ok = cok && u < nvalid;
+        float y[4] = {ov[u].x, ov[u].y, ov[u].z, ov[u].w};
+        x_next4(y, A.scale != nullptr, sc, sh, SKIP, SKIP ? pv[u] : make_float4(0.f, 0.f, 0.f, 0.f), A.thr,
+                A.inv_keep, A.seed, (uint64_t)i[u]);
+        if (ok) {
+            if (A.xn) store4(A.xn + 4 * i[u], y[0], y[1], y[2], y[3], A.nt);
+#pragma unroll
+            for (int k = 0; k < 4; ++k) m = max(m, __float_as_uint(y[k]) & 0x7fffffffu);
+        }
+#pragma unroll
+        for (int k = 0; k < 4; ++k) acc[k] = __fadd_rn(acc[k], ok ? y[k] : 0.f);
+    }
+}
+
+template <bool SKIP>
+__global__ __launch_bounds__(256) void k_sage_apply_pool(ApplyPoolArgs A) {
+    const int lane = threadIdx.x & 63;
+    const int wave = __builtin_amdgcn_readfirstlane(threadIdx.x >> 6);
+    const int H4 = A.H / 4;
+    const int tile = blockIdx.y * A.ct + wave % A.ct;
+    const int64_t w = (int64_t)blockIdx.x * (4 / A.ct) + wave / A.ct;
+    bool live = tile * 64 < H4;
+    int32_t beg = 0, end = 0;
+    int64_t seg = -1;
+    if (live && w < A.n_chunks) {
+        const int32_t h = A.chunk_heavy[w];
+        const int32_t r = A.heavy_row[h];
+        const int32_t k = (int32_t)(w - A.heavy_chunk0[h]);
+        beg = A.rowptr[r] + k * A.chunk;
+        end = min(beg + A.chunk, A.rowptr[r + 1]);
+    } else if (live) {
+        seg = w - A.n_chunks;
+        live = seg < A.n_light;
+        if (live) {
+            beg = A.rowptr[seg];
+            end = A.rowptr[seg + 1];
+            if (end - beg > A.chunk) {
+                live = false;
+                end = beg;
+            }
+        }
+    }
+    const bool cok = tile * 64 + lane < H4;
+    const int c4 = cok ? tile * 64 + lane : 0;
+    const float4 sc = A.scale ? *reinterpret_cast<const float4*>(A.scale + 4 * c4) : make_float4(1.f, 1.f, 1.f, 1.f);
+    const float4 sh = A.shift ? *reinterpret_cast<const float4*>(A.shift + 4 * c4) : make_float4(0.f, 0.f, 0.f, 0.f);
+    float acc[4] = {0.f, 0.f, 0.f, 0.f};
+    uint32_t m = 0;
+    int32_t e = beg;
+    for (; e + 8 <= end; e += 8) apply_pool_batch<SKIP>(A, acc, m, e, 8, c4, cok, sc, sh);
+    if (e < end) apply_pool_batch<SKIP>(A, acc, m, e, end - e, c4, cok, sc, sh);
+    if (A.amax) block_amax(A.amax, m);
+    if (!live || !cok) return;
+    const float s = (seg >= 0 && A.mean) ? inv_deg(end - beg) : 1.f;
+    float* dst = seg >= 0 ? A.out + seg * A.H : A.partial + w * A.H;
+    *reinterpret_cast<float4*>(dst + 4 * c4) = make_float4(acc[0] * s, acc[1] * s, acc[2] * s, acc[3] * s);
+}
+
+__global__ __launch_bounds__(256) void k_pool_grad_scale(const float* __restrict__ g, const int32_t* __restrict__ rowptr,
+                                                         int64_t n, int H, float* __restrict__ out) {
+    const int64_t i = (int64_t)blockIdx.x * 256 + threadIdx.x;
+    if (i >= n) return;
+    const int64_t s = i / H;
+    const int32_t d = rowptr[s + 1] - rowptr[s];
+    out[i] = __fdiv_rn(g[i], (float)(d > 0 ? d : 1));
 }
 
 __global__ __launch_bounds__(256) void k_sage_bwd_stats(const float* __restrict__ g,
@@ -840,6 +945,72 @@
     hipLaunchKernelGGL(k_sage_apply, dim3((unsigned)blocks), dim3(256), 0, s, (const float4*)o, scale, shift,
                        (const float4*)x_prev, skip, thr, inv_keep, seed, n4, H / 4, (float4*)x_next,
                        reinterpret_cast<uint32_t*>(amax), rows_nt(), rev);
+    BGNN_CHECK_LAUNCH();
+    return BGNN_OK;
+}
+
+extern "C" int bgnn_sage_apply_pool(const float* o, const float* scale, const float* shift, const float* x_prev,
+                                    int32_t skip, float p, uint64_t seed, int64_t n_rows, int32_t H, float* x_next,
+                                    float* amax, const bgnn_csr_t* pool, int32_t reduce, float* partial,
+                                    float* pooled, void* stream) {
+    BGNN_REQUIRE(H > 0 && H % 4 == 0, "sage_apply_pool: H must be a multiple of 4");
+    BGNN_REQUIRE(n_rows >= 0, "sage_apply_pool: negative n_rows");
+    BGNN_REQUIRE(n_rows == 0 || o, "sage_apply_pool: null o");
+    BGNN_REQUIRE(p >= 0.f && p < 1.f, "sage_apply_pool: dropout p must be in [0, 1)");
+    BGNN_REQUIRE((scale == nullptr) == (shift == nullptr), "sage_apply_pool: scale/shift must both be set or NULL");
+    BGNN_REQUIRE(!skip || x_prev, "sage_apply_pool: skip requires x_prev");
+    BGNN_REQUIRE(al16(o) && al16(x_next) && (!x_prev || al16(x_prev)) && (!scale || (al16(scale) && al16(shift))),
+                 "sage_apply_pool: pointers must be 16-byte aligned");
+    BGNN_REQUIRE(pool && pool->rowptr, "sage_apply_pool: null pool csr");
+    BGNN_REQUIRE(reduce == BGNN_REDUCE_SUM || reduce == BGNN_REDUCE_MEAN, "sage_apply_pool: reduce must be sum/mean");
+    BGNN_REQUIRE(pool->n_rows >= 0, "sage_apply_pool: negative segment count");
+    BGNN_REQUIRE(pool->nnz == n_rows, "sage_apply_pool: the pool must list each of the n_rows rows once (nnz = %lld)",
+                 (long long)pool->nnz);
+    BGNN_REQUIRE(n_rows == 0 || pool->col, "sage_apply_pool: null col");
+    BGNN_REQUIRE(pool->n_rows == 0 || pooled, "sage_apply_pool: null pooled");
+    BGNN_REQUIRE(pool->n_chunks <= 0 ||
+                     (partial && pool->chunk > 0 && pool->heavy_row && pool->heavy_chunk0 && pool->chunk_heavy),
+                 "sage_apply_pool: heavy segments need partial and the CSR's chunk plan");
+    BGNN_REQUIRE(al16(partial) && al16(pooled), "sage_apply_pool: partial / pooled must be 16-byte aligned");
+    if (n_rows == 0) return BGNN_OK;
+    hipStream_t s = as_stream(stream);
+    ApplyPoolArgs A{};
+    A.o = o; A.scale = scale; A.shift = shift; A.xprev = x_prev;
+    A.thr = dropout_threshold(p);
+    A.inv_keep = A.thr ? 1.f / (1.f - p) : 1.f;
+    A.seed = seed;
+    A.H = H;
+    A.nt = rows_nt();
+    A.xn = x_next;
+    A.amax = reinterpret_cast<uint32_t*>(amax);
+    A.rowptr = pool->rowptr; A.col = pool->col;
+    A.heavy_row = pool->heavy_row; A.heavy_chunk0 = pool->heavy_chunk0; A.chunk_heavy = pool->chunk_heavy;
+    A.n_chunks = pool->n_chunks > 0 ? pool->n_chunks : 0;
+    A.chunk = (A.n_chunks > 0 && pool->chunk > 0) ? pool->chunk : 0x7fffffff;
+    A.mean = reduce == BGNN_REDUCE_MEAN;
+    A.n_light = (A.n_chunks > 0 && pool->n_heavy == pool->n_rows) ? 0 : pool->n_rows;
+    A.partial = partial;
+    A.out = pooled;
+    const int64_t items = A.n_chunks + A.n_light;
+    const int tiles = (H / 4 + 63) / 64;
+    A.ct = tiles <= 2 ? tiles : 4;
+    const int ipb = 4 / A.ct;
+    const dim3 grid((unsigned)((items + ipb - 1) / ipb), (unsigned)((tiles + A.ct - 1) / A.ct));
+    if (skip) hipLaunchKernelGGL(k_sage_apply_pool<true>, grid, dim3(256), 0, s, A);
+    else hipLaunchKernelGGL(k_sage_apply_pool<false>, grid, dim3(256), 0, s, A);
+    BGNN_CHECK_LAUNCH();
+    if (A.n_chunks > 0) return seg_combine_plain(pool, H, reduce, partial, pooled, s);
+    return BGNN_OK;
+}
+
+extern "C" int bgnn_pool_grad_scale(const float* g, const int32_t* rowptr, int64_t segments, int32_t H, float* out,
+                                    void* stream) {
+    BGNN_REQUIRE(segments >= 0 && H > 0, "pool_grad_scale: bad sizes");
+    BGNN_REQUIRE(segments == 0 || (g && rowptr && out), "pool_grad_scale: null pointer");
+    if (segments == 0) return BGNN_OK;
+    const int64_t n = segments * H;
+    hipLaunchKernelGGL(k_pool_grad_scale, dim3((unsigned)((n + 255) / 256)), dim3(256), 0, as_stream(stream), g, rowptr,
+                       n, H, out);
     BGNN_CHECK_LAUNCH();
     return BGNN_OK;
 }
diff --git a/buck-gnn_amd/csrc/spmm.hip b/buck-gnn_amd/csrc/spmm.hip
--- a/buck-gnn_amd/csrc/spmm.hip
+++ b/buck-gnn_amd/csrc/spmm.hip
@@ -1084,6 +1084,21 @@
     return BGNN_OK;
 }
 
+int seg_combine_plain(const bgnn_csr_t* csr, int32_t H, int32_t reduce, float* partial, float* out, hipStream_t s) {
+    SegArgs A = args_from_csr(csr);
+    A.H = H;
+    A.out = out; A.ldo = H;
+    A.partial = partial;
+    A.nt = g_seg_nt;
+    const dim3 grid(A.n_heavy, (H + 511) / 512);
+    if (reduce == BGNN_REDUCE_MEAN)
+        hipLaunchKernelGGL((k_seg_combine<4, 2, 64, OP_MEAN, EPI_PLAIN>), grid, dim3(64 * kCombineWaves), 0, s, A);
+    else
+        hipLaunchKernelGGL((k_seg_combine<4, 2, 64, OP_SUM, EPI_PLAIN>), grid, dim3(64 * kCombineWaves), 0, s, A);
+    BGNN_CHECK_LAUNCH();
+    return BGNN_OK;
+}
+
 extern int g_x6_bdma;
 extern int g_h3p_nsb;
 #ifdef BGNN_H3P_ABLATION
diff --git a/include/bgnn.h b/include/bgnn.h
--- a/include/bgnn.h
+++ b/include/bgnn.h
@@ -8,7 +8,7 @@
 extern "C" {
 #endif
 
-#define BGNN_ABI_VERSION 17
+#define BGNN_ABI_VERSION 18
 
 #define BGNN_OK 0
 #define BGNN_E_ARG 1001
@@ -121,6 +121,15 @@
                     const float* x_prev, int32_t skip, float p, uint64_t seed,
                     int64_t n_rows, int32_t H, float* x_next, float* amax,
                     const int32_t* ranges, float* range_partial, void* stream);
+
+int bgnn_sage_apply_pool(const float* o, const float* scale, const float* shift,
+                         const float* x_prev, int32_t skip, float p, uint64_t seed,
+                         int64_t n_rows, int32_t H, float* x_next, float* amax,
+                         const bgnn_csr_t* pool, int32_t reduce, float* partial, float* pooled,
+                         void* stream);
+
+int bgnn_pool_grad_scale(const float* g, const int32_t* rowptr, int64_t segments, int32_t H,
+                         float* out, void* stream);
 
 int bgnn_sage_infer_bf16(const bgnn_csr_t* csr, const void* z, int64_t ldz, const float* bias,
                          const float* scale, const float* shift, const void* x_prev, int64_t ldx,
```

Measured after the change: 2206, median of 6. +1.8%, better.
